# HuiHuiLan/Clustering-Hidden-Markov-Models-with-Variational-Bayesian-Hierarchical-EM

Measured on AMD Instinct MI355X. Metric: VBHEM E-steps/sec (whole node), N baseHMMs × K clusters × S states; ELBO match, higher is better.
Workload: dtype f64; 1 GPU; C4: N=100000 base HMMs, K=16 clusters, S=8 states, Sb=8, d=8, full cov, tau=10, Nv=100; N=100000, K=16, S=8, Sb=8, d=8, tau=10, parallelism=bases sharded over 1 GPU(s), 1 RCCL all-reduce/E-step

## Files before the change

clustering-hidden-markov-models-with-variational-bayesian-hierarchical-em_amd/csrc/vbhem_capi.hip:

```cpp
#include <hip/hip_runtime.h>

#include <algorithm>
#include <atomic>
#include <chrono>
#include <cmath>
#include <cstdio>
#include <cstring>
#include <cstdlib>
#include <random>
#include <string>
#include <utility>
#include <vector>

#include "vbhem_estep.h"
#include "vbhem_internal.h"
#include "vbhem_exact.h"
#include "vbhem_math.h"

static std::atomic<size_t> g_debug_extra_lds{0};

namespace {

thread_local std::string g_err;

struct TimingState {
  int level = 0;
  std::vector<std::pair<hipEvent_t, hipEvent_t>> fb, stats, em, gf, emd;
  std::vector<long long> fb_pairs;
  std::vector<hipEvent_t> pool;
  ~TimingState() {
    for (hipEvent_t e : pool) (void)hipEventDestroy(e);
  }
};
thread_local TimingState g_timing;

thread_local std::string g_last_kernel[3];
std::string split_name(const vbhem::SplitArgs &a) {
  return "vbhem::fb_split_kernel<" + std::to_string(a.S) + ", " + std::to_string(a.lpc) + ", " +
         std::to_string(a.mode) + ">";
}

struct SwitchRow {
  const char *name;
  long long unset;
  long long vbhem::Switches::*field;
};
constexpr SwitchRow kSwitchRows[] = {
#define X(name, unset, doc) {"VBHEM_" #name, unset, &vbhem::Switches::name},
    VBHEM_SWITCHES(X)
#undef X
};
constexpr int kSwitchCount = (int)(sizeof(kSwitchRows) / sizeof(kSwitchRows[0]));

long long switch_value(const SwitchRow &r, long long v) { return r.unset == 0 ? (v != 0) : v; }

const vbhem::Switches &default_switches() {
  static const vbhem::Switches def = [] {
    vbhem::Switches s;
    for (const SwitchRow &r : kSwitchRows)
      if (const char *ev = std::getenv(r.name)) {
        if (r.unset == 0) s.*r.field = ev[0] != '\0' && std::strcmp(ev, "0") != 0;
        else s.*r.field = std::strtoll(ev, nullptr, 10);
      }
    return s;
  }();
  return def;
}
thread_local vbhem::Switches g_switches = default_switches();

const SwitchRow *find_switch(const char *name) {
  if (!name) return nullptr;
  if (std::strncmp(name, "VBHEM_", 6) == 0) name += 6;
  for (const SwitchRow &r : kSwitchRows)
    if (std::strcmp(name, r.name + 6) == 0) return &r;
  return nullptr;
}

bool timing_on(hipStream_t st, bool fb_launch = false) {
  if (g_timing.level == 0 || (g_timing.level == 2 && !fb_launch)) return false;
  hipStreamCaptureStatus cs = hipStreamCaptureStatusNone;
  if (hipStreamIsCapturing(st, &cs) != hipSuccess) return false;
  return cs == hipStreamCaptureStatusNone;
}

hipEvent_t timing_event(hipStream_t st, bool record = true) {
  hipEvent_t ev = nullptr;
  if (!g_timing.pool.empty()) {
    ev = g_timing.pool.back();
    g_timing.pool.pop_back();
  } else if (hipEventCreateWithFlags(&ev, hipEventDisableSystemFence) != hipSuccess) {
    return nullptr;
  }
  if (record) (void)hipEventRecord(ev, st);
  return ev;
}
void timing_recycle(hipEvent_t ev) {
  if (ev) g_timing.pool.push_back(ev);
}

}

namespace vbhem {
const Switches &switches() { return g_switches; }
void *timing_begin(hipStream_t st) { return timing_on(st) ? timing_event(st) : nullptr; }
void timing_end_em_math(void *ev0, hipStream_t st) {
  if (ev0) g_timing.emd.emplace_back(static_cast<hipEvent_t>(ev0), timing_event(st));
}
unsigned long long flag_tag() {
  static const unsigned long long t = [] {
    std::random_device rd;
    unsigned long long v = ((unsigned long long)rd() << 32) ^ rd();
    v ^= (unsigned long long)std::chrono::steady_clock::now().time_since_epoch().count();
    return v | 1ull;
  }();
  return t;
}
}

namespace {

int fail(int code, const std::string &msg) {
  g_err = msg;
  if (code == VBHEM_ERR_HIP) (void)hipGetLastError();
  return code;
}

}

int vbhem::set_error(int code, const std::string &msg) { return fail(code, msg); }

namespace {

using vbhem::align_up;
using vbhem::hip_fail;

constexpr size_t kLdsLimit = 160 * 1024;
constexpr int kFbMaxThreads = 512;
constexpr int kExactThreads = vbhem::kExactSlots;
constexpr int kChunkMinBases = 64;
constexpr size_t kGroupBudget = (size_t)8 << 30;
constexpr int kMaxSlabs = 512;

inline int odd_up(int x) { return (x % 2 == 0) ? x + 1 : x; }

struct FbPlan {
  vbhem::FbArgs a;
  dim3 block;
  size_t lds;
  int PPB;
};

bool plan_fb(int SB, int d, int covmode, int K, int S, int T, FbPlan &out) {
  const int NE = S * SB;
  if (NE > kFbMaxThreads) return false;
  const int RS = odd_up(SB), AS = odd_up(S), ABS = odd_up(SB);
  const int np = covmode == VBHEM_COV_FULL ? d * (d + 1) / 2 : d;
  const int MS = odd_up(d), PS = odd_up(np);
  double best = -1.0;
  bool found = false;
  for (int ppb = 1; ppb <= 32; ++ppb) {
    const int BJ = std::min(ppb, K);
    const int BI = ppb / BJ;
    const int P = BI * BJ;
    if (P != ppb) continue;
    const int threads = (P * NE + 63) / 64 * 64;
    if (threads > kFbMaxThreads) break;
    size_t off = 0;
    vbhem::FbArgs a{};
    a.off_At = (int)off; off += (size_t)BJ * S * AS;
    a.off_amax = (int)off; off += (size_t)BJ * S;
    a.off_lpi = (int)off; off += (size_t)BJ * S;
    a.off_Ab = (int)off; off += (size_t)BI * SB * ABS;
    a.off_pib = (int)off; off += (size_t)BI * SB;
    a.off_flag = (int)off; off += (size_t)(P + 1) / 2;
    a.off_reg = (int)off;
    size_t k1 = 0;
    a.off_k1m = (int)k1; k1 += (size_t)BJ * S * MS;
    a.off_k1P = (int)k1; k1 += (size_t)BJ * S * PS;
    a.off_k1c = (int)k1; k1 += (size_t)BJ * S;
    a.off_k1mu = (int)k1; k1 += (size_t)BI * SB * MS;
    a.off_k1C = (int)k1; k1 += (size_t)BI * SB * PS;
    const size_t pstride = (size_t)(T - 1) * S * RS + (size_t)(T - 1) * NE + 3 * (size_t)S * RS +
                           (size_t)S * S + SB;
    const size_t reg = std::max(k1, (size_t)P * pstride);
    const size_t lds = (off + reg) * sizeof(double);
    if (lds > kLdsLimit) continue;
    const double util = double(P * NE) / threads;
    const int blocks_per_cu = std::max<int>(1, (int)(kLdsLimit / lds));
    const int waves = std::min(32, blocks_per_cu * threads / 64);
    const double score = util * std::min(waves, 16) + 1e-3 * std::min(threads, 256);
    if (score > best) {
      best = score;
      found = true;
      a.SB = SB; a.d = d; a.covmode = covmode; a.K = K; a.S = S; a.T = T;
      a.BI = BI; a.BJ = BJ; a.NE = NE; a.RS = RS; a.AS = AS; a.ABS = ABS;
      a.njb = (K + BJ - 1) / BJ;
      a.np = np; a.MS = MS; a.PS = PS;
      a.pair_stride = (int)pstride;
      out.a = a;
      out.block = dim3(threads);
      out.lds = lds;
      out.PPB = P;
    }
  }
  return found;
}

struct SplitPlan {
  bool ok = false;
  vbhem::SplitArgs a{};
  size_t lds = 0;
  size_t lds_bwd = 0;
  size_t lds_list = 0;
  int ppb = 0;
  vbhem::SplitArgs al{};
  size_t lds_l = 0;
};

SplitPlan plan_split(int SB, int d, int covmode, int K, int S, int T, int LPC) {
  SplitPlan sp;
  if (!vbhem::split_supported(S, SB, d)) return sp;
  const int SH = (S + LPC - 1) / LPC;
  const int LPP = S * LPC;
  const int XCS = (LPC * SH + 1) / 2 * 2 + 2;
  const int XP = S * XCS + 2;
  const int OFF_X = (2 * S * S + 2 * S + 1) / 2 * 2;
  double best = -1.0;
  for (int nwb = 1; nwb <= 4; ++nwb) {
    const int NT = nwb * 64;
    const int ppb = NT / LPP;
    if (ppb < 1) continue;
    const int off_Y = OFF_X + ppb * XP;
    const int off_F = (off_Y + ppb * S + 1) / 2 * 2;
    const int off_R = (off_F + (ppb + 1) / 2 + 1) / 2 * 2;
    const size_t lattice = (size_t)std::max(0, T - 2) * SH * NT;
    const size_t xi_park = S > 8 ? (size_t)ppb * S * S * LPC * SH : 0;
    const size_t region = std::max<size_t>(std::max(lattice, xi_park), 2);
    const size_t lds = ((size_t)off_R + region) * sizeof(double);
    const int off_L = (int)(off_R + region);
    const size_t lds_list = ((size_t)off_L + ((size_t)K + 2) / 2) * sizeof(double);
    if (lds_list > kLdsLimit) continue;
    const double util = double(ppb * LPP) / NT;
    if (util > best + 0.02 || (LPC != vbhem::split_lpc(S) && util >= best)) {
      best = util;
      vbhem::SplitArgs &x = sp.a;
      x.SB = SB; x.d = d; x.covmode = covmode; x.K = K; x.S = S; x.T = T; x.nwb = nwb;
      x.lpc = LPC;
      x.off_Y = off_Y; x.off_F = off_F; x.off_R = off_R; x.off_L = off_L;
      x.mode = vbhem::kFbDense;
      sp.lds = lds;
      x.off_T = off_R + 2;
      sp.lds_bwd = ((size_t)x.off_T + vbhem::kLogTabDoubles + vbhem::kExpTabDoubles) * sizeof(double);
      sp.lds_list = lds_list;
      sp.ppb = ppb;
      sp.ok = true;
    }
  }
  int best_w = 0;
  for (int nwb : {8, 4, 2, 1}) {
    if (!sp.ok) break;
    const int NT = nwb * 64;
    const int ppb = NT / LPP;
    if (ppb < 1) continue;
    const int off_Y = OFF_X + ppb * XP;
    const int off_F = (off_Y + ppb * S + 1) / 2 * 2;
    const int off_R = (off_F + (ppb + 1) / 2 + 1) / 2 * 2;
    const size_t lattice = (size_t)std::max(0, T - 2) * SH * NT;
    const size_t xi_park = S > 8 ? (size_t)ppb * S * S * LPC * SH : 0;
    const size_t region = std::max<size_t>(std::max(lattice, xi_park), 2);
    const int off_L = (int)(off_R + region);
    const int off_T = (off_L + (K + 2) / 2 + 1) / 2 * 2;
    const size_t lds = ((size_t)off_T + vbhem::kExpTabEntries + 2 * vbhem::kLogTabEntries) * sizeof(double);
    if (lds > kLdsLimit) continue;
    const int waves = std::min(8, nwb * (int)(kLdsLimit / lds));
    if (waves > best_w) {
      best_w = waves;
      vbhem::SplitArgs x = sp.a;
      x.nwb = nwb;
      x.off_Y = off_Y; x.off_F = off_F; x.off_R = off_R; x.off_L = off_L; x.off_T = off_T;
      x.mode = vbhem::kFbList;
      sp.al = x;
      sp.lds_l = lds;
    }
  }
  return sp;
}

size_t exact_stride(int S, int SB, int T) {
  return (size_t)S * S * SB * T + (size_t)vbhem::exact_wave_lds(S, SB);
}

int check_inputs(const vbhem_base_t *b, const vbhem_cluster_t *c, int T, bool need_ptrs = true) {
  if (!b || !c) return fail(VBHEM_ERR_ARG, "null base or cluster descriptor");
  if (b->N < 0 || b->SB < 1 || b->d < 1 || c->K < 1 || c->S < 1 || T < 1)
    return fail(VBHEM_ERR_ARG, "invalid sizes (need N>=0, SB>=1, d>=1, K>=1, S>=1, T>=1)");
  if (b->covmode != VBHEM_COV_DIAG && b->covmode != VBHEM_COV_FULL)
    return fail(VBHEM_ERR_ARG, "covmode must be VBHEM_COV_DIAG or VBHEM_COV_FULL");
  if (need_ptrs && b->N > 0 &&
      (!b->prior || !b->A || !b->centres || !b->covars || !c->logA || !c->logPi || !c->m ||
       !c->P || !c->c))
    return fail(VBHEM_ERR_ARG, "null input array");
  if ((long long)b->N * c->K > 0x7fffffffLL)
    return fail(VBHEM_ERR_UNSUPPORTED, "N*K exceeds 2^31-1 pairs per call; shard the bases");
  return VBHEM_OK;
}

void fill_inputs(vbhem::FbArgs &a, const vbhem_base_t *b, const vbhem_cluster_t *c) {
  a.prior = b->prior; a.A = b->A; a.centres = b->centres; a.covars = b->covars;
  a.logA = c->logA; a.logPi = c->logPi; a.m = c->m; a.P = c->P; a.c = c->c;
}

struct Carver {
  char *base;
  size_t off = 0;
  explicit Carver(void *p) : base(static_cast<char *>(p)) {}
  template <class T>
  T *take(size_t n) {
    off = align_up(off, 256);
    T *p = base ? reinterpret_cast<T *>(base + off) : nullptr;
    off += n * sizeof(T);
    return p;
  }
};

bool u_gemm_ok(const vbhem_base_t *b) {
  return vbhem::emission_kdp(b->d, b->covmode) / 4 <= vbhem::kUMaxKq && !vbhem::switches().NO_UGEMM;
}
bool need_u_ws(const vbhem_base_t *b) { return !b->U && u_gemm_ok(b); }

struct PairsWs {
  int *fpre;
  int *flags;
  double *scratch;
  double *tnu;
  double *E, *W, *bias, *shift;
  double *U;
};

inline size_t emission_w_doubles(int d, int covmode, int K, int S) {
  return (size_t)vbhem::emission_kdp(d, covmode) * vbhem::emission_ksp(K * S);
}

size_t carve_pairs(void *ws, const vbhem_base_t *b, const vbhem_cluster_t *c, int T, bool need_tnu,
                   PairsWs &w) {
  Carver cv(ws);
  const size_t np = (size_t)b->N * c->K;
  w.fpre = cv.take<int>(vbhem::kFlagPre + vbhem::kFlagHead + np);
  w.flags = w.fpre + vbhem::kFlagPre;
  w.tnu = need_tnu ? cv.take<double>(np * c->S * b->SB) : nullptr;
  w.E = cv.take<double>(np * c->S * b->SB);
  w.W = cv.take<double>(emission_w_doubles(b->d, b->covmode, c->K, c->S));
  w.bias = cv.take<double>((size_t)vbhem::emission_ksp(c->K * c->S));
  w.shift = cv.take<double>((size_t)b->d);
  w.U = need_u_ws(b) ? cv.take<double>(vbhem::u_doubles((long long)b->N * b->SB + 16, b->d,
                                                         b->covmode))
                     : nullptr;
  w.scratch = cv.take<double>(exact_stride(c->S, b->SB, T) * kExactThreads);
  return cv.off + 256;
}

struct FusedWs {
  int group;
  int nslab;
  int slab_len;
  int *fpre, *flags;
  int *gate_cnt, *list, *list_tot;
  double *Atg;
  double *scratch, *nu1, *xi, *tnu, *Z, *slabs;
  double *E, *W, *bias, *shift;
  double *U;
  double *l4parts;
};

size_t carve_fused(void *ws, const vbhem_base_t *b, const vbhem_cluster_t *c, int T, FusedWs &w,
                   int R = 1) {
  Carver cv(ws);
  const int K = c->K, S = c->S, SB = b->SB;
  const size_t per_base = (size_t)K * (S + (size_t)S * S + 2 * (size_t)S * SB) * sizeof(double);
  size_t g = std::max<size_t>(1, kGroupBudget / std::max<size_t>(1, per_base));
  g = std::min<size_t>(g, (size_t)std::max(1, b->N));
  const vbhem::Switches &sw = vbhem::switches();
  if (sw.GROUP_BASES >= 0)
    g = std::max<size_t>(1, std::min<size_t>(g, (size_t)sw.GROUP_BASES));
  w.group = (int)g;
  int maxslab = kMaxSlabs;
  if (sw.NSLAB >= 0) maxslab = (int)std::max(1ll, std::min(8192ll, sw.NSLAB));
  w.nslab = std::min<int>(w.group, maxslab);
  w.slab_len = R * (int)vbhem_stats_len(K / R, S, b->d, b->covmode);
  w.fpre = cv.take<int>(vbhem::kFlagPre + vbhem::kFlagHead + 2 * g * K);
  w.flags = w.fpre + vbhem::kFlagPre;
  w.nu1 = cv.take<double>(g * K * S);
  w.xi = cv.take<double>(g * K * S * S);
  w.tnu = cv.take<double>(g * K * S * SB);
  w.Z = cv.take<double>(g * K);
  w.slabs = cv.take<double>((size_t)w.nslab * w.slab_len);
  w.E = cv.take<double>(g * K * S * SB);
  w.W = cv.take<double>(emission_w_doubles(b->d, b->covmode, K, S));
  w.bias = cv.take<double>((size_t)vbhem::emission_ksp(K * S));
  w.shift = cv.take<double>((size_t)b->d);
  w.U = need_u_ws(b) ? cv.take<double>(vbhem::u_doubles((long long)g * SB + 16, b->d, b->covmode))
                     : nullptr;
  w.gate_cnt = cv.take<int>((size_t)w.nslab * K);
  w.list = cv.take<int>(g * K);
  w.list_tot = cv.take<int>((size_t)K);
  w.Atg = cv.take<double>((size_t)K * S * S);
  const int NU = (int)vbhem_stats_nu(b->d, b->covmode);
  w.l4parts = vbhem::list4_acc_supported(S, SB, T, K, NU)
                  ? cv.take<double>((size_t)vbhem::l4s_max_slots(kExactThreads, K) *
                                    vbhem::l4s_part_len(S, vbhem::us_nup(NU)))
                  : nullptr;
  w.scratch = cv.take<double>(exact_stride(S, SB, T) * kExactThreads);
  return cv.off + 256;
}

struct FbCtx {
  FbPlan plan;
  SplitPlan split;
  SplitPlan bwd;
  size_t bwd2_lds = 0;
  int bwd2_ppb = 0, bwd2_nwb = 0;
  bool bwd12 = false;
  bool bwd4 = false;
  bool list4 = false;
  bool list12 = false;
  bool k1_in_kernel = false;
  bool bwd2_prep = false;
  int *fpre = nullptr;
  vbhem::EmissionArgs em{};
  size_t em_lds = 0;
  bool use_u = false;
  size_t em_lds_u = 0;
  const vbhem_base_t *base = nullptr;
  double *u_ws = nullptr;
};

int prepare_fb(FbCtx &c, const vbhem_base_t *b, const vbhem_cluster_t *cl, int T,
               double smooth = 1.0, bool split_first_pass = false) {
  c.split = plan_split(b->SB, b->d, b->covmode, cl->K, cl->S, T, vbhem::split_lpc(cl->S));
  c.bwd = plan_split(b->SB, b->d, b->covmode, cl->K, cl->S, T, vbhem::split_lpc_bwd(cl->S));
  if (c.split.ok) {
    vbhem::EmissionArgs &e = c.em;
    e.SB = b->SB; e.d = b->d; e.covmode = b->covmode; e.K = cl->K; e.S = cl->S;
    e.smooth = smooth;
    e.centres = b->centres; e.covars = b->covars; e.m = cl->m; e.P = cl->P; e.c = cl->c;
    if (!vbhem::plan_emission(e, c.em_lds)) c.split.ok = false;
    if (c.split.ok && u_gemm_ok(b) && vbhem::plan_emission_u(e, c.em_lds_u)) {
      c.use_u = true;
      e.zfix = b->U;
    }
  }
  c.base = b;
  const bool have_elems = plan_fb(b->SB, b->d, b->covmode, cl->K, cl->S, T, c.plan);
  if (!c.split.ok && !have_elems)
    return fail(VBHEM_ERR_UNSUPPORTED,
                "no launch geometry fits (S*SB must be <= 512 and the per-pair lattice "
                "(2*(T-1)+3)*S*SB doubles must fit in 160 KiB of LDS)");
  if (!have_elems) c.plan = FbPlan{};
  fill_inputs(c.plan.a, b, cl);
  c.plan.a.SB = b->SB; c.plan.a.d = b->d; c.plan.a.covmode = b->covmode;
  c.plan.a.K = cl->K; c.plan.a.S = cl->S; c.plan.a.T = T;
  c.plan.a.smooth = smooth;
  if (c.split.ok) {
    vbhem::SplitArgs &a = c.split.a;
    a.prior = b->prior; a.A = b->A; a.logA = cl->logA; a.logPi = cl->logPi;
    vbhem::SplitArgs &al = c.split.al;
    al.prior = b->prior; al.A = b->A; al.logA = cl->logA; al.logPi = cl->logPi;
    vbhem::SplitArgs &ab = c.bwd.a;
    ab.prior = b->prior; ab.A = b->A; ab.logA = cl->logA; ab.logPi = cl->logPi;
    if (c.bwd.ok && cl->S <= vbhem::kBwd2MaxS && !vbhem::switches().NO_BWD2) {
      if (!split_first_pass) {
        c.bwd2_nwb = vbhem::bwd2_waves(cl->S);
        c.bwd2_lds = vbhem::bwd2_lds(cl->S, c.bwd2_nwb);
        c.bwd2_ppb = vbhem::bwd2_ppb(cl->S, c.bwd2_nwb);
        c.bwd4 = vbhem::bwd4_supported(cl->S, b->SB) && !vbhem::switches().NO_BWD4;
        c.bwd12 = vbhem::bwd12_supported(cl->S, b->SB) && !vbhem::switches().NO_BWD12;
      }
      c.list4 = vbhem::list4_supported(cl->S, b->SB, T, cl->K) && !vbhem::switches().NO_LIST4;
      c.list12 = vbhem::list12_supported(cl->S, b->SB, T, cl->K) && !vbhem::switches().NO_LIST12;
    }
    c.k1_in_kernel = c.use_u && c.bwd2_lds && !c.bwd4 && !c.bwd12 && !c.list4 && !c.list12 &&
                     c.em.kdp <= vbhem::kK1InKernelMaxKdp && !vbhem::switches().NO_K1_IN_KERNEL;
  }
  return VBHEM_OK;
}

void set_k1_operands(const FbCtx &c, int i_begin, vbhem::SplitArgs &ca) {
  if (c.base->U) {
    ca.eU = c.base->U;
    ca.e_col0 = 0;
  } else {
    ca.eU = c.u_ws;
    ca.e_col0 = (long long)i_begin * c.base->SB / 16 * 16;
  }
  ca.eW = c.em.W;
  ca.ebias = c.em.bias;
  ca.ekdp = c.em.kdp;
  ca.eksp = c.em.ksp;
  ca.esmooth = c.em.smooth;
}

int run_emission_prep(FbCtx &c, double *W, double *bias, double *shift, hipStream_t st,
                      int *zero_ints = nullptr, int n_zero = 0, double *Atg = nullptr,
                      const double *logA = nullptr) {
  if (!c.split.ok) return VBHEM_OK;
  c.em.W = W; c.em.bias = bias; c.em.shift = shift;
  c.em.zero_ints = zero_ints; c.em.n_zero = zero_ints ? n_zero : 0;
  c.em.Atg = Atg; c.em.logA = logA;
  hipError_t e = vbhem::launch_emission_prep(c.em, st);
  if (e != hipSuccess) return hip_fail(e, "emission_prep_kernel");
  return VBHEM_OK;
}

unsigned list_grid(const vbhem::SplitArgs &a, size_t lds) {
  const int cus = vbhem::device_cus();
  const int per_cu = std::max(1, vbhem::split_resident_blocks(a, lds));
  return (unsigned)(cus * per_cu);
}

int run_fb_list(const FbCtx &c, int i_begin, int i_end, int i_buf0, double *nu1, double *xi,
                double *tnu, const double *Ebuf, long long e_ld, const int *list,
                const int *list_tot, int list_cap, int *flags, double *scratch, double *LL,
                hipStream_t st, bool fold = false, bool *inlined = nullptr,
                const vbhem::StatsArgs *acc_sa = nullptr, double *acc_parts = nullptr,
                int *acc_waves = nullptr) {
  if (i_end <= i_begin) return VBHEM_OK;
  if (!c.split.lds_l) return fail(VBHEM_ERR_UNSUPPORTED, "gate-list pass does not fit LDS");
  vbhem::SplitArgs ca = c.split.al;
  ca.mode = vbhem::kFbList;
  ca.E = Ebuf; ca.e_ld = e_ld;
  ca.i_begin = i_begin; ca.i_end = i_end; ca.i_buf0 = i_buf0;
  ca.LL = nullptr; ca.nu1 = nu1; ca.xi = xi; ca.tnu = tnu;
  ca.flag_count = flags; ca.flag_list = flags + vbhem::kFlagHead;
  ca.list = list; ca.list_tot = list_tot; ca.list_cap = list_cap;
  ca.xinline = 0;
  const vbhem::Switches &sw = vbhem::switches();
  const bool acc = c.list4 && acc_sa && acc_parts && acc_sa->Us && acc_sa->Z && !acc_sa->vhem &&
                   vbhem::list4_acc_supported(ca.S, ca.SB, ca.T, ca.K, acc_sa->NU) &&
                   !sw.NO_LIST4_STATS && !sw.NO_STATS_M && !sw.NO_STATS_U;
  if (acc_waves) *acc_waves = 0;
  auto set_inline = [&](long long waves) {
    if (!(fold || (acc && !sw.NO_FOLD_EXACT)) || waves > kExactThreads || sw.NO_LIST_INLINE) return;
    ca.xinline = 1;
    ca.xscr = scratch;
    ca.xstride = (long long)exact_stride(c.plan.a.S, c.plan.a.SB, c.plan.a.T);
    vbhem::FbArgs &x = ca.xf;
    x = c.plan.a;
    x.i_begin = i_begin; x.i_end = i_end; x.i_buf0 = i_buf0;
    x.LL = LL; x.nu1 = nu1; x.xi = xi; x.tnu = tnu;
    x.flag_count = flags; x.flag_list = flags + vbhem::kFlagHead;
  };
  hipEvent_t ev0 = timing_on(st) ? timing_event(st) : nullptr;
  hipError_t e;
  if (c.list4) {
    ca.Atg = c.bwd.a.Atg;
    unsigned grid = (unsigned)(vbhem::device_cus() * std::max(1, vbhem::list4_resident_blocks(acc)));
    set_inline(vbhem::list4_inline_waves(ca, grid));
    if (acc && ca.xinline) {
      ca.acc = 1;
      ca.acc_nup = vbhem::us_nup(acc_sa->NU);
      ca.accZ = acc_sa->Z; ca.accUs = acc_sa->Us; ca.acc_parts = acc_parts;
      if (acc_waves) *acc_waves = (int)vbhem::list4_inline_waves(ca, grid);
    } else if (acc) {
      grid = (unsigned)(vbhem::device_cus() * std::max(1, vbhem::list4_resident_blocks()));
      if (fold) set_inline(vbhem::list4_inline_waves(ca, grid));
    }
    e = vbhem::launch_list4(ca, grid, st);
    if (e != hipSuccess) return hip_fail(e, "fb_list4_kernel");
    g_last_kernel[1] = "vbhem::fb_list4_kernel<" + std::to_string(ca.T) +
                       (vbhem::list4_fast(ca) ? ", true>" : ", false>");
  } else if (c.list12) {
    ca.Atg = c.bwd.a.Atg;
    const unsigned grid = (unsigned)(vbhem::device_cus() * std::max(1, vbhem::list12_resident_blocks()));
    e = vbhem::launch_list12(ca, grid, st);
    if (e != hipSuccess) return hip_fail(e, "fb_list12_kernel");
    g_last_kernel[1] = "vbhem::fb_list12_kernel<" + std::to_string(ca.T) +
                       (vbhem::list12_fast(ca) ? ", true>" : ", false>");
  } else {
    if (c.k1_in_kernel) set_k1_operands(c, i_begin, ca);
    const unsigned grid = list_grid(ca, c.split.lds_l);
    if (ca.S >= vbhem::kSplitInlineMinS && ca.S <= vbhem::kSplitInlineMaxS)
      set_inline((long long)grid * ca.nwb);
    e = vbhem::launch_split(ca, grid, c.split.lds_l, st);
    if (e != hipSuccess) return hip_fail(e, "fb_split_kernel(list)");
    g_last_kernel[1] = split_name(ca);
  }
  if (ev0) g_timing.gf.emplace_back(ev0, timing_event(st));
  if (inlined) *inlined = ca.xinline != 0;
  if (fold) return VBHEM_OK;
  vbhem::FbArgs a = c.plan.a;
  a.i_begin = i_begin; a.i_end = i_end; a.i_buf0 = i_buf0;
  a.LL = LL; a.nu1 = nu1; a.xi = xi; a.tnu = tnu;
  a.flag_count = flags; a.flag_list = flags + vbhem::kFlagHead;
  e = vbhem::launch_fb_exact(a, scratch, exact_stride(a.S, a.SB, a.T), kExactThreads, st);
  if (e != hipSuccess) return hip_fail(e, "fb_exact_kernel");
  return VBHEM_OK;
}

int run_fb(const FbCtx &c, int i_begin, int i_end, int i_buf0, double *LL, double *nu1,
           double *xi, double *tnu, double *Ebuf, long long e_ld, int *flags, double *scratch,
           hipStream_t st, int mode = vbhem::kFbDense, vbhem::FbArgs *fold = nullptr) {
  if (i_end <= i_begin) return VBHEM_OK;
  vbhem::FbArgs a = c.plan.a;
  a.i_begin = i_begin;
  a.i_end = i_end;
  a.i_buf0 = i_buf0;
  a.LL = LL; a.nu1 = nu1; a.xi = xi; a.tnu = tnu;
  a.flag_count = flags;
  a.flag_list = flags + vbhem::kFlagHead;
  hipError_t e = hipSuccess;
  const bool k1 = c.k1_in_kernel && mode == vbhem::kFbBackward;
  if (!c.split.ok) {
    e = hipMemsetAsync(flags, 0, sizeof(int), st);
    if (e != hipSuccess) return hip_fail(e, "hipMemsetAsync(flags)");
  }
  if (c.split.ok) {
    vbhem::EmissionArgs ea = c.em;
    ea.i_begin = i_begin; ea.i_end = i_end; ea.i_buf0 = i_buf0; ea.E = Ebuf; ea.e_ld = e_ld;
    size_t em_lds = c.em_lds;
    hipEvent_t em0 = !k1 && timing_on(st) ? timing_event(st) : nullptr;
    if (c.use_u) {
      em_lds = c.em_lds_u;
      if (c.base->U) {
        ea.U = c.base->U;
        ea.u_col0 = 0;
      } else {
        if (!c.u_ws) return fail(VBHEM_ERR_WORKSPACE, "no operand buffer for the emission GEMM");
        const vbhem_base_t *b = c.base;
        vbhem::UPrepArgs ua{};
        ua.N = b->N; ua.SB = b->SB; ua.d = b->d; ua.covmode = b->covmode;
        ua.kdp = c.em.kdp; ua.i_begin = i_begin; ua.i_end = i_end;
        ua.u_col0 = (long long)i_begin * b->SB / 16 * 16;
        ua.nstates = b->nstates; ua.centres = b->centres; ua.covars = b->covars;
        ua.U = c.u_ws; ua.z = c.em.shift;
        e = vbhem::launch_u_prep(ua, st);
        if (e != hipSuccess) return hip_fail(e, "u_prep_kernel");
        ea.U = c.u_ws;
        ea.u_col0 = ua.u_col0;
      }
    }
    if (!k1) {
      e = vbhem::launch_emission(ea, em_lds, st);
      if (e != hipSuccess) return hip_fail(e, "emission_kernel");
      if (em0) g_timing.em.emplace_back(em0, timing_event(st));
    }
  }
  const bool ext_timed = c.split.ok && mode == vbhem::kFbBackward && (c.bwd4 || c.bwd12 || c.bwd2_lds);
  const bool timed = timing_on(st, true);
  hipEvent_t ev0 = timed ? timing_event(st, !ext_timed) : nullptr;
  hipEvent_t ev1 = timed && ext_timed ? timing_event(st, false) : nullptr;
  if (c.split.ok) {
    const SplitPlan &sp = mode == vbhem::kFbBackward ? c.bwd : c.split;
    vbhem::SplitArgs ca = sp.a;
    ca.mode = mode;
    ca.E = Ebuf; ca.e_ld = e_ld;
    ca.i_begin = i_begin; ca.i_end = i_end; ca.i_buf0 = i_buf0;
    ca.LL = LL; ca.nu1 = nu1; ca.xi = xi; ca.tnu = tnu;
    ca.flag_count = flags; ca.flag_list = flags + vbhem::kFlagHead;
    const unsigned ntile = (unsigned)((i_end - i_begin + sp.ppb - 1) / sp.ppb);
    unsigned grid = ntile * (unsigned)ca.K;
    if (mode == vbhem::kFbBackward && c.bwd4) {
      const int ppb = vbhem::bwd4_ppb();
      const unsigned nt4 = (unsigned)((i_end - i_begin + ppb - 1) / ppb);
      const unsigned all = (unsigned)(vbhem::device_cus() * std::max(1, vbhem::bwd4_resident_blocks()));
      unsigned nb = std::max(1u, std::min(nt4, all / (unsigned)ca.K));
      if (nb >= 8) nb = nb / 8 * 8;
      e = vbhem::launch_bwd4(ca, (unsigned)ca.K * nb, st, ev1 ? ev0 : nullptr, ev1);
      if (e != hipSuccess) return hip_fail(e, "fb_bwd4_kernel");
      g_last_kernel[0] = vbhem::bwd4_o32(ca) ? "vbhem::fb_bwd4_kernel<true>" : "vbhem::fb_bwd4_kernel<false>";
    } else if (mode == vbhem::kFbBackward && c.bwd12) {
      const int ppb = vbhem::bwd12_ppb();
      const unsigned nt12 = (unsigned)((i_end - i_begin + ppb - 1) / ppb);
      const unsigned all = (unsigned)(vbhem::device_cus() * std::max(1, vbhem::bwd12_resident_blocks()));
      unsigned nb = std::max(1u, std::min(nt12, all / (unsigned)ca.K));
      if (nb >= 8) nb = nb / 8 * 8;
      e = vbhem::launch_bwd12(ca, (unsigned)ca.K * nb, st, ev1 ? ev0 : nullptr, ev1);
      if (e != hipSuccess) return hip_fail(e, "fb_bwd12_kernel");
      g_last_kernel[0] = vbhem::bwd12_o32(ca) ? "vbhem::fb_bwd12_kernel<true>" : "vbhem::fb_bwd12_kernel<false>";
    } else if (mode == vbhem::kFbBackward && c.bwd2_lds) {
      ca.nwb = c.bwd2_nwb;
      if (k1) set_k1_operands(c, i_begin, ca);
      if (k1 && c.bwd2_prep) {
        ca.prep = 1;
        ca.pm = c.em.m; ca.pP = c.em.P; ca.pc = c.em.c; ca.pz = c.em.zfix; ca.pshift = c.em.shift;
        ca.ftag = reinterpret_cast<unsigned long long *>(c.fpre);
        ca.ftag_val = vbhem::flag_tag();
      }
      const unsigned nt2 = (unsigned)((i_end - i_begin + c.bwd2_ppb - 1) / c.bwd2_ppb);
      const unsigned all = (unsigned)(vbhem::device_cus() *
                                      std::max(1, vbhem::bwd2_resident_blocks(ca.S, ca.nwb, c.bwd2_lds)));
      unsigned nb = std::max(1u, std::min(nt2, all / (unsigned)ca.K));
      if (nb >= 8) nb = nb / 8 * 8;
      const size_t lds2 = c.bwd2_lds + g_debug_extra_lds.load(std::memory_order_relaxed);
      e = vbhem::launch_bwd2(ca, (unsigned)ca.K * nb, lds2, st, ev1 ? ev0 : nullptr, ev1);
      if (e != hipSuccess) return hip_fail(e, "fb_bwd2_kernel");
      g_last_kernel[0] = "vbhem::fb_bwd2_kernel<" + std::to_string(ca.S) + ">";
    } else {
      if (mode == vbhem::kFbBackward) {
        unsigned nb = std::max(1u, std::min(ntile, list_grid(ca, sp.lds_bwd) / (unsigned)ca.K));
        if (nb >= 8) nb = nb / 8 * 8;
        grid = (unsigned)ca.K * nb;
      }
      e = vbhem::launch_split(ca, grid, mode == vbhem::kFbBackward ? sp.lds_bwd : sp.lds, st);
      if (e != hipSuccess) return hip_fail(e, "fb_split_kernel");
      g_last_kernel[0] = split_name(ca);
    }
  } else {
    const int nib = (i_end - i_begin + a.BI - 1) / a.BI;
    const dim3 grid((unsigned)nib * (unsigned)a.njb);
    e = vbhem::launch_fb(a, grid, c.plan.block, c.plan.lds, st);
    if (e != hipSuccess) return hip_fail(e, "fb_pairs_kernel");
    g_last_kernel[0] = "vbhem::fb_pairs_kernel";
  }
  if (ev0) {
    g_timing.fb.emplace_back(ev0, ev1 ? ev1 : timing_event(st));
    g_timing.fb_pairs.push_back((long long)(i_end - i_begin) * a.K);
  }
  if (fold) {
    *fold = a;
    return VBHEM_OK;
  }
  e = vbhem::launch_fb_exact(a, scratch, exact_stride(a.S, a.SB, a.T), kExactThreads, st);
  if (e != hipSuccess) return hip_fail(e, "fb_exact_kernel");
  return VBHEM_OK;
}

}

extern "C" {

const char *vbhem_last_error(void) { return g_err.c_str(); }

size_t vbhem_debug_extra_lds(size_t bytes) { return g_debug_extra_lds.exchange(bytes); }

const char *vbhem_last_kernel(int pass) {
  return (pass >= 0 && pass <= 2) ? g_last_kernel[pass].c_str() : "";
}

const char *vbhem_version(void) { return "vbhem-mi355x 0.1.0 (gfx950)"; }

size_t vbhem_stats_nu(int d, int covmode) {
  return covmode == VBHEM_COV_FULL ? (size_t)1 + d + (size_t)d * (d + 1) / 2 : (size_t)1 + 2 * d;
}

size_t vbhem_stats_len(int K, int S, int d, int covmode) {
  return (size_t)K + (size_t)K * S + (size_t)K * S * S + 2 + (size_t)K * S * vbhem_stats_nu(d, covmode);
}

size_t vbhem_prepare_base_bytes(const vbhem_base_t *base) {
  if (!base || base->N < 0 || base->SB < 1 || base->d < 1 || base->d > vbhem::kUHead ||
      (base->covmode != VBHEM_COV_DIAG && base->covmode != VBHEM_COV_FULL))
    return 0;
  if (vbhem::emission_kdp(base->d, base->covmode) / 4 > vbhem::kUMaxKq) return 0;
  return (vbhem::u_doubles((long long)base->N * base->SB, base->d, base->covmode) +
          vbhem::us_doubles(base->N, base->SB, base->d, base->covmode)) * sizeof(double);
}

int vbhem_prepare_base(const vbhem_base_t *base, double *U_dev, size_t bytes, void *stream) {
  const size_t need = vbhem_prepare_base_bytes(base);
  if (need == 0)
    return fail(VBHEM_ERR_UNSUPPORTED, "vbhem_prepare_base: invalid descriptor or d too large");
  if (!U_dev || bytes < need)
    return fail(VBHEM_ERR_WORKSPACE, "vbhem_prepare_base: need " + std::to_string(need) + " bytes");
  if (base->N > 0 && (!base->centres || !base->covars))
    return fail(VBHEM_ERR_ARG, "vbhem_prepare_base: null base array");
  vbhem::UPrepArgs ua{};
  ua.N = base->N; ua.SB = base->SB; ua.d = base->d; ua.covmode = base->covmode;
  ua.kdp = vbhem::emission_kdp(base->d, base->covmode);
  ua.i_begin = 0; ua.i_end = base->N; ua.u_col0 = 0;
  ua.nstates = base->nstates; ua.centres = base->centres; ua.covars = base->covars;
  ua.U = U_dev; ua.z = nullptr;
  hipError_t e = vbhem::launch_u_prep(ua, static_cast<hipStream_t>(stream));
  if (e != hipSuccess) return hip_fail(e, "u_prep_kernel");
  e = vbhem::launch_us_build(ua, U_dev + vbhem::u_doubles((long long)base->N * base->SB, base->d,
                                                         base->covmode),
                             static_cast<hipStream_t>(stream));
  if (e != hipSuccess) return hip_fail(e, "us_build_kernel");
  return VBHEM_OK;
}

size_t vbhem_pairs_workspace_bytes(const vbhem_base_t *base, const vbhem_cluster_t *clus, int T) {
  if (check_inputs(base, clus, T, false) != VBHEM_OK) return 0;
  PairsWs w;
  return carve_pairs(nullptr, base, clus, T, true, w);
}

}

namespace {

int estep_pairs_impl(const vbhem_base_t *base, const vbhem_cluster_t *clus, int T, double smooth,
                     double *LL_elbo_dev, double *sum_nu_1_dev, double *emit_pr_dev,
                     double *emit_mu_dev, double *emit_Mu_dev, double *sum_xi_dev,
                     double *sum_t_nu_dev, void *workspace_dev, size_t workspace_bytes,
                     void *stream) {
  if (!(smooth > 0.0) || !std::isfinite(smooth))
    return fail(VBHEM_ERR_ARG, "smooth must be a positive finite number");
  int rc = check_inputs(base, clus, T);
  if (rc != VBHEM_OK) return rc;
  if (base->N == 0) return VBHEM_OK;
  if (!LL_elbo_dev || !sum_nu_1_dev || !emit_pr_dev || !emit_mu_dev || !emit_Mu_dev || !sum_xi_dev)
    return fail(VBHEM_ERR_ARG, "null output array");
  PairsWs w;
  const size_t need = carve_pairs(nullptr, base, clus, T, sum_t_nu_dev == nullptr, w);
  if (!workspace_dev || workspace_bytes < need)
    return fail(VBHEM_ERR_WORKSPACE, "workspace too small: need " + std::to_string(need) + " bytes");
  carve_pairs(workspace_dev, base, clus, T, sum_t_nu_dev == nullptr, w);
  double *tnu = sum_t_nu_dev ? sum_t_nu_dev : w.tnu;
  hipStream_t st = static_cast<hipStream_t>(stream);
  FbCtx ctx;
  rc = prepare_fb(ctx, base, clus, T, smooth);
  if (rc != VBHEM_OK) return rc;
  ctx.u_ws = w.U;
  if (!ctx.split.ok) {
    hipError_t e0 = hipMemsetAsync(w.fpre, 0, (vbhem::kFlagPre + vbhem::kFlagHead) * sizeof(int), st);
    if (e0 != hipSuccess) return hip_fail(e0, "hipMemsetAsync(flags)");
  }
  rc = run_emission_prep(ctx, w.W, w.bias, w.shift, st, w.fpre, vbhem::kFlagPre + vbhem::kFlagHead);
  if (rc != VBHEM_OK) return rc;
  rc = run_fb(ctx, 0, base->N, 0, LL_elbo_dev, sum_nu_1_dev, sum_xi_dev, tnu, w.E,
              (long long)base->N * base->SB, w.flags,
              w.scratch, st);
  if (rc != VBHEM_OK) return rc;
  vbhem::EmitArgs ea{};
  ea.SB = base->SB; ea.d = base->d; ea.covmode = base->covmode; ea.K = clus->K; ea.S = clus->S;
  ea.i_begin = 0; ea.i_end = base->N;
  ea.centres = base->centres; ea.covars = base->covars; ea.tnu = tnu;
  ea.emit_pr = emit_pr_dev; ea.emit_mu = emit_mu_dev; ea.emit_Mu = emit_Mu_dev;
  hipError_t e = vbhem::launch_emit(ea, st);
  if (e != hipSuccess) return hip_fail(e, "pair_emit_kernel");
  return VBHEM_OK;
}

}

extern "C" {

int vbhem_estep_pairs(const vbhem_base_t *base, const vbhem_cluster_t *clus, int T,
                      double *LL_elbo_dev, double *sum_nu_1_dev, double *emit_pr_dev,
                      double *emit_mu_dev, double *emit_Mu_dev, double *sum_xi_dev,
                      double *sum_t_nu_dev, void *workspace_dev, size_t workspace_bytes,
                      void *stream) {
  return estep_pairs_impl(base, clus, T, 1.0, LL_elbo_dev, sum_nu_1_dev, emit_pr_dev, emit_mu_dev,
                          emit_Mu_dev, sum_xi_dev, sum_t_nu_dev, workspace_dev, workspace_bytes,
                          stream);
}

int vhem_estep_pairs(const vbhem_base_t *base, const vbhem_cluster_t *clus, int T, double smooth,
                     double *LL_elbo_dev, double *sum_nu_1_dev, double *emit_pr_dev,
                     double *emit_mu_dev, double *emit_Mu_dev, double *sum_xi_dev,
                     double *sum_t_nu_dev, void *workspace_dev, size_t workspace_bytes,
                     void *stream) {
  return estep_pairs_impl(base, clus, T, smooth, LL_elbo_dev, sum_nu_1_dev, emit_pr_dev,
                          emit_mu_dev, emit_Mu_dev, sum_xi_dev, sum_t_nu_dev, workspace_dev,
                          workspace_bytes, stream);
}

size_t vbhem_fused_workspace_bytes(const vbhem_base_t *base, const vbhem_cluster_t *clus, int T) {
  return vbhem_fused_trials_workspace_bytes(base, clus, 1, T);
}

size_t vbhem_fused_trials_workspace_bytes(const vbhem_base_t *base, const vbhem_cluster_t *clus,
                                          int R, int T) {
  if (check_inputs(base, clus, T, false) != VBHEM_OK || R < 1 || clus->K % R != 0) return 0;
  FusedWs w;
  return carve_fused(nullptr, base, clus, T, w, R);
}

int vbhem_estep_fused(const vbhem_base_t *base, const vbhem_cluster_t *clus, int T,
                      const double *tildeN_dev, const double *logOmega_dev, double *stats_dev,
                      double *hatZ_dev, double *LL_elbo_dev, void *workspace_dev,
                      size_t workspace_bytes, void *stream) {
  return vbhem_estep_fused_trials(base, clus, 1, T, tildeN_dev, logOmega_dev, stats_dev, hatZ_dev,
                                  LL_elbo_dev, workspace_dev, workspace_bytes, stream);
}

static std::atomic<unsigned long long *> g_done_word{nullptr};
static std::atomic<unsigned long long> g_done_val{0};

int vbhem_arm_done_word(void *word, unsigned long long value) {
  if (word && reinterpret_cast<uintptr_t>(word) % 8 != 0) return fail(VBHEM_ERR_ARG, "done word not 8-byte aligned");
  g_done_val.store(value);
  g_done_word.store(static_cast<unsigned long long *>(word));
  return VBHEM_OK;
}

int vbhem_done_word_alloc(void **host_ptr, void **dev_ptr) {
  if (!host_ptr || !dev_ptr) return fail(VBHEM_ERR_ARG, "null pointer");
  void *h = nullptr;
  hipError_t e = hipHostMalloc(&h, 64, hipHostMallocMapped | hipHostMallocCoherent);
  if (e != hipSuccess) return hip_fail(e, "hipHostMalloc(done word)");
  std::memset(h, 0, 64);
  void *d = nullptr;
  e = hipHostGetDevicePointer(&d, h, 0);
  if (e != hipSuccess) {
    (void)hipHostFree(h);
    return hip_fail(e, "hipHostGetDevicePointer(done word)");
  }
  *host_ptr = h;
  *dev_ptr = d;
  return VBHEM_OK;
}

int vbhem_done_word_free(void *host_ptr) {
  if (!host_ptr) return VBHEM_OK;
  const hipError_t e = hipHostFree(host_ptr);
  return e == hipSuccess ? VBHEM_OK : hip_fail(e, "hipHostFree(done word)");
}

struct VhemIn {
  double smooth, inf_norm;
  const double *omegaB;
};

static int fused_impl(const vbhem_base_t *base, const vbhem_cluster_t *clus, int R, int T,
                      const double *tildeN_dev, const double *logOmega_dev, double *stats_dev,
                      double *hatZ_dev, double *LL_elbo_dev, void *workspace_dev,
                      size_t workspace_bytes, void *stream, const VhemIn *vh) {
  unsigned long long *const done_word = g_done_word.exchange(nullptr);
  const unsigned long long done_val = g_done_val.load();
  int rc = check_inputs(base, clus, T);
  if (rc != VBHEM_OK) return rc;
  if (vh) {
    if (!(vh->smooth > 0.0) || !std::isfinite(vh->smooth))
      return fail(VBHEM_ERR_ARG, "smooth must be a positive finite number");
    if (!(vh->inf_norm > 0.0) || !std::isfinite(vh->inf_norm))
      return fail(VBHEM_ERR_ARG, "inf_norm must be a positive finite number");
    if (base->N > 0 && !vh->omegaB) return fail(VBHEM_ERR_ARG, "null fused argument");
  }
  if (R < 1 || clus->K % R != 0)
    return fail(VBHEM_ERR_ARG, "trials: K must be a positive multiple of R");
  if (!vh && R > 1 && clus->K > 256)
    return fail(VBHEM_ERR_UNSUPPORTED, "trials: at most 256 clusters in total (R * K_trial)");
  if (!logOmega_dev || !stats_dev ||
      (base->N > 0 && (!tildeN_dev || !hatZ_dev || !LL_elbo_dev)))
    return fail(VBHEM_ERR_ARG, "null fused argument");
  if ((vh ? vbhem::vhem_resp_lds(clus->K, clus->K / R) : vbhem::resp_lds(clus->K, clus->K / R)) >
      kLdsLimit)
    return fail(VBHEM_ERR_UNSUPPORTED, "fused: too many clusters for the responsibilities "
                                       "kernel (K <= ~2,400)");
  FusedWs w;
  const size_t need = carve_fused(nullptr, base, clus, T, w, R);
  if (!workspace_dev || workspace_bytes < need)
    return fail(VBHEM_ERR_WORKSPACE, "workspace too small: need " + std::to_string(need) + " bytes");
  carve_fused(workspace_dev, base, clus, T, w, R);
  hipStream_t st = static_cast<hipStream_t>(stream);

  const int K = clus->K, S = clus->S, SB = base->SB, d = base->d;
  vbhem::StatsArgs sa{};
  sa.K = K; sa.S = S; sa.SB = SB; sa.d = d; sa.covmode = base->covmode;
  sa.NU = (int)vbhem_stats_nu(d, base->covmode);
  sa.slab_len = w.slab_len;
  sa.KT = K / R;
  sa.SL = w.slab_len / R;
  sa.centres = base->centres; sa.covars = base->covars; sa.LL = LL_elbo_dev;
  sa.nu1 = w.nu1; sa.xi = w.xi; sa.tnu = w.tnu; sa.tildeN = tildeN_dev; sa.logOmega = logOmega_dev;
  sa.Z = w.Z; sa.hatZ = hatZ_dev; sa.slabs = w.slabs;
  if (vh) {
    sa.vhem = 1;
    sa.omegaB = vh->omegaB;
    sa.inf_norm = vh->inf_norm;
  }
  size_t slds = 0;
  int ngroups = 1;
  const bool dense_ok = vbhem::plan_stats(sa, slds, ngroups);

  FbCtx ctx;
  rc = prepare_fb(ctx, base, clus, T, vh ? vh->smooth : 1.0, vh != nullptr);
  if (rc != VBHEM_OK) return rc;
  ctx.u_ws = w.U;
  size_t sl_lds = 0;
  const vbhem::Switches &sw = vbhem::switches();
  const bool gated = !sw.FUSED_DENSE && ctx.split.ok && ctx.split.lds_l &&
                     vbhem::plan_stats_list(sa, sl_lds) &&
                     vbhem::gate_list_lds(K) <= kLdsLimit;
  if (R > 1 && !gated)
    return fail(VBHEM_ERR_UNSUPPORTED,
                "trials need the gated schedule (split-kernel shapes: S <= 16, Sb <= S)");
  if (!gated && !dense_ok)
    return fail(VBHEM_ERR_UNSUPPORTED, "statistics tile does not fit (S or d too large)");
  sa.gate_cnt = gated ? w.gate_cnt : nullptr;
  sa.list = w.list; sa.list_tot = w.list_tot; sa.list_cap = w.group;
  auto chunks = [&w](int nb) { return std::min(w.nslab, (nb + kChunkMinBases - 1) / kChunkMinBases); };
  const int nslab_used = std::max(1, chunks(std::min(base->N, w.group)));
  sa.nzero_m = std::min(nslab_used, 128);
  int stats_slabs = nslab_used;
  hipError_t e = hipSuccess;
  if (!gated || base->N == 0) {
    e = hipMemsetAsync(w.slabs, 0, sizeof(double) * (size_t)nslab_used * w.slab_len, st);
    if (e != hipSuccess) return hip_fail(e, "hipMemsetAsync(slabs)");
  }
  struct HeadGuard {
    int *fpre;
    hipStream_t st;
    ~HeadGuard() {
      if (fpre) (void)hipMemsetAsync(fpre, 0, (vbhem::kFlagPre + vbhem::kFlagHead) * sizeof(int), st);
    }
  } guard{w.fpre, st};
  if (!ctx.split.ok) {
    e = hipMemsetAsync(w.fpre, 0, (vbhem::kFlagPre + vbhem::kFlagHead) * sizeof(int), st);
    if (e != hipSuccess) return hip_fail(e, "hipMemsetAsync(flags)");
  }
  if (gated) ctx.bwd.a.Atg = w.Atg;
  if (gated && ctx.k1_in_kernel && ctx.em.zfix && ctx.bwd2_nwb * 64 >= 512 &&
      !sw.NO_BWD2_PREP) {
    ctx.em.W = w.W; ctx.em.bias = w.bias; ctx.em.shift = w.shift;
    ctx.bwd2_prep = true;
    ctx.fpre = w.fpre;
  } else {
    rc = run_emission_prep(ctx, w.W, w.bias, w.shift, st, w.fpre, vbhem::kFlagPre + vbhem::kFlagHead,
                           gated ? w.Atg : nullptr, clus->logA);
    if (rc != VBHEM_OK) return rc;
  }
  const bool fold = gated && R == 1 && base->N <= w.group && ctx.split.ok && K < kExactThreads &&
                    w.nslab <= kExactThreads && !sw.NO_FOLD_EXACT;
  sa.fold = 0;
  for (int g0 = 0; g0 < base->N; g0 += w.group) {
    const int g1 = std::min(base->N, g0 + w.group);
    const long long e_ld = (long long)w.group * SB;
    rc = run_fb(ctx, g0, g1, g0, LL_elbo_dev, w.nu1, w.xi, w.tnu, w.E, e_ld, w.flags, w.scratch,
                st, gated ? vbhem::kFbBackward : vbhem::kFbDense, fold ? &sa.fx : nullptr);
    if (rc != VBHEM_OK) return rc;
    if (fold) {
      sa.fold = 1;
      sa.xscratch = w.scratch;
      sa.xstride = (long long)exact_stride(S, SB, T);
      sa.xslots = kExactThreads;
    }
    sa.i_begin = g0; sa.i_end = g1; sa.i_buf0 = g0;
    sa.assign = gated && g0 == 0;
    sa.U = nullptr;
    sa.Us = nullptr;
    if (ctx.split.ok && ctx.use_u) {
      sa.ukdp = ctx.em.kdp;
      if (base->U) {
        sa.U = base->U; sa.uz = base->U; sa.u_col0 = 0;
        sa.Us = base->U + vbhem::u_doubles((long long)base->N * SB, base->d, base->covmode);
      } else if (ctx.u_ws) {
        sa.U = ctx.u_ws; sa.uz = ctx.em.shift; sa.u_col0 = (long long)g0 * SB / 16 * 16;
      }
    }
    const int nchunk = std::max(1, chunks(g1 - g0));
    hipEvent_t ev0 = timing_on(st) ? timing_event(st) : nullptr;
    e = vbhem::launch_resp(sa, nchunk, st);
    if (e != hipSuccess) return hip_fail(e, "resp_kernel");
    if (gated) {
      e = vbhem::launch_gate_list(sa, nchunk, st);
      if (e != hipSuccess) return hip_fail(e, "gate_list_kernel");
      if (ev0) g_timing.stats.emplace_back(ev0, timing_event(st));
      bool inl = false;
      int l4w = 0;
      rc = run_fb_list(ctx, g0, g1, g0, w.nu1, w.xi, w.tnu, w.E, e_ld, w.list, w.list_tot,
                       w.group, w.flags, w.scratch, LL_elbo_dev, st, fold, &inl, &sa, w.l4parts, &l4w);
      if (rc != VBHEM_OK) return rc;
      if (fold) sa.fold = inl ? 2 : 1;
      ev0 = timing_on(st) ? timing_event(st) : nullptr;
      int ss = nchunk;
      if (l4w > 0) {
        ss = 1;
        g_last_kernel[2] = "vbhem::list4_stats_reduce_kernel";
        e = vbhem::launch_list4_stats_reduce(sa, w.l4parts, l4w, st);
        if (e != hipSuccess) return hip_fail(e, "list4_stats_reduce_kernel");
      } else {
        g_last_kernel[2] = "vbhem::stats_list_kernels";
        e = vbhem::launch_stats_list(sa, nchunk, sl_lds, st, &ss);
      }
      if (e != hipSuccess) return hip_fail(e, "stats_list_kernel");
      if (g0 == 0) stats_slabs = ss;
    } else {
      e = vbhem::launch_stats(sa, nchunk, ngroups, slds, st);
      if (e != hipSuccess) return hip_fail(e, "stats_kernel");
    }
    if (ev0) g_timing.stats.emplace_back(ev0, timing_event(st));
  }
  e = vbhem::launch_stats_final(w.slabs, nslab_used, stats_slabs, w.slab_len, sa.KT, S, sa.SL,
                                stats_dev, st, w.fpre, done_word, done_val);
  if (e != hipSuccess) return hip_fail(e, "stats_final_kernel");
  guard.fpre = nullptr;
  return VBHEM_OK;
}

int vbhem_estep_fused_trials(const vbhem_base_t *base, const vbhem_cluster_t *clus, int R, int T,
                             const double *tildeN_dev, const double *logOmega_dev,
                             double *stats_dev, double *hatZ_dev, double *LL_elbo_dev,
                             void *workspace_dev, size_t workspace_bytes, void *stream) {
  return fused_impl(base, clus, R, T, tildeN_dev, logOmega_dev, stats_dev, hatZ_dev, LL_elbo_dev,
                    workspace_dev, workspace_bytes, stream, nullptr);
}

size_t vhem_fused_workspace_bytes(const vbhem_base_t *base, const vbhem_cluster_t *clus, int T) {
  return vbhem_fused_trials_workspace_bytes(base, clus, 1, T);
}

size_t vhem_fused_trials_workspace_bytes(const vbhem_base_t *base, const vbhem_cluster_t *clus,
                                         int R, int T) {
  return vbhem_fused_trials_workspace_bytes(base, clus, R, T);
}

int vhem_estep_fused(const vbhem_base_t *base, const vbhem_cluster_t *clus, int T, double smooth,
                     const double *Ni_dev, const double *omegaB_dev, double inf_norm,
                     const double *logOmega_dev, double *stats_dev, double *Z_dev,
                     double *LL_elbo_dev, void *workspace_dev, size_t workspace_bytes,
                     void *stream) {
  return vhem_estep_fused_trials(base, clus, 1, T, smooth, Ni_dev, omegaB_dev, inf_norm,
                                 logOmega_dev, stats_dev, Z_dev, LL_elbo_dev, workspace_dev,
                                 workspace_bytes, stream);
}

int vhem_estep_fused_trials(const vbhem_base_t *base, const vbhem_cluster_t *clus, int R, int T,
                            double smooth, const double *Ni_dev, const double *omegaB_dev,
                            double inf_norm, const double *logOmega_dev, double *stats_dev,
                            double *Z_dev, double *LL_elbo_dev, void *workspace_dev,
                            size_t workspace_bytes, void *stream) {
  const VhemIn vh{smooth, inf_norm, omegaB_dev};
  return fused_impl(base, clus, R, T, Ni_dev, logOmega_dev, stats_dev, Z_dev, LL_elbo_dev,
                    workspace_dev, workspace_bytes, stream, &vh);
}

int vbhem_set_fused_mode(int mode) {
  const int prev = g_switches.FUSED_DENSE ? VBHEM_FUSED_DENSE : VBHEM_FUSED_GATED;
  if (mode == VBHEM_FUSED_GATED || mode == VBHEM_FUSED_DENSE)
    g_switches.FUSED_DENSE = mode == VBHEM_FUSED_DENSE;
  return prev;
}

int vbhem_switch_count(void) { return kSwitchCount; }

const char *vbhem_switch_name(int index) {
  return index >= 0 && index < kSwitchCount ? kSwitchRows[index].name : nullptr;
}

int vbhem_switch_get(const char *name, long long *value) {
  const SwitchRow *r = find_switch(name);
  if (!r) return fail(VBHEM_ERR_ARG, std::string("unknown switch: ") + (name ? name : "(null)"));
  if (value) *value = g_switches.*r->field;
  return VBHEM_OK;
}

int vbhem_switch_set(const char *name, long long value, long long *previous) {
  const SwitchRow *r = find_switch(name);
  if (!r) return fail(VBHEM_ERR_ARG, std::string("unknown switch: ") + (name ? name : "(null)"));
  if (previous) *previous = g_switches.*r->field;
  g_switches.*r->field = switch_value(*r, value);
  return VBHEM_OK;
}

void vbhem_switch_reset(void) { g_switches = default_switches(); }

int vbhem_timing_enable(int on) {
  g_timing.level = (on == 1 || on == 2) ? on : 0;
  return VBHEM_OK;
}

int vbhem_timing_read(double *fb_ms, long long *fb_launches, long long *fb_pairs, double *stats_ms,
                      long long *stats_launches) {
  double f = 0.0, s = 0.0;
  long long np = 0;
  int rc = VBHEM_OK;
  auto drain = [&rc](std::vector<std::pair<hipEvent_t, hipEvent_t>> &v, double &acc) {
    for (auto &pr : v) {
      float ms = 0.f;
      if (pr.first && pr.second) {
        hipError_t e = hipEventSynchronize(pr.second);
        if (e == hipSuccess) e = hipEventElapsedTime(&ms, pr.first, pr.second);
        if (e != hipSuccess) rc = hip_fail(e, "vbhem_timing_read");
        acc += ms;
      }
      timing_recycle(pr.first);
      timing_recycle(pr.second);
    }
  };
  const long long nf = (long long)g_timing.fb.size(), ns = (long long)g_timing.stats.size();
  drain(g_timing.fb, f);
  drain(g_timing.stats, s);
  for (long long x : g_timing.fb_pairs) np += x;
  g_timing.fb.clear();
  g_timing.stats.clear();
  g_timing.fb_pairs.clear();
  if (fb_ms) *fb_ms = f;
  if (fb_launches) *fb_launches = nf;
  if (fb_pairs) *fb_pairs = np;
  if (stats_ms) *stats_ms = s;
  if (stats_launches) *stats_launches = ns;
  return rc;
}

static int drain_events(std::vector<std::pair<hipEvent_t, hipEvent_t>> &v, double *ms_out,
                        long long *n_out, const char *where) {
  double t = 0.0;
  int rc = VBHEM_OK;
  const long long n = (long long)v.size();
  for (auto &pr : v) {
    float ms = 0.f;
    if (pr.first && pr.second) {
      hipError_t e = hipEventSynchronize(pr.second);
      if (e == hipSuccess) e = hipEventElapsedTime(&ms, pr.first, pr.second);
      if (e != hipSuccess) rc = hip_fail(e, where);
      t += ms;
    }
    timing_recycle(pr.first);
    timing_recycle(pr.second);
  }
  v.clear();
  if (ms_out) *ms_out = t;
  if (n_out) *n_out = n;
  return rc;
}

int vbhem_timing_read_em_math(double *ms, long long *launches) {
  return drain_events(g_timing.emd, ms, launches, "vbhem_timing_read_em_math");
}

int vbhem_timing_read_gated(double *fwd_ms, long long *fwd_launches) {
  return drain_events(g_timing.gf, fwd_ms, fwd_launches, "vbhem_timing_read_gated");
}

int vbhem_timing_read_emission(double *em_ms, long long *em_launches) {
  double t = 0.0;
  int rc = VBHEM_OK;
  const long long n = (long long)g_timing.em.size();
  for (auto &pr : g_timing.em) {
    float ms = 0.f;
    if (pr.first && pr.second) {
      hipError_t e = hipEventSynchronize(pr.second);
      if (e == hipSuccess) e = hipEventElapsedTime(&ms, pr.first, pr.second);
      if (e != hipSuccess) rc = hip_fail(e, "vbhem_timing_read_emission");
      t += ms;
    }
    timing_recycle(pr.first);
    timing_recycle(pr.second);
  }
  g_timing.em.clear();
  if (em_ms) *em_ms = t;
  if (em_launches) *em_launches = n;
  return rc;
}

int vbhem_last_fallback_count(void *stream, const void *workspace_dev) {
  int v[vbhem::kFlagPre + 2] = {0};
  if (!workspace_dev) return fail(VBHEM_ERR_ARG, "null workspace");
  hipStream_t st = static_cast<hipStream_t>(stream);
  hipError_t e = hipMemcpyAsync(v, workspace_dev, sizeof(v), hipMemcpyDeviceToHost, st);
  if (e == hipSuccess) e = hipStreamSynchronize(st);
  if (e != hipSuccess) return hip_fail(e, "vbhem_last_fallback_count");
  if (v[vbhem::kFlagLost] == vbhem::kFlagLostMark)
    return fail(VBHEM_ERR_WORKSPACE, "fb_bwd2_kernel lost the flag-head handshake: the fused "
                                     "call's statistics are NaN (results untrusted)");
  return std::max(v[2], std::max(v[vbhem::kFlagPre], v[vbhem::kFlagPre + 1]));
}

int vbhem_host_device_pointer(void *host_ptr, void **dev_ptr) {
  if (!host_ptr || !dev_ptr) return fail(VBHEM_ERR_ARG, "null pointer");
  *dev_ptr = nullptr;
  hipPointerAttribute_t at{};
  if (hipPointerGetAttributes(&at, host_ptr) != hipSuccess || at.type != hipMemoryTypeHost) {
    (void)hipGetLastError();
    return fail(VBHEM_ERR_ARG, "not pinned host memory");
  }
  void *d = nullptr;
  hipError_t e = hipHostGetDevicePointer(&d, host_ptr, 0);
  if (e != hipSuccess || !d) {
    (void)hipGetLastError();
    return fail(VBHEM_ERR_ARG, "pinned host memory is not mapped for the device");
  }
  *dev_ptr = d;
  return VBHEM_OK;
}

}

namespace {

int estep_pairs_host_impl(int device, const vbhem_base_t *bh, const vbhem_cluster_t *ch, int T,
                          double smooth, double *LL_elbo, double *sum_nu_1, double *emit_pr,
                          double *emit_mu, double *emit_Mu, double *sum_xi) {
  int rc = check_inputs(bh, ch, T);
  if (rc != VBHEM_OK) return rc;
  if (bh->N == 0) return VBHEM_OK;
  hipError_t e = hipSetDevice(device);
  if (e != hipSuccess) return hip_fail(e, "hipSetDevice");
  const size_t N = bh->N, SB = bh->SB, d = bh->d, K = ch->K, S = ch->S;
  const size_t dC = bh->covmode == VBHEM_COV_FULL ? d * d : d;
  const size_t n_in[] = {N * SB, N * SB * SB, N * SB * d, N * SB * dC,
                         K * S * S, K * S, K * S * d, K * S * dC, K * S};
  const double *h_in[] = {bh->prior, bh->A, bh->centres, bh->covars,
                          ch->logA, ch->logPi, ch->m, ch->P, ch->c};
  const size_t n_out[] = {N * K, N * K * S, N * K * S, N * K * S * d, N * K * S * dC, N * K * S * S};
  double *h_out[] = {LL_elbo, sum_nu_1, emit_pr, emit_mu, emit_Mu, sum_xi};
  double *d_in[9] = {nullptr};
  double *d_out[6] = {nullptr};
  void *ws = nullptr;
  rc = VBHEM_OK;
  for (int k = 0; k < 9 && rc == VBHEM_OK; ++k) {
    e = hipMalloc(&d_in[k], std::max<size_t>(1, n_in[k]) * sizeof(double));
    if (e == hipSuccess) e = hipMemcpy(d_in[k], h_in[k], n_in[k] * sizeof(double), hipMemcpyHostToDevice);
    if (e != hipSuccess) rc = hip_fail(e, "upload");
  }
  for (int k = 0; k < 6 && rc == VBHEM_OK; ++k) {
    e = hipMalloc(&d_out[k], std::max<size_t>(1, n_out[k]) * sizeof(double));
    if (e != hipSuccess) rc = hip_fail(e, "hipMalloc(out)");
  }
  vbhem_base_t bd = *bh;
  vbhem_cluster_t cd = *ch;
  bd.nstates = nullptr;
  bd.U = nullptr;
  bd.prior = d_in[0]; bd.A = d_in[1]; bd.centres = d_in[2]; bd.covars = d_in[3];
  cd.logA = d_in[4]; cd.logPi = d_in[5]; cd.m = d_in[6]; cd.P = d_in[7]; cd.c = d_in[8];
  size_t wsb = 0;
  if (rc == VBHEM_OK) {
    wsb = vbhem_pairs_workspace_bytes(&bd, &cd, T);
    e = hipMalloc(&ws, wsb);
    if (e != hipSuccess) rc = hip_fail(e, "hipMalloc(workspace)");
  }
  if (rc == VBHEM_OK)
    rc = estep_pairs_impl(&bd, &cd, T, smooth, d_out[0], d_out[1], d_out[2], d_out[3], d_out[4],
                          d_out[5], nullptr, ws, wsb, nullptr);
  if (rc == VBHEM_OK) {
    e = hipDeviceSynchronize();
    if (e != hipSuccess) rc = hip_fail(e, "kernel execution");
  }
  for (int k = 0; k < 6 && rc == VBHEM_OK; ++k) {
    e = hipMemcpy(h_out[k], d_out[k], n_out[k] * sizeof(double), hipMemcpyDeviceToHost);
    if (e != hipSuccess) rc = hip_fail(e, "download");
  }
  for (int k = 0; k < 9; ++k) if (d_in[k]) (void)hipFree(d_in[k]);
  for (int k = 0; k < 6; ++k) if (d_out[k]) (void)hipFree(d_out[k]);
  if (ws) (void)hipFree(ws);
  return rc;
}

}

extern "C" {

int vbhem_estep_pairs_host(int device, const vbhem_base_t *bh, const vbhem_cluster_t *ch, int T,
                           double *LL_elbo, double *sum_nu_1, double *emit_pr, double *emit_mu,
                           double *emit_Mu, double *sum_xi) {
  return estep_pairs_host_impl(device, bh, ch, T, 1.0, LL_elbo, sum_nu_1, emit_pr, emit_mu,
                               emit_Mu, sum_xi);
}

int vhem_estep_pairs_host(int device, const vbhem_base_t *bh, const vbhem_cluster_t *ch, int T,
                          double smooth, double *LL_elbo, double *sum_nu_1, double *emit_pr,
                          double *emit_mu, double *emit_Mu, double *sum_xi) {
  return estep_pairs_host_impl(device, bh, ch, T, smooth, LL_elbo, sum_nu_1, emit_pr, emit_mu,
                               emit_Mu, sum_xi);
}

}

struct vbhem_ctx {
  int device = 0, N = 0, SB = 0, d = 0, covmode = 0, K = 0, S = 0, R = 1, T = 1;
  size_t stats_len = 0, ws_bytes = 0;
  hipStream_t stream = nullptr;
  int *nstates = nullptr;
  double *prior = nullptr, *A = nullptr, *centres = nullptr, *covars = nullptr;
  double *logA = nullptr, *logPi = nullptr, *m = nullptr, *P = nullptr, *c = nullptr;
  double *tildeN = nullptr, *logOmega = nullptr, *stats = nullptr, *hatZ = nullptr, *LL = nullptr;
  double *U = nullptr;
  void *ws = nullptr;
};

namespace {

void ctx_free(vbhem_ctx *x) {
  if (!x) return;
  int prev = 0;
  const bool dev_ok = hipGetDevice(&prev) == hipSuccess && hipSetDevice(x->device) == hipSuccess;
  void *ptrs[] = {x->nstates, x->prior, x->A, x->centres, x->covars, x->logA, x->logPi, x->m,
                  x->P, x->c, x->tildeN, x->logOmega, x->stats, x->hatZ, x->LL, x->U, x->ws};
  for (void *q : ptrs)
    if (q) (void)hipFree(q);
  if (x->stream) (void)hipStreamDestroy(x->stream);
  if (dev_ok) (void)hipSetDevice(prev);
  delete x;
}

template <class T>
hipError_t dev_alloc(T **p, size_t n) {
  return hipMalloc(reinterpret_cast<void **>(p), std::max<size_t>(1, n) * sizeof(T));
}

}

extern "C" {

int vbhem_ctx_create(int device, const vbhem_base_t *bh, int K, int S, int R, int T,
                     vbhem_ctx_t **ctx_out) {
  if (!ctx_out) return fail(VBHEM_ERR_ARG, "null context pointer");
  *ctx_out = nullptr;
  vbhem_cluster_t probe{K, S, nullptr, nullptr, nullptr, nullptr, nullptr};
  int rc = check_inputs(bh, &probe, T, false);
  if (rc != VBHEM_OK) return rc;
  if (bh->N > 0 && (!bh->prior || !bh->A || !bh->centres || !bh->covars))
    return fail(VBHEM_ERR_ARG, "null base array");
  if (R < 1 || K % R != 0) return fail(VBHEM_ERR_ARG, "trials: K must be a positive multiple of R");
  vbhem_ctx *x = new vbhem_ctx;
  x->device = device; x->N = bh->N; x->SB = bh->SB; x->d = bh->d; x->covmode = bh->covmode;
  x->K = K; x->S = S; x->R = R; x->T = T;
  x->stats_len = (size_t)R * vbhem_stats_len(K / R, S, bh->d, bh->covmode);
  hipError_t e = hipSetDevice(device);
  if (e != hipSuccess) { ctx_free(x); return hip_fail(e, "hipSetDevice"); }
  e = hipStreamCreateWithFlags(&x->stream, hipStreamNonBlocking);
  const size_t N = bh->N, SB = bh->SB, d = bh->d;
  const size_t dC = bh->covmode == VBHEM_COV_FULL ? d * d : d;
  if (e == hipSuccess) e = dev_alloc(&x->nstates, N);
  if (e == hipSuccess) e = dev_alloc(&x->prior, N * SB);
  if (e == hipSuccess) e = dev_alloc(&x->A, N * SB * SB);
  if (e == hipSuccess) e = dev_alloc(&x->centres, N * SB * d);
  if (e == hipSuccess) e = dev_alloc(&x->covars, N * SB * dC);
  if (e == hipSuccess) e = dev_alloc(&x->logA, (size_t)K * S * S);
  if (e == hipSuccess) e = dev_alloc(&x->logPi, (size_t)K * S);
  if (e == hipSuccess) e = dev_alloc(&x->m, (size_t)K * S * d);
  if (e == hipSuccess) e = dev_alloc(&x->P, (size_t)K * S * dC);
  if (e == hipSuccess) e = dev_alloc(&x->c, (size_t)K * S);
  if (e == hipSuccess) e = dev_alloc(&x->tildeN, N);
  if (e == hipSuccess) e = dev_alloc(&x->logOmega, (size_t)K);
  if (e == hipSuccess) e = dev_alloc(&x->stats, x->stats_len);
  if (e == hipSuccess) e = dev_alloc(&x->hatZ, N * K);
  if (e == hipSuccess) e = dev_alloc(&x->LL, N * K);
  if (e != hipSuccess) { ctx_free(x); return hip_fail(e, "vbhem_ctx_create(alloc)"); }
  if (N > 0) {
    if (bh->nstates) {
      e = hipMemcpy(x->nstates, bh->nstates, N * sizeof(int), hipMemcpyHostToDevice);
    } else {
      std::vector<int> ns(N, (int)SB);
      e = hipMemcpy(x->nstates, ns.data(), N * sizeof(int), hipMemcpyHostToDevice);
    }
    if (e == hipSuccess) e = hipMemcpy(x->prior, bh->prior, N * SB * 8, hipMemcpyHostToDevice);
    if (e == hipSuccess) e = hipMemcpy(x->A, bh->A, N * SB * SB * 8, hipMemcpyHostToDevice);
    if (e == hipSuccess) e = hipMemcpy(x->centres, bh->centres, N * SB * d * 8, hipMemcpyHostToDevice);
    if (e == hipSuccess) e = hipMemcpy(x->covars, bh->covars, N * SB * dC * 8, hipMemcpyHostToDevice);
    if (e != hipSuccess) { ctx_free(x); return hip_fail(e, "vbhem_ctx_create(upload)"); }
  }
  vbhem_base_t bd{bh->N, bh->SB, bh->d, bh->covmode, x->nstates, x->prior, x->A, x->centres,
                  x->covars, nullptr};
  if (const size_t ub = vbhem_prepare_base_bytes(&bd)) {
    e = hipMalloc(&x->U, ub);
    if (e != hipSuccess) { ctx_free(x); return hip_fail(e, "vbhem_ctx_create(U)"); }
    rc = vbhem_prepare_base(&bd, x->U, ub, x->stream);
    if (rc != VBHEM_OK) { ctx_free(x); return rc; }
    bd.U = x->U;
  }
  vbhem_cluster_t cd{K, S, x->logA, x->logPi, x->m, x->P, x->c};
  x->ws_bytes = vbhem_fused_trials_workspace_bytes(&bd, &cd, R, T);
  if (x->ws_bytes == 0) { ctx_free(x); return fail(VBHEM_ERR_ARG, "vbhem_ctx_create: bad sizes"); }
  e = hipMalloc(&x->ws, x->ws_bytes);
  if (e != hipSuccess) { ctx_free(x); return hip_fail(e, "vbhem_ctx_create(workspace)"); }
  *ctx_out = x;
  return VBHEM_OK;
}

int vbhem_ctx_fused(vbhem_ctx_t *x, const vbhem_cluster_t *ch, const double *tildeN_host,
                    const double *logOmega_host, double *stats_host, double *hatZ_host,
                    double *LL_host) {
  if (!x || !ch) return fail(VBHEM_ERR_ARG, "null context or cluster descriptor");
  if (ch->K != x->K || ch->S != x->S)
    return fail(VBHEM_ERR_ARG, "cluster descriptor K/S differ from the context's");
  if (!ch->logA || !ch->logPi || !ch->m || !ch->P || !ch->c || !logOmega_host || !stats_host ||
      (x->N > 0 && !tildeN_host))
    return fail(VBHEM_ERR_ARG, "null host array");
  hipError_t e = hipSetDevice(x->device);
  if (e != hipSuccess) return hip_fail(e, "hipSetDevice");
  const size_t K = x->K, S = x->S, d = x->d, N = x->N;
  const size_t dC = x->covmode == VBHEM_COV_FULL ? d * d : d;
  hipStream_t st = x->stream;
  e = hipMemcpyAsync(x->logA, ch->logA, K * S * S * 8, hipMemcpyHostToDevice, st);
  if (e == hipSuccess) e = hipMemcpyAsync(x->logPi, ch->logPi, K * S * 8, hipMemcpyHostToDevice, st);
  if (e == hipSuccess) e = hipMemcpyAsync(x->m, ch->m, K * S * d * 8, hipMemcpyHostToDevice, st);
  if (e == hipSuccess) e = hipMemcpyAsync(x->P, ch->P, K * S * dC * 8, hipMemcpyHostToDevice, st);
  if (e == hipSuccess) e = hipMemcpyAsync(x->c, ch->c, K * S * 8, hipMemcpyHostToDevice, st);
  if (e == hipSuccess) e = hipMemcpyAsync(x->logOmega, logOmega_host, K * 8, hipMemcpyHostToDevice, st);
  if (e == hipSuccess && N > 0)
    e = hipMemcpyAsync(x->tildeN, tildeN_host, N * 8, hipMemcpyHostToDevice, st);
  if (e != hipSuccess) return hip_fail(e, "vbhem_ctx_fused(upload)");
  vbhem_base_t bd{x->N, x->SB, x->d, x->covmode, x->nstates, x->prior, x->A, x->centres,
                  x->covars, x->U};
  vbhem_cluster_t cd{x->K, x->S, x->logA, x->logPi, x->m, x->P, x->c};
  int rc = vbhem_estep_fused_trials(&bd, &cd, x->R, x->T, x->tildeN, x->logOmega, x->stats,
                                    x->hatZ, x->LL, x->ws, x->ws_bytes, st);
  if (rc != VBHEM_OK) return rc;
  e = hipMemcpyAsync(stats_host, x->stats, x->stats_len * 8, hipMemcpyDeviceToHost, st);
  if (e == hipSuccess && hatZ_host && N > 0)
    e = hipMemcpyAsync(hatZ_host, x->hatZ, N * K * 8, hipMemcpyDeviceToHost, st);
  if (e == hipSuccess && LL_host && N > 0)
    e = hipMemcpyAsync(LL_host, x->LL, N * K * 8, hipMemcpyDeviceToHost, st);
  if (e == hipSuccess) e = hipStreamSynchronize(st);
  if (e != hipSuccess) return hip_fail(e, "vbhem_ctx_fused(download)");
  return VBHEM_OK;
}

void vbhem_ctx_destroy(vbhem_ctx_t *x) { ctx_free(x); }

int vbhem_estep_fused_host(int device, const vbhem_base_t *bh, const vbhem_cluster_t *ch, int T,
                           const double *tildeN_host, const double *logOmega_host,
                           double *stats_host, double *hatZ_host, double *LL_host) {
  if (!ch) return fail(VBHEM_ERR_ARG, "null cluster descriptor");
  vbhem_ctx_t *x = nullptr;
  int rc = vbhem_ctx_create(device, bh, ch->K, ch->S, 1, T, &x);
  if (rc != VBHEM_OK) return rc;
  rc = vbhem_ctx_fused(x, ch, tildeN_host, logOmega_host, stats_host, hatZ_host, LL_host);
  vbhem_ctx_destroy(x);
  return rc;
}

}
```

clustering-hidden-markov-models-with-variational-bayesian-hierarchical-em_amd/csrc/vbhem_internal.h:

```cpp
#pragma once
#include <hip/hip_runtime.h>

#include <cstddef>
#include <map>
#include <mutex>
#include <string>
#include <tuple>

#include "vbhem_estep.h"
#include "vbhem_switches.h"
#include "vbhem_list4_slots.h"

namespace vbhem {

int set_error(int code, const std::string &msg);
static inline int hip_fail(hipError_t e, const char *where) {
  return set_error(VBHEM_ERR_HIP, std::string(where) + ": " + hipGetErrorString(e));
}

static inline size_t align_up(size_t x, size_t a) { return (x + a - 1) / a * a; }

inline int current_device() {
  int dev = 0;
  if (hipGetDevice(&dev) != hipSuccess) dev = 0;
  return dev;
}
inline hipError_t set_dyn_lds(const void *fn, size_t lds) {
  static std::mutex mu;
  static std::map<std::pair<int, const void *>, size_t> done;
  const auto key = std::make_pair(current_device(), fn);
  std::lock_guard<std::mutex> g(mu);
  auto it = done.find(key);
  if (it != done.end() && it->second >= lds) return hipSuccess;
  hipError_t e = hipFuncSetAttribute(fn, hipFuncAttributeMaxDynamicSharedMemorySize, (int)lds);
  if (e == hipSuccess) done[key] = lds;
  return e;
}
inline int resident_per_cu(const void *fn, int threads, size_t lds) {
  static std::mutex mu;
  static std::map<std::tuple<int, const void *, int, size_t>, int> memo;
  const auto key = std::make_tuple(current_device(), fn, threads, lds);
  {
    std::lock_guard<std::mutex> g(mu);
    auto it = memo.find(key);
    if (it != memo.end()) return it->second;
  }
  int n = 0;
  if (set_dyn_lds(fn, lds) != hipSuccess ||
      hipOccupancyMaxActiveBlocksPerMultiprocessor(&n, fn, threads, lds) != hipSuccess || n < 1)
    return 1;
  std::lock_guard<std::mutex> g(mu);
  memo[key] = n;
  return n;
}
inline int device_cus() {
  static std::mutex mu;
  static std::map<int, int> cus;
  const int dev = current_device();
  {
    std::lock_guard<std::mutex> g(mu);
    auto it = cus.find(dev);
    if (it != cus.end()) return it->second;
  }
  int n = 0;
  if (hipDeviceGetAttribute(&n, hipDeviceAttributeMultiprocessorCount, dev) != hipSuccess || n < 1)
    return 256;
  std::lock_guard<std::mutex> g(mu);
  cus[dev] = n;
  return n;
}

constexpr int kCovDiag = 0;
constexpr int kCovFull = 1;

struct FbArgs {
  int SB, d, covmode, K, S, T;
  int BI, BJ, NE, RS, AS, ABS, njb;
  int i_begin, i_end, i_buf0;
  int np, MS, PS;
  const double *prior, *A, *centres, *covars;
  const double *logA, *logPi, *m, *P, *c;
  double *LL, *nu1, *xi, *tnu;
  int *flag_count, *flag_list;
  int off_At, off_amax, off_lpi, off_Ab, off_pib, off_flag, off_reg;
  int off_k1m, off_k1P, off_k1c, off_k1mu, off_k1C;
  int pair_stride;
  double smooth;
};

struct EmitArgs {
  int SB, d, covmode, K, S;
  int i_begin, i_end;
  const double *centres, *covars, *tnu;
  double *emit_pr, *emit_mu, *emit_Mu;
};

struct StatsArgs {
  int K, S, SB, SBp, d, covmode, NU;
  int JG;
  int NBB;
  int AST;
  int UST;
  int i_begin, i_end, i_buf0, slab_len;
  const double *centres, *covars, *LL, *nu1, *xi, *tnu, *tildeN, *logOmega;
  double *Z;
  double *hatZ, *slabs;
  int *gate_cnt;
  int *list;
  int *list_tot;
  int list_cap;
  int PB;
  int assign;
  int KT, SL;
  const double *U, *uz;
  long long u_col0;
  int ukdp;
  int nzero;
  const double *Us;
  int nzero_m;
  int fold;
  FbArgs fx;
  double *xscratch;
  long long xstride;
  int xslots;
  int vhem;
  const double *omegaB;
  double inf_norm;
};

constexpr int kSplitMaxS = 16;
template <int S>
struct SplitLPC {
#ifdef VBHEM_SPLIT_LPC5
  static constexpr int value = S <= 4 ? 1 : S == 5 ? VBHEM_SPLIT_LPC5 : S <= 8 ? 2 : 4;
#else
  static constexpr int value = S <= 4 ? 1 : S <= 8 ? 2 : 4;
#endif
};
template <int S>
struct BwdLPC {
  static constexpr int value = S <= 8 ? 1 : 2;
};
template <int S, int LPC>
struct SplitLayout {
  static constexpr int SH = (S + LPC - 1) / LPC;
  static constexpr int XCS = (LPC * SH + 1) / 2 * 2 + 2;
  static constexpr int XP = S * XCS + 2;
  static constexpr int HEAD = 2 * S * S + 2 * S;
  static constexpr int OFF_X = (HEAD + 1) / 2 * 2;
};
inline int emission_kdp(int d, int covmode) {
  const int kd = covmode == kCovFull ? d * (d + 1) / 2 + d : 2 * d;
  return (kd + 3) / 4 * 4;
}
inline int emission_ksp(int ks) { return (ks + 127) / 128 * 128; }

struct EmissionArgs {
  int SB, d, covmode, K, S, KD, CB;
  int kdp, ksp;
  bool wfull;
  bool wlds;
  int nwave;
  int i_begin, i_end, i_buf0;
  long long e_ld;
  const double *centres, *covars, *m, *P, *c;
  double *W, *bias, *shift;
  double *E;
  double smooth;
  const double *U, *zfix;
  long long u_col0;
  int urc;
  int ukqb;
  const double *logA;
  double *Atg;
  int *zero_ints;
  int n_zero;
};
bool plan_emission(EmissionArgs &a, size_t &lds);
bool plan_emission_u(EmissionArgs &a, size_t &lds);

constexpr int kUHead = 64;
constexpr int kUMaxKq = 40;
inline long long u_tiles(long long ncols) { return (ncols + 15) / 16; }
inline size_t u_doubles(long long ncols, int d, int covmode) {
  return (size_t)kUHead + (size_t)u_tiles(ncols) * (emission_kdp(d, covmode) / 4) * 64;
}
struct UPrepArgs {
  int N, SB, d, covmode, kdp;
  int i_begin, i_end;
  long long u_col0;
  const int *nstates;
  const double *centres, *covars;
  double *U;
  const double *z;
};
hipError_t launch_u_prep(const UPrepArgs &a, hipStream_t st);
__host__ __device__ inline int us_sbp(int SB) { return (SB + 3) / 4 * 4; }
__host__ __device__ inline int us_nup(int NU) { return (NU + 15) / 16 * 16; }
__host__ __device__ inline int us_nu(int d, int covmode) { return 1 + d + (covmode == kCovFull ? d * (d + 1) / 2 : d); }
inline size_t us_doubles(long long N, int SB, int d, int covmode) {
  return (size_t)N * us_sbp(SB) * us_nup(us_nu(d, covmode));
}
hipError_t launch_us_build(const UPrepArgs &a, double *Us, hipStream_t st);
hipError_t launch_emission_prep(const EmissionArgs &a, hipStream_t st);
hipError_t launch_emission(const EmissionArgs &a, size_t lds, hipStream_t st);

enum FbMode : int { kFbDense = 0, kFbBackward = 1, kFbList = 2 };

struct SplitArgs {
  int SB, d, covmode, K, S, T, nwb, lpc;
  int mode;
  int i_begin, i_end, i_buf0;
  int off_Y, off_F, off_R;
  int off_L;
  int off_T;
  const double *prior, *A;
  const double *logA, *logPi;
  const double *E;
  long long e_ld;
  double *LL, *nu1, *xi, *tnu;
  int *flag_count, *flag_list;
  const int *list, *list_tot;
  int list_cap;
  const double *Atg;
  const double *eU, *eW, *ebias;
  long long e_col0;
  int ekdp, eksp;
  double esmooth;
  int xinline;
  double *xscr;
  long long xstride;
  FbArgs xf;
  int prep;
  const double *pm, *pP, *pc, *pz;
  double *pshift;
  unsigned long long *ftag;
  unsigned long long ftag_val;
  int acc;
  int acc_nup;
  const double *accZ;
  const double *accUs;
  double *acc_parts;
};

constexpr double kLog2PiE = 1.8378770664093454835606594728112353;
__device__ __forceinline__ double em_psym(const double *P, int a, int b, int d) {
  return 0.5 * (P[a * d + b] + P[b * d + a]);
}
__device__ __forceinline__ double em_pm_full(const double *P, const double *mr, const double *zs,
                                             int a, int d) {
  double v = 0.0;
  for (int b = 0; b < d; ++b) v = fma(em_psym(P, a, b, d), mr[b] - zs[b], v);
  return v;
}
__device__ __forceinline__ double em_w_full(const double *P, int a, int b, int d) {
  return -0.5 * ((a == b) ? P[a * d + a] : em_psym(P, a, b, d));
}
__device__ __forceinline__ double em_bias(int d, double c, double q) {
  return -0.5 * (d * kLog2PiE + c + q);
}

constexpr int kK1InKernelMaxKdp = 8;
constexpr int kSplitInlineMinS = 4, kSplitInlineMaxS = 6;

__device__ __forceinline__ void k1_column(const SplitArgs &p, long long col,
                                          double (&u)[kK1InKernelMaxKdp]) {
  const long long c = col - p.e_col0;
  const double *Ut = p.eU + kUHead + (size_t)(c >> 4) * (p.ekdp / 4) * 64 + (int)(c & 15);
#pragma unroll
  for (int e = 0; e < kK1InKernelMaxKdp; ++e)
    u[e] = e < p.ekdp ? Ut[(e >> 2) * 64 + (e & 3) * 16] : 0.0;
}
__device__ __forceinline__ double k1_entry(const SplitArgs &p, int jr,
                                           const double (&u)[kK1InKernelMaxKdp]) {
  double acc = p.ebias[jr];
#pragma unroll
  for (int e = 0; e < kK1InKernelMaxKdp; ++e)
    if (e < p.ekdp) acc = fma(p.eW[(size_t)e * p.eksp + jr], u[e], acc);
  return acc;
}
bool split_supported(int S, int SB, int d);
int split_lpc(int S);
int split_lpc_bwd(int S);
hipError_t launch_split(const SplitArgs &a, unsigned grid, size_t lds, hipStream_t st);
int split_resident_blocks(const SplitArgs &a, size_t lds);

constexpr int kBwd2MaxS = 16;
int bwd2_waves(int S);
size_t bwd2_lds(int S, int nwb);
int bwd2_ppb(int S, int nwb);
int bwd2_resident_blocks(int S, int nwb, size_t lds);
hipError_t launch_bwd2(const SplitArgs &a, unsigned grid, size_t lds, hipStream_t st,
                       hipEvent_t t0 = nullptr, hipEvent_t t1 = nullptr);

void *timing_begin(hipStream_t st);
void timing_end_em_math(void *ev0, hipStream_t st);

bool bwd4_supported(int S, int SB);
int bwd4_waves();
int bwd4_ppb();
int bwd4_resident_blocks();
bool bwd4_o32(const SplitArgs &a);
bool bwd12_o32(const SplitArgs &a);
bool list4_fast(const SplitArgs &a);
bool list12_fast(const SplitArgs &a);
hipError_t launch_bwd4(const SplitArgs &a, unsigned grid, hipStream_t st, hipEvent_t t0 = nullptr,
                       hipEvent_t t1 = nullptr);
bool bwd12_supported(int S, int SB);
int bwd12_ppb();
int bwd12_resident_blocks();
hipError_t launch_bwd12(const SplitArgs &a, unsigned grid, hipStream_t st, hipEvent_t t0 = nullptr,
                        hipEvent_t t1 = nullptr);

constexpr int kList4MaxK = 1024;
bool list4_supported(int S, int SB, int T, int K);
int list4_resident_blocks(bool acc = false);
long long list4_inline_waves(const SplitArgs &a, unsigned grid);
hipError_t launch_list4(const SplitArgs &a, unsigned grid, hipStream_t st);
bool list4_acc_supported(int S, int SB, int T, int K, int NU);
hipError_t launch_list4_stats_reduce(const StatsArgs &a, const double *parts, int nw, hipStream_t st);

bool list12_supported(int S, int SB, int T, int K);
int list12_resident_blocks();
hipError_t launch_list12(const SplitArgs &a, unsigned grid, hipStream_t st);

hipError_t launch_fb(const FbArgs &a, dim3 grid, dim3 block, size_t lds, hipStream_t st);
constexpr int kFlagHead = 4;
constexpr int kFlagPre = 4;
constexpr int kFlagLost = 3;
constexpr int kFlagLostMark = 0x4C4F5354;
unsigned long long flag_tag();
constexpr int kFlagBad = 1, kFlagNonFinite = 2;
#ifndef VBHEM_EXACT_BLOCK
#define VBHEM_EXACT_BLOCK 512
#endif
constexpr int kExactBlock = VBHEM_EXACT_BLOCK;
constexpr int kExactBlocks = 131072 / kExactBlock;
constexpr int kExactSlots = kExactBlocks * kExactBlock / 64;
hipError_t launch_fb_exact(const FbArgs &a, double *scratch, size_t stride, int nslots,
                           hipStream_t st, bool from_fold = false);
hipError_t launch_emit(const EmitArgs &a, hipStream_t st);
bool plan_stats(StatsArgs &a, size_t &lds, int &ngroups);
hipError_t launch_resp(const StatsArgs &a, int nchunk, hipStream_t st);
hipError_t launch_stats(const StatsArgs &a, int nchunk, int ngroups, size_t lds, hipStream_t st);
bool plan_stats_list(StatsArgs &a, size_t &lds);
hipError_t launch_gate_list(const StatsArgs &a, int nchunk, hipStream_t st);
size_t gate_list_lds(int K);
size_t resp_lds(int K, int KT);
size_t vhem_resp_lds(int K, int KT);
hipError_t launch_stats_list(const StatsArgs &a, int nchunk, size_t lds, hipStream_t st,
                             int *stats_slabs = nullptr);
hipError_t launch_stats_final(const double *slabs, int nslab, int nslab_stats, int slab_len, int KT,
                              int S, int SL, double *out, hipStream_t st, int *fpre = nullptr,
                              unsigned long long *done = nullptr, unsigned long long done_val = 0);

}
```

clustering-hidden-markov-models-with-variational-bayesian-hierarchical-em_amd/csrc/vbhem_stats.hip:

```cpp
#include <hip/hip_runtime.h>

#include <algorithm>
#include <cmath>
#include <cstdlib>

#include "vbhem_internal.h"
#include "vbhem_exact.h"

namespace vbhem {

namespace {

typedef double double4_t __attribute__((ext_vector_type(4)));

__device__ __forceinline__ double wave_max(double v) {
#pragma unroll
  for (int off = 32; off >= 1; off >>= 1) v = fmax(v, __shfl_xor(v, off, 64));
  return v;
}
__device__ __forceinline__ double wave_sum(double v) {
#pragma unroll
  for (int off = 32; off >= 1; off >>= 1) v += __shfl_xor(v, off, 64);
  return v;
}

__device__ __forceinline__ int qdiv(int x, float inv) { return (int)(((float)x + 0.5f) * inv); }

__device__ __forceinline__ void chunk_range(int nb, int i_begin, int chunk, int nchunk, int &b0,
                                            int &b1) {
  const int per = (nb + nchunk - 1) / nchunk;
  b0 = i_begin + chunk * per;
  b1 = min(i_begin + nb, b0 + per);
}

}

constexpr double kGateZ = 1e-8;
constexpr int kGateVbhem = 0, kGateVhem = 1;
template <int GM>
struct Gate {
  static constexpr double value = GM == kGateVhem ? 0.0 : kGateZ;
};

#ifndef VBHEM_RESP_THREADS
#define VBHEM_RESP_THREADS 512
#endif
constexpr int kRespThreads = VBHEM_RESP_THREADS;
constexpr int kRespFoldWaves = 4;

__device__ __forceinline__ double group_max(double v, int G) {
  for (int off = G >> 1; off >= 1; off >>= 1) v = fmax(v, __shfl_xor(v, off, 64));
  return v;
}
__device__ __forceinline__ double group_sum(double v, int G) {
  for (int off = G >> 1; off >= 1; off >>= 1) v += __shfl_xor(v, off, 64);
  return v;
}

#ifndef VBHEM_RESP_UNROLL
#define VBHEM_RESP_UNROLL 1
#endif

#ifndef VBHEM_RESP_WPE
#define VBHEM_RESP_WPE 4
#endif
typedef unsigned int resp_u2 __attribute__((ext_vector_type(2)));

template <int KP>
__global__ __launch_bounds__(kRespThreads) __attribute__((amdgpu_waves_per_eu(VBHEM_RESP_WPE))) void resp_kernel(
    const StatsArgs p) {
  extern __shared__ double lds[];
  const int tid = threadIdx.x, lane = tid & 63, wave = tid >> 6;
  constexpr int NW = kRespThreads / 64;
  const int K = KP ? KP : p.K;
  int G = KP ? KP : 1;
  if (!KP)
    while (G < K && G < 64) G <<= 1;
  const int BPW = 64 / G;
  const int sub = lane / G, gl = lane - sub * G;
  double *accNj = lds;
  double *accLt = accNj + NW * BPW * K;
  int *gcnt = reinterpret_cast<int *>(accLt + 2 * NW);
  int b0, b1;
  chunk_range(p.i_end - p.i_begin, p.i_begin, blockIdx.x, gridDim.x, b0, b1);
  if (p.fold) {
    int *fc = p.fx.flag_count;
    const int cnt = __atomic_load_n(fc, __ATOMIC_RELAXED);
    if (blockIdx.x == 0 && tid == 0) fc[3] = cnt;
    if (cnt > 0) {
      const int nw = min(kRespFoldWaves, max(1, p.xslots / (int)gridDim.x));
      int *q = reinterpret_cast<int *>(lds), *qn = q + kRespThreads;
      auto mine = [&](int pair) { const int i = pair / K; return i >= b0 && i < b1; };
      if (exact_wave_in_lds(p.fx.S, p.fx.SB))
        fold_exact<false>(p.fx, 0, cnt, mine, p.xscratch, p.xstride, (int)blockIdx.x * nw, nw, q, qn,
                          lds + fold_lds_bytes(kRespThreads, 0, 1, 1) / sizeof(double));
      else
        fold_exact<true>(p.fx, 0, cnt, mine, p.xscratch, p.xstride, (int)blockIdx.x * nw, nw, q, qn,
                         nullptr);
    }
  }
  for (int x = tid; x < NW * BPW * K + 2 * NW; x += kRespThreads) accNj[x] = 0.0;
  for (int x = tid; x < K; x += kRespThreads) gcnt[x] = 0;
  __syncthreads();
  double l1 = 0.0, l7 = 0.0;
  if constexpr (KP > 0) {
    constexpr int BP = 64 / KP;
    const int stride = NW * BP;
    const double lo = p.logOmega[gl];
    const int nb = b1 - b0;
    const __amdgpu_buffer_rsrc_t rh = __builtin_amdgcn_make_buffer_rsrc(
        p.hatZ + (size_t)b0 * KP, (short)0, nb * KP * 8, 0x00020000);
    const __amdgpu_buffer_rsrc_t rz = __builtin_amdgcn_make_buffer_rsrc(
        p.Z + (size_t)(b0 - p.i_buf0) * KP, (short)0, nb * KP * 8, 0x00020000);
    auto step = [&](int ib, double tnb, double llb) {
#pragma clang fp contract(off)
      const bool iv = ib < b1;
      const double lz = tnb * (lo + llb);
      double mx = lz;
#pragma unroll
      for (int off = KP >> 1; off >= 1; off >>= 1) mx = fmax(mx, __shfl_xor(mx, off, 64));
      double sm = exp(lz - mx);
#pragma unroll
      for (int off = KP >> 1; off >= 1; off >>= 1) sm += __shfl_xor(sm, off, 64);
      const double lse = mx + log(sm);
      const double hz = exp(lz - lse) + 1e-50;
      const double Z = hz * tnb;
      const int off = iv ? ((ib - b0) * KP + gl) * 8 : 0x7ffffff0;
      __builtin_amdgcn_raw_buffer_store_b64(__builtin_bit_cast(resp_u2, hz), rh, off, 0, 0);
      __builtin_amdgcn_raw_buffer_store_b64(__builtin_bit_cast(resp_u2, Z), rz, off, 0, 0);
      accNj[(wave * BP + sub) * KP + gl] += iv ? Z : 0.0;
      atomicAdd(&gcnt[gl], (iv && Z > kGateZ) ? 1 : 0);
      l1 += iv ? Z * llb : 0.0;
      l7 += iv ? hz * log(hz) : 0.0;
    };
    auto ld = [&](int ib, double &tnb, double &llb) {
      const int ii = ib < b1 ? ib : b0;
      tnb = p.tildeN[ii];
      llb = p.LL[(size_t)ii * KP + gl];
    };
    int i = b0 + wave * BP + sub;
    double tA, lA, tB, lB;
    ld(i, tA, lA);
    for (; i - sub < b1; i += 2 * stride) {
      ld(i + stride, tB, lB);
      step(i, tA, lA);
      ld(i + 2 * stride, tA, lA);
      step(i + stride, tB, lB);
    }
  } else if (K <= G) {
    const int stride = NW * BPW;
    const double lo = gl < K ? p.logOmega[gl] : 0.0;
    int i = b0 + wave * BPW + sub;
    int ii = i < b1 ? i : b0;
    double tn = p.tildeN[ii];
    double ll = gl < K ? p.LL[(size_t)ii * K + gl] : 0.0;
    auto step = [&](int ib, double tnb, double llb) {
#pragma clang fp contract(off)
      const bool iv = ib < b1;
      const double lz = tnb * (lo + llb);
      double mx = gl < K ? lz : -INFINITY;
      mx = group_max(mx, G);
      double sm = gl < K ? exp(lz - mx) : 0.0;
      sm = group_sum(sm, G);
      const double lse = mx + log(sm);
      if (iv && gl < K) {
        const double hz = exp(lz - lse) + 1e-50;
        const double Z = hz * tnb;
        p.hatZ[(size_t)ib * K + gl] = hz;
        p.Z[(size_t)(ib - p.i_buf0) * K + gl] = Z;
        accNj[(wave * BPW + sub) * K + gl] += Z;
        if (Z > kGateZ) atomicAdd(&gcnt[gl], 1);
        l1 += Z * llb;
        l7 += hz * log(hz);
      }
    };
#if VBHEM_RESP_UNROLL == 2
    for (; i - sub < b1; i += 2 * stride) {
      const int i2 = i + stride, i2c = i2 < b1 ? i2 : b0;
      const int in = i + 2 * stride < b1 ? i + 2 * stride : b0;
      const double tn2 = p.tildeN[i2c];
      const double ll2 = gl < K ? p.LL[(size_t)i2c * K + gl] : 0.0;
      const double tn_n = p.tildeN[in];
      const double ll_n = gl < K ? p.LL[(size_t)in * K + gl] : 0.0;
      step(i, tn, ll);
      step(i2, tn2, ll2);
      tn = tn_n;
      ll = ll_n;
    }
#else
    for (; i - sub < b1; i += stride) {
      const int in = i + stride < b1 ? i + stride : b0;
      const double tn_n = p.tildeN[in];
      const double ll_n = gl < K ? p.LL[(size_t)in * K + gl] : 0.0;
      step(i, tn, ll);
      tn = tn_n;
      ll = ll_n;
    }
#endif
  } else
  for (int i = b0 + wave * BPW + sub; i - sub < b1; i += NW * BPW) {
#pragma clang fp contract(off)
    const bool iv = i < b1;
    const int ii = iv ? i : b0;
    const double tn = p.tildeN[ii];
    const double *LL = p.LL + (size_t)ii * K;
    double mx = -INFINITY;
    for (int j = gl; j < K; j += G) mx = fmax(mx, tn * (p.logOmega[j] + LL[j]));
    mx = group_max(mx, G);
    double sm = 0.0;
    for (int j = gl; j < K; j += G) sm += exp(tn * (p.logOmega[j] + LL[j]) - mx);
    sm = group_sum(sm, G);
    const double lse = mx + log(sm);
    if (iv) {
      for (int j = gl; j < K; j += G) {
        const double ll = LL[j];
        const double hz = exp(tn * (p.logOmega[j] + ll) - lse) + 1e-50;
        const double Z = hz * tn;
        p.hatZ[(size_t)i * K + j] = hz;
        p.Z[(size_t)(i - p.i_buf0) * K + j] = Z;
        accNj[(wave * BPW + sub) * K + j] += Z;
        if (Z > kGateZ) atomicAdd(&gcnt[j], 1);
        l1 += Z * ll;
        l7 += hz * log(hz);
      }
    }
  }
  l1 = wave_sum(l1);
  l7 = wave_sum(l7);
  if (lane == 0) {
    accLt[2 * wave] = l1;
    accLt[2 * wave + 1] = l7;
  }
  __syncthreads();
  double *slab = p.slabs + (size_t)blockIdx.x * p.slab_len;
  for (int j = tid; j < K; j += kRespThreads) {
    double s = 0.0;
    for (int w = 0; w < NW * BPW; ++w) s += accNj[w * K + j];
    slab[j] = p.assign ? s : slab[j] + s;
  }
  if (tid < 2) {
    double s = 0.0;
    for (int w = 0; w < NW; ++w) s += accLt[2 * w + tid];
    double &dst = slab[(size_t)K + (size_t)K * p.S + (size_t)K * p.S * p.S + tid];
    dst = p.assign ? s : dst + s;
  }
  if (p.gate_cnt)
    for (int j = tid; j < K; j += kRespThreads) p.gate_cnt[(size_t)blockIdx.x * K + j] = gcnt[j];
}

constexpr int kRespSlots = 4;

__global__ __launch_bounds__(kRespThreads) void resp_trials_kernel(const StatsArgs p) {
  extern __shared__ double lds[];
  const int tid = threadIdx.x, lane = tid & 63, wave = tid >> 6;
  constexpr int NW = kRespThreads / 64;
  const int K = p.K, KT = p.KT, R = K / KT, SL = p.SL, S = p.S;
  int G = 1;
  while (G < K && G < 64) G <<= 1;
  const int BPW = 64 / G;
  const int sub = lane / G, gl = lane - sub * G;
  double *accNj = lds;
  double *accLt = accNj + NW * BPW * K;
  int *gcnt = reinterpret_cast<int *>(accLt + 2 * NW * R);
  for (int x = tid; x < NW * BPW * K + 2 * NW * R; x += kRespThreads) accNj[x] = 0.0;
  for (int x = tid; x < K; x += kRespThreads) gcnt[x] = 0;
  __syncthreads();
  int tr[kRespSlots];
#pragma unroll
  for (int s = 0; s < kRespSlots; ++s) {
    const int j = gl + s * G;
    tr[s] = j < K ? j / KT : -1;
  }
  int b0, b1;
  chunk_range(p.i_end - p.i_begin, p.i_begin, blockIdx.x, gridDim.x, b0, b1);
  double l1[kRespSlots], l7[kRespSlots];
#pragma unroll
  for (int s = 0; s < kRespSlots; ++s) l1[s] = l7[s] = 0.0;
  for (int i = b0 + wave * BPW + sub; i - sub < b1; i += NW * BPW) {
#pragma clang fp contract(off)
    const bool iv = i < b1;
    const int ii = iv ? i : b0;
    const double tn = p.tildeN[ii];
    const double *LL = p.LL + (size_t)ii * K;
    double lz[kRespSlots], lse[kRespSlots];
#pragma unroll
    for (int s = 0; s < kRespSlots; ++s) {
      const int j = tr[s] >= 0 ? gl + s * G : 0;
      lz[s] = tr[s] >= 0 ? tn * (p.logOmega[j] + LL[j]) : -INFINITY;
      lse[s] = 0.0;
    }
    for (int r = 0; r < R; ++r) {
      double mx = -INFINITY;
#pragma unroll
      for (int s = 0; s < kRespSlots; ++s) mx = tr[s] == r ? fmax(mx, lz[s]) : mx;
      mx = group_max(mx, G);
      double sm = 0.0;
#pragma unroll
      for (int s = 0; s < kRespSlots; ++s) sm += tr[s] == r ? exp(lz[s] - mx) : 0.0;
      sm = group_sum(sm, G);
      const double l = mx + log(sm);
#pragma unroll
      for (int s = 0; s < kRespSlots; ++s) lse[s] = tr[s] == r ? l : lse[s];
    }
    if (iv) {
#pragma unroll
      for (int s = 0; s < kRespSlots; ++s) {
        if (tr[s] < 0) continue;
        const int j = gl + s * G;
        const double hz = exp(lz[s] - lse[s]) + 1e-50;
        const double Z = hz * tn;
        p.hatZ[(size_t)i * K + j] = hz;
        p.Z[(size_t)(i - p.i_buf0) * K + j] = Z;
        accNj[(wave * BPW + sub) * K + j] += Z;
        if (Z > kGateZ) atomicAdd(&gcnt[j], 1);
        l1[s] += Z * LL[j];
        l7[s] += hz * log(hz);
      }
    }
  }
  for (int r = 0; r < R; ++r) {
    double a = 0.0, b = 0.0;
#pragma unroll
    for (int s = 0; s < kRespSlots; ++s) {
      a += tr[s] == r ? l1[s] : 0.0;
      b += tr[s] == r ? l7[s] : 0.0;
    }
    a = wave_sum(a);
    b = wave_sum(b);
    if (lane == 0) {
      accLt[(wave * R + r) * 2] = a;
      accLt[(wave * R + r) * 2 + 1] = b;
    }
  }
  __syncthreads();
  double *slab = p.slabs + (size_t)blockIdx.x * p.slab_len;
  for (int j = tid; j < K; j += kRespThreads) {
    double s = 0.0;
    for (int w = 0; w < NW * BPW; ++w) s += accNj[w * K + j];
    const int r = j / KT;
    double &dst = slab[(size_t)r * SL + (j - r * KT)];
    dst = p.assign ? s : dst + s;
  }
  for (int x = tid; x < 2 * R; x += kRespThreads) {
    const int r = x >> 1, q = x & 1;
    double s = 0.0;
    for (int w = 0; w < NW; ++w) s += accLt[(w * R + r) * 2 + q];
    double &dst = slab[(size_t)r * SL + KT + (size_t)KT * S + (size_t)KT * S * S + q];
    dst = p.assign ? s : dst + s;
  }
  if (p.gate_cnt)
    for (int j = tid; j < K; j += kRespThreads) p.gate_cnt[(size_t)blockIdx.x * K + j] = gcnt[j];
}

__global__ __launch_bounds__(kRespThreads) void vhem_resp_kernel(const StatsArgs p) {
  extern __shared__ double lds[];
  const int tid = threadIdx.x, lane = tid & 63, wave = tid >> 6;
  constexpr int NW = kRespThreads / 64;
  const int K = p.K, KT = p.KT, R = K / KT, SL = p.SL, S = p.S;
  int G = 1;
  while (G < KT && G < 64) G <<= 1;
  const int TPS = 64 / G;
  const int sub = lane / G, gl = lane - sub * G;
  double *accNj = lds;
  double *accL = accNj + NW * K;
  int *gcnt = reinterpret_cast<int *>(accL + NW * R);
  int b0, b1;
  chunk_range(p.i_end - p.i_begin, p.i_begin, blockIdx.x, gridDim.x, b0, b1);
  if (p.fold) {
    int *fc = p.fx.flag_count;
    const int cnt = __atomic_load_n(fc, __ATOMIC_RELAXED);
    if (blockIdx.x == 0 && tid == 0) fc[3] = cnt;
    if (cnt > 0) {
      const int nw = min(kRespFoldWaves, max(1, p.xslots / (int)gridDim.x));
      int *q = reinterpret_cast<int *>(lds), *qn = q + kRespThreads;
      auto mine = [&](int pair) { const int i = pair / K; return i >= b0 && i < b1; };
      if (exact_wave_in_lds(p.fx.S, p.fx.SB))
        fold_exact<false>(p.fx, 0, cnt, mine, p.xscratch, p.xstride, (int)blockIdx.x * nw, nw, q, qn,
                          lds + fold_lds_bytes(kRespThreads, 0, 1, 1) / sizeof(double));
      else
        fold_exact<true>(p.fx, 0, cnt, mine, p.xscratch, p.xstride, (int)blockIdx.x * nw, nw, q, qn,
                         nullptr);
    }
  }
  for (int x = tid; x < NW * K + NW * R; x += kRespThreads) accNj[x] = 0.0;
  for (int x = tid; x < K; x += kRespThreads) gcnt[x] = 0;
  __syncthreads();
  const double inf_norm = p.inf_norm;
  for (int i = b0 + wave; i < b1; i += NW) {
#pragma clang fp contract(off)
    const double ni = p.tildeN[i], ob = p.omegaB[i];
    const double *LL = p.LL + (size_t)i * K;
    for (int r0 = 0; r0 < R; r0 += TPS) {
      const int r = r0 + sub;
      const bool rv = r < R;
      const int jb = (rv ? r : 0) * KT;
      double mx = -INFINITY;
      for (int j = gl; j < KT; j += G)
        mx = fmax(mx, p.logOmega[jb + j] + ni * (LL[jb + j] / inf_norm));
      mx = group_max(mx, G);
      double sm = 0.0;
      for (int j = gl; j < KT; j += G)
        sm += exp((p.logOmega[jb + j] + ni * (LL[jb + j] / inf_norm)) - mx);
      sm = group_sum(sm, G);
      const double lse = mx + log(sm);
      if (rv) {
        for (int j = gl; j < KT; j += G) {
          const double lz = p.logOmega[jb + j] + ni * (LL[jb + j] / inf_norm);
          const double Z = exp(lz - mx) / sm;
          const double w = Z * ob;
          p.hatZ[(size_t)i * K + jb + j] = Z;
          p.Z[(size_t)(i - p.i_buf0) * K + jb + j] = w;
          accNj[wave * K + jb + j] += Z;
          if (w > Gate<kGateVhem>::value) atomicAdd(&gcnt[jb + j], 1);
        }
        if (gl == 0) accL[wave * R + r] += lse;
      }
    }
  }
  __syncthreads();
  double *slab = p.slabs + (size_t)blockIdx.x * p.slab_len;
  for (int j = tid; j < K; j += kRespThreads) {
    double s = 0.0;
    for (int w = 0; w < NW; ++w) s += accNj[w * K + j];
    const int r = j / KT;
    double &dst = slab[(size_t)r * SL + (j - r * KT)];
    dst = p.assign ? s : dst + s;
  }
  for (int x = tid; x < 2 * R; x += kRespThreads) {
    const int r = x >> 1, q = x & 1;
    double s = 0.0;
    if (q == 0)
      for (int w = 0; w < NW; ++w) s += accL[w * R + r];
    double &dst = slab[(size_t)r * SL + KT + (size_t)KT * S + (size_t)KT * S * S + q];
    dst = p.assign ? s : dst + s;
  }
  if (p.gate_cnt)
    for (int j = tid; j < K; j += kRespThreads) p.gate_cnt[(size_t)blockIdx.x * K + j] = gcnt[j];
}

constexpr int kListThreads = 256;

template <int GM>
__global__ __launch_bounds__(kListThreads) void gate_list_kernel(const StatsArgs p) {
  extern __shared__ int ish[];
  const int tid = threadIdx.x, lane = tid & 63, wave = tid >> 6;
  constexpr int NW = kListThreads / 64;
  const int K = p.K, nchunk = gridDim.x, me = blockIdx.x;
  int *before = ish;
  int *total = ish + K;
  int *wcnt = ish + 2 * K;
  int *pb = wcnt + NW;
  int *pt = pb + kListThreads;
  for (int j0 = 0; j0 < K; j0 += kListThreads) {
    const int KC = min(K - j0, kListThreads), R = kListThreads / KC;
    const int r = tid / KC, j = j0 + (tid - r * KC);
    if (r < R) {
      int sb = 0, stt = 0;
      for (int c0 = r; c0 < nchunk; c0 += 32 * R) {
        int v[32];
#pragma unroll
        for (int q = 0; q < 32; ++q) {
          const int c = min(c0 + q * R, nchunk - 1);
          v[q] = p.gate_cnt[(size_t)c * K + j];
        }
#pragma unroll
        for (int q = 0; q < 32; ++q) {
          const int c = c0 + q * R;
          stt += c < nchunk ? v[q] : 0;
          sb += c < me ? v[q] : 0;
        }
      }
      pb[tid] = sb;
      pt[tid] = stt;
    }
    __syncthreads();
    if (tid < KC) {
      int sb = 0, stt = 0;
      for (int q = 0; q < R; ++q) {
        sb += pb[q * KC + tid];
        stt += pt[q * KC + tid];
      }
      before[j0 + tid] = sb;
      total[j0 + tid] = stt;
    }
    __syncthreads();
  }
  if (me == 0)
    for (int j = tid; j < K; j += kListThreads) p.list_tot[j] = total[j];
  int b0, b1;
  chunk_range(p.i_end - p.i_begin, p.i_begin, me, nchunk, b0, b1);
  unsigned long long *msk = reinterpret_cast<unsigned long long *>(
      ish + ((2 * K + NW + 2 * kListThreads + 1) & ~1));
  constexpr int kJB = 16;
  for (int i0 = b0; i0 < b1; i0 += kListThreads) {
    const int i = i0 + tid;
    const bool iv = i < b1;
    const double *Zi = p.Z + (size_t)((iv ? i : b0) - p.i_buf0) * K;
    for (int j0 = 0; j0 < K; j0 += kJB) {
      double z[kJB];
#pragma unroll
      for (int q = 0; q < kJB; ++q) z[q] = j0 + q < K ? Zi[j0 + q] : 0.0;
#pragma unroll
      for (int q = 0; q < kJB; ++q) {
        const unsigned long long m = __ballot(iv && z[q] > Gate<GM>::value);
        if (lane == 0 && j0 + q < K) msk[wave * K + j0 + q] = m;
      }
    }
    __syncthreads();
    for (int j = 0; j < K; ++j) {
      const unsigned long long m = msk[wave * K + j];
      if ((m >> lane) & 1ull) {
        int off = before[j];
        for (int w = 0; w < wave; ++w) off += __popcll(msk[w * K + j]);
        p.list[(size_t)j * p.list_cap + off + __popcll(m & ((1ull << lane) - 1ull))] = i;
      }
    }
    __syncthreads();
    for (int j = tid; j < K; j += kListThreads) {
      int t = 0;
      for (int w = 0; w < NW; ++w) t += __popcll(msk[w * K + j]);
      before[j] += t;
    }
    __syncthreads();
  }
}

constexpr int kSlThreads = 256;

template <int PER>
__global__ __launch_bounds__(kSlThreads) void stats_list_kernel(const StatsArgs p) {
  extern __shared__ double lds[];
  const int tid = threadIdx.x;
  const int K = p.K, S = p.S, SB = p.SB, d = p.d, NU = p.NU, PB = p.PB;
  const int j = blockIdx.y, c = blockIdx.x, nch = gridDim.x;
  const bool full = p.covmode == kCovFull;
  const int dd = full ? d * d : d;
  const int OT = S * SB, OM = OT + S, OU = OM + S * S;
  const int RS = (OU + SB * NU + 1) / 2 * 2;
  const int NO = S + S * S + S * NU;
  double *rec = lds;
  int *tab = reinterpret_cast<int *>(rec + (size_t)PB * RS);
  double *sz = reinterpret_cast<double *>(tab + (NU + 1) / 2 * 2);
  int *sidx = reinterpret_cast<int *>(sz + PB);
  for (int cc = tid; cc < NU; cc += kSlThreads) {
    int a = -1, b = -1;
    if (cc >= 1 && cc <= d) {
      a = cc - 1;
    } else if (cc > d) {
      if (full) {
        int k = cc - 1 - d;
        a = 0;
        while (k >= d - a) { k -= d - a; ++a; }
        b = a + k;
      } else {
        a = b = cc - 1 - d;
      }
    }
    tab[cc] = (a + 1) | ((b + 1) << 16);
  }
  const int tot = p.list_tot[j];
  const int n0 = (int)((long long)tot * c / nch), n1 = (int)((long long)tot * (c + 1) / nch);
  const int *lst = p.list + (size_t)j * p.list_cap;
  const float invNU = 1.0f / (float)NU, invOU = 1.0f / (float)OU, invUN = 1.0f / (float)(SB * NU);
  double *slab = p.slabs + (size_t)c * p.slab_len;
  const int KT = p.KT, tr = j / KT, jt = j - tr * KT;
  double *tsl = slab + (size_t)tr * p.SL;
  for (int o0 = 0; o0 < NO; o0 += PER * kSlThreads) {
    double acc[PER];
#pragma unroll
    for (int e = 0; e < PER; ++e) acc[e] = 0.0;
    for (int n = n0; n < n1; n += PB) {
      const int np = min(PB, n1 - n);
      __syncthreads();
      if (tid < np) {
        const int i = lst[n + tid];
        const size_t lp = (size_t)(i - p.i_buf0) * K + j;
        sidx[tid] = i;
        sz[tid] = p.Z[lp];
      }
      __syncthreads();
      for (int x = tid; x < np * OU; x += kSlThreads) {
        const int pq = qdiv(x, invOU), e = x - pq * OU;
        const size_t lp = (size_t)(sidx[pq] - p.i_buf0) * K + j;
        double v;
        if (e < OT) v = p.tnu[lp * OT + e];
        else if (e < OM) v = p.nu1[lp * S + (e - OT)];
        else v = p.xi[lp * S * S + (e - OM)];
        rec[(size_t)pq * RS + e] = sz[pq] * v;
      }
      for (int x = tid; x < np * SB * NU; x += kSlThreads) {
        const int pq = qdiv(x, invUN), e = x - pq * SB * NU;
        const int bb = qdiv(e, invNU), cc = e - bb * NU;
        const int i = sidx[pq];
        const int t = tab[cc], a = (t & 0xffff) - 1, b2 = (t >> 16) - 1;
        const double *mu = p.centres + ((size_t)i * SB + bb) * d;
        const double *C = p.covars + ((size_t)i * SB + bb) * dd;
        double u;
        if (a < 0) u = 1.0;
        else if (b2 < 0) u = mu[a];
        else u = (full ? C[a * d + b2] : C[a]) + mu[a] * mu[b2];
        rec[(size_t)pq * RS + OU + e] = u;
      }
      __syncthreads();
#pragma unroll
      for (int e = 0; e < PER; ++e) {
        const int o = o0 + tid + e * kSlThreads;
        if (o < S) {
          for (int pq = 0; pq < np; ++pq) acc[e] += rec[(size_t)pq * RS + OT + o];
        } else if (o < S + S * S) {
          for (int pq = 0; pq < np; ++pq) acc[e] += rec[(size_t)pq * RS + OM + (o - S)];
        } else if (o < NO) {
          const int oo = o - S - S * S;
          const int sg = qdiv(oo, invNU), cc = oo - sg * NU;
          for (int pq = 0; pq < np; ++pq) {
            const double *r = rec + (size_t)pq * RS;
            for (int bb = 0; bb < SB; ++bb) acc[e] = fma(r[sg * SB + bb], r[OU + bb * NU + cc], acc[e]);
          }
        }
      }
    }
#pragma unroll
    for (int e = 0; e < PER; ++e) {
      const int o = o0 + tid + e * kSlThreads;
      double *dst = nullptr;
      if (o < S) {
        dst = tsl + KT + (size_t)jt * S + o;
      } else if (o < S + S * S) {
        dst = tsl + KT + (size_t)KT * S + (size_t)jt * S * S + (o - S);
      } else if (o < NO) {
        const int oo = o - S - S * S;
        dst = tsl + KT + (size_t)KT * S + (size_t)KT * S * S + 2 + (size_t)jt * S * NU + oo;
      }
      if (dst) *dst = p.assign ? acc[e] : *dst + acc[e];
    }
  }
}

constexpr int kStatsThreads = 512;
constexpr int kStatsWaves = kStatsThreads / 64;
constexpr int kStatsMaxNBB = 4;
constexpr int kStatsMaxA = 8;
constexpr int kStatsMaxR = 8;

template <int TPW, int GM>
__global__ __launch_bounds__(kStatsThreads) void stats_kernel(const StatsArgs p) {
  extern __shared__ double lds[];
  const int tid = threadIdx.x, lane = tid & 63, wave = tid >> 6;
  const int K = p.K, S = p.S, SB = p.SB, SBp = p.SBp, d = p.d, NU = p.NU, NBB = p.NBB;
  const int AST = p.AST, UST = p.UST;
  const int j0 = blockIdx.y * p.JG, j1 = min(K, j0 + p.JG), JGc = j1 - j0;
  const int RG = JGc * S, SS = S * S;
  const int MT = (RG + 15) / 16, NTL = (NU + 15) / 16, ntiles = MT * NTL;
  const bool full = p.covmode == kCovFull;
  const int dd = full ? d * d : d;
  const int NA = NBB * RG * SB;
  const int NRC = NBB * SB * dd;
  const int NR = NRC + NBB * SB * d;

  double *As = lds;
  double *Us = As + (size_t)RG * AST;
  double *raw = Us + (size_t)NBB * SBp * UST;
  double *gzs = raw + (size_t)NR;
  int *tab = reinterpret_cast<int *>(gzs + (size_t)NBB * JGc);

  for (int x = tid; x < RG * AST + NBB * SBp * UST; x += kStatsThreads) As[x] = 0.0;
  for (int c = tid; c < NU; c += kStatsThreads) {
    int a = -1, b = -1;
    if (c >= 1 && c <= d) {
      a = c - 1;
    } else if (c > d) {
      if (full) {
        int k = c - 1 - d;
        a = 0;
        while (k >= d - a) { k -= d - a; ++a; }
        b = a + k;
      } else {
        a = b = c - 1 - d;
      }
    }
    tab[c] = (a + 1) | ((b + 1) << 16);
  }

  const float invNU = 1.0f / (float)NU, invSB = 1.0f / (float)SB, invS = 1.0f / (float)S;
  const float invJG = 1.0f / (float)JGc;
  const float invRSB = 1.0f / (float)(RG * SB);

  double4_t acc[TPW];
#pragma unroll
  for (int t = 0; t < TPW; ++t) acc[t] = (double4_t){0.0, 0.0, 0.0, 0.0};

  int b0, b1;
  chunk_range(p.i_end - p.i_begin, p.i_begin, blockIdx.x, gridDim.x, b0, b1);
  const double *__restrict__ tnu = p.tnu;

  double pa[kStatsMaxA], pr[kStatsMaxR], pz = 0.0;
  auto prefetch = [&](int ib) {
    const int nq = min(NBB, b1 - ib);
#pragma unroll
    for (int e = 0; e < kStatsMaxA; ++e) {
      const int x = tid + e * kStatsThreads;
      const int q = qdiv(x, invRSB), rem = x - q * RG * SB;
      pa[e] = (x < NA && q < nq) ? tnu[((size_t)(ib + q - p.i_buf0) * K * S + (size_t)j0 * S) * SB + rem]
                                 : 0.0;
    }
    const size_t gs = (size_t)ib * SB;
#pragma unroll
    for (int e = 0; e < kStatsMaxR; ++e) {
      const int x = tid + e * kStatsThreads;
      double v = 0.0;
      if (x < NRC) {
        if (x < nq * SB * dd) v = p.covars[gs * dd + x];
      } else if (x < NR) {
        const int y = x - NRC;
        if (y < nq * SB * d) v = p.centres[gs * d + y];
      }
      pr[e] = v;
    }
    if (tid < NBB * JGc) {
      const int q = qdiv(tid, invJG), jj = tid - q * JGc;
      pz = q < nq ? p.Z[(size_t)(ib + q - p.i_buf0) * K + j0 + jj] : 0.0;
    }
  };
  __syncthreads();
  if (b0 < b1) prefetch(b0);

  for (int ib = b0; ib < b1; ib += NBB) {
    const int nq = min(NBB, b1 - ib);
    if (tid < NBB * JGc) gzs[tid] = (pz > Gate<GM>::value) ? pz : 0.0;
#pragma unroll
    for (int e = 0; e < kStatsMaxR; ++e) {
      const int x = tid + e * kStatsThreads;
      if (x < NR) raw[x] = pr[e];
    }
    __syncthreads();
#pragma unroll
    for (int e = 0; e < kStatsMaxA; ++e) {
      const int x = tid + e * kStatsThreads;
      if (x < NA) {
        const int q = qdiv(x, invRSB), rem = x - q * RG * SB;
        const int r = qdiv(rem, invSB), be = rem - r * SB;
        As[r * AST + q * SBp + be] = (q < nq) ? gzs[q * JGc + qdiv(r, invS)] * pa[e] : 0.0;
      }
    }
    for (int x = tid; x < NBB * SB * NU; x += kStatsThreads) {
      const int row = qdiv(x, invNU), c = x - row * NU;
      const int q = qdiv(row, invSB), be = row - q * SB;
      double u = 0.0;
      if (q < nq) {
        const int t = tab[c], a = (t & 0xffff) - 1, b = (t >> 16) - 1;
        const double *mu = raw + NRC + (size_t)row * d;
        if (a < 0) {
          u = 1.0;
        } else if (b < 0) {
          u = mu[a];
        } else {
          const double *C = raw + (size_t)row * dd;
          u = (full ? C[a * d + b] : C[a]) + mu[a] * mu[b];
        }
      }
      Us[(q * SBp + be) * UST + c] = u;
    }
    __syncthreads();
    if (ib + NBB < b1) prefetch(ib + NBB);
#pragma unroll
    for (int t = 0; t < TPW; ++t) {
      const int tile = wave + t * kStatsWaves;
      if (tile < ntiles) {
        const int mt = tile % MT, nt = tile / MT;
        const int row = mt * 16 + (lane & 15);
        const int col = nt * 16 + (lane & 15);
        const double *arow = As + (size_t)(row < RG ? row : 0) * AST;
        const double amask = row < RG ? 1.0 : 0.0;
        for (int ks = 0; ks < NBB * SBp; ks += 4) {
          const int k = ks + (lane >> 4);
          const double av = amask * arow[k];
          const double bv = Us[k * UST + col];
          acc[t] = __builtin_amdgcn_mfma_f64_16x16x4f64(av, bv, acc[t], 0, 0, 0);
        }
      }
    }
    __syncthreads();
  }

  double *slab = p.slabs + (size_t)blockIdx.x * p.slab_len;
  double *slabU = slab + K + (size_t)K * S + (size_t)K * SS + 2;
#pragma unroll
  for (int t = 0; t < TPW; ++t) {
    const int tile = wave + t * kStatsWaves;
    if (tile < ntiles) {
      const int mt = tile % MT, nt = tile / MT;
      const int col = nt * 16 + (lane & 15);
#pragma unroll
      for (int r = 0; r < 4; ++r) {
        const int row = mt * 16 + (lane >> 4) + 4 * r;
        if (row < RG && col < NU) slabU[((size_t)j0 * S + row) * NU + col] += acc[t][r];
      }
    }
  }
}

constexpr int kNmThreads = 256;

template <int PER, int UNR, int GM>
__global__ __launch_bounds__(kNmThreads) void nm_kernel(const StatsArgs p) {
  const int tid = threadIdx.x;
  const int K = p.K, S = p.S, KS = K * S, KSS = KS * S, NO = KS + KSS;
  int b0, b1;
  chunk_range(p.i_end - p.i_begin, p.i_begin, blockIdx.x, gridDim.x, b0, b1);
  double acc[PER];
  int jo[PER];
#pragma unroll
  for (int e = 0; e < PER; ++e) {
    acc[e] = 0.0;
    const int x = tid + e * kNmThreads;
    jo[e] = x < KS ? x / S : (x < NO ? (x - KS) / (S * S) : 0);
  }
  for (int i = b0; i < b1; i += UNR) {
    double v[UNR][PER], z[UNR][PER];
#pragma unroll
    for (int u = 0; u < UNR; ++u) {
      const bool iv = i + u < b1;
      const size_t ir = (size_t)((iv ? i + u : i) - p.i_buf0);
#pragma unroll
      for (int e = 0; e < PER; ++e) {
        const int x = tid + e * kNmThreads;
        const int xc = x < NO ? x : 0;
        const double *src = xc < KS ? p.nu1 + ir * KS + xc : p.xi + ir * KSS + (xc - KS);
        v[u][e] = *src;
        z[u][e] = p.Z[ir * K + jo[e]];
      }
    }
#pragma unroll
    for (int u = 0; u < UNR; ++u) {
      const bool iv = i + u < b1;
#pragma unroll
      for (int e = 0; e < PER; ++e) {
        const int x = tid + e * kNmThreads;
        const double zz = z[u][e];
        z[u][e] = (iv && x < NO && zz > Gate<GM>::value) ? zz : 0.0;
      }
    }
#pragma unroll
    for (int u = 0; u < UNR; ++u)
#pragma unroll
      for (int e = 0; e < PER; ++e) acc[e] = fma(z[u][e], v[u][e], acc[e]);
  }
  double *slab = p.slabs + (size_t)blockIdx.x * p.slab_len + K;
#pragma unroll
  for (int e = 0; e < PER; ++e) {
    const int x = tid + e * kNmThreads;
    if (x < NO) slab[x] += acc[e];
  }
}

constexpr int kFinalCols = 16, kFinalParts = 16;
__global__ __launch_bounds__(256) void stats_final_kernel(const double *slabs, int nslab_all,
                                                          int nslab_stats, int slab_len, int KT,
                                                          int S, int SL, double *out, int *fpre,
                                                          unsigned long long tag,
                                                          unsigned long long *done,
                                                          unsigned long long done_val) {
  __shared__ double part[kFinalParts][kFinalCols];
  if (fpre && blockIdx.x == 0 && threadIdx.x == 0) {
    int *fc = fpre + kFlagPre;
    fpre[2] = fc[1];
    for (int c = 0; c < kFlagHead; ++c)
      if (!(done && c == 2)) fc[c] = 0;
    *reinterpret_cast<unsigned long long *>(fpre) = tag;
  }
  const int c = threadIdx.x % kFinalCols, pp = threadIdx.x / kFinalCols;
  const int x = blockIdx.x * kFinalCols + c;
  const int xs = x % SL, lt = KT * (1 + S + S * S);
  const int nslab = (xs < KT || (xs >= lt && xs < lt + 2)) ? nslab_all : nslab_stats;
  double acc = 0.0;
  if (x < slab_len) {
    int k = pp;
    for (; k + 3 * kFinalParts < nslab; k += 4 * kFinalParts) {
      const double *q = slabs + (size_t)k * slab_len + x;
      const double v0 = q[0], v1 = q[(size_t)kFinalParts * slab_len],
                   v2 = q[(size_t)2 * kFinalParts * slab_len], v3 = q[(size_t)3 * kFinalParts * slab_len];
      acc += v0;
      acc += v1;
      acc += v2;
      acc += v3;
    }
    for (; k < nslab; k += kFinalParts) acc += slabs[(size_t)k * slab_len + x];
  }
  part[pp][c] = acc;
  __syncthreads();
  if (pp == 0 && x < slab_len) {
    double s = part[0][c];
#pragma unroll
    for (int q = 1; q < kFinalParts; ++q) s += part[q][c];
    if (fpre && __hip_atomic_load(fpre + kFlagLost, __ATOMIC_RELAXED, __HIP_MEMORY_SCOPE_AGENT) ==
                    kFlagLostMark)
      s = __builtin_nan("");
    if (done)
      __hip_atomic_store(reinterpret_cast<unsigned long long *>(out + x), __double_as_longlong(s),
                         __ATOMIC_RELAXED, __HIP_MEMORY_SCOPE_SYSTEM);
    else
      out[x] = s;
  }
  if (done && fpre) {
    __builtin_amdgcn_s_waitcnt(0x0F70);
    __syncthreads();
    if (threadIdx.x == 0) {
      int *cnt = fpre + kFlagPre + 2;
      const int prev = __hip_atomic_fetch_add(cnt, 1, __ATOMIC_RELAXED, __HIP_MEMORY_SCOPE_AGENT);
      if (prev == (int)gridDim.x - 1) {
        __hip_atomic_store(cnt, 0, __ATOMIC_RELAXED, __HIP_MEMORY_SCOPE_AGENT);
        __hip_atomic_store(done, done_val, __ATOMIC_RELAXED, __HIP_MEMORY_SCOPE_SYSTEM);
      }
    }
  }
}

namespace {
constexpr size_t kStatsLdsTarget = 78 * 1024;
constexpr int kMaxTPW = 16;

size_t stats_lds_bytes(int RG, int AST, int NBB, int SBp, int UST, int JG, int NU, int SB, int d,
                       int dd) {
  return ((size_t)RG * AST + (size_t)NBB * SBp * UST + (size_t)NBB * SB * (dd + d) +
          (size_t)NBB * JG) * sizeof(double) +
         (size_t)NU * sizeof(int);
}
}

bool plan_stats(StatsArgs &a, size_t &lds, int &ngroups) {
  const int K = a.K, S = a.S;
  a.SBp = (a.SB + 3) / 4 * 4;
  const int NTL = (a.NU + 15) / 16;
  a.UST = NTL * 16;
  int jg = std::max(1, 128 / S);
  ngroups = (K + jg - 1) / jg;
  jg = (K + ngroups - 1) / ngroups;
  a.JG = jg;
  const int RG = jg * S;
  const int ntiles = ((RG + 15) / 16) * NTL;
  if ((ntiles + kStatsWaves - 1) / kStatsWaves > kMaxTPW) return false;
  if (K * S + K * S * S > 24 * kNmThreads) return false;
  if (RG > kStatsThreads) return false;
  const int dd = a.covmode == kCovFull ? a.d * a.d : a.d;
  int nbb = kStatsMaxNBB;
  for (; nbb >= 1; --nbb) {
    const bool regs_ok = (nbb * RG * a.SB + kStatsThreads - 1) / kStatsThreads <= kStatsMaxA &&
                         (nbb * a.SB * (dd + a.d) + kStatsThreads - 1) / kStatsThreads <= kStatsMaxR;
    a.NBB = nbb;
    a.AST = nbb * a.SBp + 1;
    lds = stats_lds_bytes(RG, a.AST, nbb, a.SBp, a.UST, jg, a.NU, a.SB, a.d, dd);
    if (regs_ok && lds <= kStatsLdsTarget) break;
  }
  if (nbb < 1) return false;
  return true;
}

template <int TPW, int GM>
static hipError_t launch_stats_t(const StatsArgs &a, int nchunk, int ngroups, size_t lds,
                                 hipStream_t st) {
  hipError_t e = set_dyn_lds(reinterpret_cast<const void *>(&stats_kernel<TPW, GM>), lds);
  if (e != hipSuccess) return e;
  hipLaunchKernelGGL((stats_kernel<TPW, GM>), dim3(nchunk, ngroups), dim3(kStatsThreads), lds, st, a);
  if ((e = hipGetLastError()) != hipSuccess) return e;
  const int no = a.K * a.S + a.K * a.S * a.S;
  if (no <= 6 * kNmThreads)
    hipLaunchKernelGGL((nm_kernel<6, 4, GM>), dim3(nchunk), dim3(kNmThreads), 0, st, a);
  else
    hipLaunchKernelGGL((nm_kernel<24, 1, GM>), dim3(nchunk), dim3(kNmThreads), 0, st, a);
  return hipGetLastError();
}

size_t resp_lds(int K, int KT) {
  int G = 1;
  while (G < K && G < 64) G <<= 1;
  const size_t R = KT >= 1 && K % KT == 0 ? (size_t)(K / KT) : 1;
  return std::max(((size_t)(kRespThreads / 64) * ((64 / G) * (size_t)K + 2 * R)) * sizeof(double) +
                      (size_t)K * sizeof(int),
                  (size_t)(kRespThreads + 1) * sizeof(int));
}

template <int KP>
static hipError_t launch_resp_k(const StatsArgs &a, int nchunk, size_t lds, hipStream_t st) {
  hipError_t e = set_dyn_lds(reinterpret_cast<const void *>(&resp_kernel<KP>), lds);
  if (e != hipSuccess) return e;
  hipLaunchKernelGGL(resp_kernel<KP>, dim3(nchunk), dim3(kRespThreads), lds, st, a);
  return hipGetLastError();
}

size_t vhem_resp_lds(int K, int KT) {
  const size_t R = KT >= 1 && K % KT == 0 ? (size_t)(K / KT) : 1;
  return std::max((size_t)(kRespThreads / 64) * ((size_t)K + R) * sizeof(double) +
                      (size_t)K * sizeof(int),
                  (size_t)(kRespThreads + 1) * sizeof(int));
}

hipError_t launch_resp(const StatsArgs &a, int nchunk, hipStream_t st) {
  size_t lds = a.vhem ? vhem_resp_lds(a.K, a.KT) : resp_lds(a.K, a.KT);
  if (a.fold) lds = std::max(lds, fold_lds_bytes(kRespThreads, kRespFoldWaves, a.fx.S, a.fx.SB));
  if (a.vhem) {
    if (a.KT < 1 || a.K % a.KT != 0 || !a.omegaB) return hipErrorInvalidValue;
    hipError_t e = set_dyn_lds(reinterpret_cast<const void *>(&vhem_resp_kernel), lds);
    if (e != hipSuccess) return e;
    hipLaunchKernelGGL(vhem_resp_kernel, dim3(nchunk), dim3(kRespThreads), lds, st, a);
    return hipGetLastError();
  }
  if (a.KT != a.K) {
    if (a.K > kRespSlots * 64 || a.KT < 1 || a.K % a.KT != 0) return hipErrorInvalidValue;
    hipError_t e = set_dyn_lds(reinterpret_cast<const void *>(&resp_trials_kernel), lds);
    if (e != hipSuccess) return e;
    hipLaunchKernelGGL(resp_trials_kernel, dim3(nchunk), dim3(kRespThreads), lds, st, a);
    return hipGetLastError();
  }
  switch (switches().RESP_GENERIC ? 0 : a.K) {
    case 4: return launch_resp_k<4>(a, nchunk, lds, st);
    case 8: return launch_resp_k<8>(a, nchunk, lds, st);
    case 16: return launch_resp_k<16>(a, nchunk, lds, st);
    case 32: return launch_resp_k<32>(a, nchunk, lds, st);
    case 64: return launch_resp_k<64>(a, nchunk, lds, st);
    default: return launch_resp_k<0>(a, nchunk, lds, st);
  }
}

hipError_t launch_stats(const StatsArgs &a, int nchunk, int ngroups, size_t lds, hipStream_t st) {
  const int RG = a.JG * a.S;
  const int ntiles = ((RG + 15) / 16) * ((a.NU + 15) / 16);
  const int tpw = (ntiles + kStatsWaves - 1) / kStatsWaves;
  if (a.vhem) {
    if (tpw <= 4) return launch_stats_t<4, kGateVhem>(a, nchunk, ngroups, lds, st);
    if (tpw <= 8) return launch_stats_t<8, kGateVhem>(a, nchunk, ngroups, lds, st);
    return launch_stats_t<16, kGateVhem>(a, nchunk, ngroups, lds, st);
  }
  if (tpw <= 4) return launch_stats_t<4, kGateVbhem>(a, nchunk, ngroups, lds, st);
  if (tpw <= 8) return launch_stats_t<8, kGateVbhem>(a, nchunk, ngroups, lds, st);
  return launch_stats_t<16, kGateVbhem>(a, nchunk, ngroups, lds, st);
}

constexpr int kSuWaves = 4;

__device__ __forceinline__ void su_output(const StatsArgs &p, const double *red, const double *zs,
                                          int c, int nch, int j, int tid, int row = -1) {
  const int S = p.S, NU = p.NU, d = p.d;
  const bool full = p.covmode == kCovFull;
  const int KT = p.KT, tr = j / KT, jt = j - tr * KT;
  double *tsl = p.slabs + (size_t)c * p.slab_len + (size_t)tr * p.SL;
  const int NO = S * NU + S + S * S;
  for (int o = tid; o < NO; o += 64 * kSuWaves) {
    double v;
    double *dst;
    if (row >= 0 && (o < S * NU ? o / NU : o < S * NU + S ? o - S * NU : (o - S * NU - S) / S) != row) continue;
    if (o < S * NU) {
      const int s2 = o / NU, f = o - s2 * NU;
      const double *rs = red + (size_t)s2 * NU;
      const double N = rs[0];
      if (f == 0) {
        v = N;
      } else if (f <= d) {
        v = fma(zs[f - 1], N, rs[f]);
      } else {
        int a = f - 1 - d, b = a;
        if (full) {
          int k = a;
          a = 0;
          while (k >= d - a) { k -= d - a; ++a; }
          b = a + k;
        }
        const double q2 = (full && a != b) ? 0.5 * rs[f] : rs[f];
        v = q2 + (zs[a] * rs[1 + b] + zs[b] * rs[1 + a]) + zs[a] * zs[b] * N;
      }
      dst = tsl + KT + (size_t)KT * S + (size_t)KT * S * S + 2 + (size_t)jt * S * NU + o;
    } else if (o < S * NU + S) {
      v = red[o];
      dst = tsl + KT + (size_t)jt * S + (o - S * NU);
    } else {
      v = red[o];
      dst = tsl + KT + (size_t)KT * S + (size_t)jt * S * S + (o - S * NU - S);
    }
    *dst = p.assign ? v : *dst + v;
    if (p.assign)
      for (int cz = c + nch; cz < p.nzero; cz += nch) dst[(size_t)(cz - c) * p.slab_len] = 0.0;
  }
}


template <int FPL, int SM>
__global__ __launch_bounds__(64 * kSuWaves) void stats_list_u_kernel(const StatsArgs p) {
  extern __shared__ double lds[];
  const int tid = threadIdx.x, lane = tid & 63, wave = tid >> 6;
  const int K = p.K, S = p.S, SB = p.SB, d = p.d, NU = p.NU, kq = p.ukdp / 4;
  const bool full = p.covmode == kCovFull;
  const int NPF = full ? d * (d + 1) / 2 : d;
  const int j = blockIdx.y, c = blockIdx.x, nch = gridDim.x;
  const int OT = S * SB, TS = (OT + 1) / 2 * 2, KP = p.ukdp + 1;
  const int WS = TS + (SB * KP + 1) / 2 * 2;
  double *tw = lds + (size_t)wave * WS;
  double *uw = tw + TS;
  double *red = lds + (size_t)kSuWaves * WS;
  double *zs = red + (size_t)S * NU + S + S * S;
  for (int a = tid; a < d; a += 64 * kSuWaves) zs[a] = p.uz[a];
  int ue[FPL];
  bool fv[FPL];
#pragma unroll
  for (int q = 0; q < FPL; ++q) {
    const int f = lane + 64 * q;
    fv[q] = f < NU;
    ue[q] = f == 0 ? -1 : f <= d ? NPF + f - 1 : f - 1 - d;
  }
  double acc[FPL][SM], accx[4], accn = 0.0;
#pragma unroll
  for (int q = 0; q < FPL; ++q)
#pragma unroll
    for (int s2 = 0; s2 < SM; ++s2) acc[q][s2] = 0.0;
#pragma unroll
  for (int e = 0; e < 4; ++e) accx[e] = 0.0;
  const int tot = p.list_tot[j];
  const int n0 = (int)((long long)tot * c / nch), n1 = (int)((long long)tot * (c + 1) / nch);
  const int *lst = p.list + (size_t)j * p.list_cap;
  const double *Ub0 = p.U + kUHead;
  for (int nb = n0 + wave; nb < n1; nb += 64 * kSuWaves) {
    const int nl = nb + lane * kSuWaves;
    const int il = nl < n1 ? lst[nl] : 0;
    const int np = min(64, (n1 - nb + kSuWaves - 1) / kSuWaves);
    for (int k = 0; k < np; ++k) {
      const int i = __builtin_amdgcn_readlane(il, k);
      const size_t lp = (size_t)(i - p.i_buf0) * K + j;
      const double z = p.Z[lp];
      {
        double v[4];
#pragma unroll
        for (int e = 0; e < 4; ++e) {
          const int x = lane + 64 * e;
          v[e] = x < OT ? p.tnu[lp * OT + x] : 0.0;
        }
#pragma unroll
        for (int e = 0; e < 4; ++e) {
          const int x = lane + 64 * e;
          if (x < OT) {
            const int s2 = x / SB, b = x - s2 * SB;
            tw[b * S + s2] = z * v[e];
          }
        }
      }
#pragma unroll
      for (int e = 0; e < 4; ++e) {
        const int x = lane + 64 * e;
        if (x < S * S) accx[e] = fma(z, p.xi[lp * S * S + x], accx[e]);
      }
      if (lane < S) accn = fma(z, p.nu1[lp * S + lane], accn);
      const long long c0 = (long long)i * SB - p.u_col0;
      for (int x0 = lane; x0 < 4 * kq * SB; x0 += 64 * 8) {
        double v[8];
#pragma unroll
        for (int e = 0; e < 8; ++e) {
          const int x = x0 + 64 * e;
          const int t4 = x / SB, b = x - t4 * SB;
          const long long col = c0 + b;
          v[e] = x < 4 * kq * SB
                     ? Ub0[(size_t)(col >> 4) * kq * 64 + (t4 >> 2) * 64 + (t4 & 3) * 16 + (col & 15)]
                     : 0.0;
        }
#pragma unroll
        for (int e = 0; e < 8; ++e) {
          const int x = x0 + 64 * e;
          const int t4 = x / SB, b = x - t4 * SB;
          if (x < 4 * kq * SB) uw[b * KP + t4] = v[e];
        }
      }
      __builtin_amdgcn_fence(__ATOMIC_RELEASE, "wavefront");
      __builtin_amdgcn_wave_barrier();
      __builtin_amdgcn_fence(__ATOMIC_ACQUIRE, "wavefront");
#pragma unroll 1
      for (int b = 0; b < SM; ++b) {
        if (b < SB) {
          double uv[FPL];
#pragma unroll
          for (int q = 0; q < FPL; ++q)
            uv[q] = !fv[q] ? 0.0 : ue[q] < 0 ? 1.0 : uw[b * KP + ue[q]];
#pragma unroll
          for (int s2 = 0; s2 < SM; ++s2) {
            if (s2 < S) {
              const double tv = tw[b * S + s2];
#pragma unroll
              for (int q = 0; q < FPL; ++q) acc[q][s2] = fma(tv, uv[q], acc[q][s2]);
            }
          }
        }
      }
      __builtin_amdgcn_fence(__ATOMIC_RELEASE, "wavefront");
      __builtin_amdgcn_wave_barrier();
      __builtin_amdgcn_fence(__ATOMIC_ACQUIRE, "wavefront");
    }
  }
  for (int w = 0; w < kSuWaves; ++w) {
    if (wave == w) {
#pragma unroll
      for (int q = 0; q < FPL; ++q)
#pragma unroll
        for (int s2 = 0; s2 < SM; ++s2) {
          const int f = lane + 64 * q;
          if (fv[q] && s2 < S) {
            double *r = red + (size_t)s2 * NU + f;
            *r = w == 0 ? acc[q][s2] : *r + acc[q][s2];
          }
        }
      if (lane < S) {
        double *r = red + (size_t)S * NU + lane;
        *r = w == 0 ? accn : *r + accn;
      }
#pragma unroll
      for (int e = 0; e < 4; ++e) {
        const int x = lane + 64 * e;
        if (x < S * S) {
          double *r = red + (size_t)S * NU + S + x;
          *r = w == 0 ? accx[e] : *r + accx[e];
        }
      }
    }
    __syncthreads();
  }
  su_output(p, red, zs, c, nch, j, tid);
}

constexpr int kSmWaves = 4;
static_assert(kSmWaves == kSuWaves, "su_output's thread stride");
typedef double dbl4 __attribute__((ext_vector_type(4)));

template <int NTW, int G, int KSM, int NXR, int PD>
__global__ __launch_bounds__(64 * kSmWaves) void stats_list_m_kernel(const StatsArgs p) {
  extern __shared__ double lds[];
  constexpr int TG = kSmWaves / G;
  const int tid = threadIdx.x, lane = tid & 63, wave = __builtin_amdgcn_readfirstlane(tid >> 6);
  const int pg = wave % G, tg = wave / G;
  const int K = p.K, S = p.S, SB = p.SB, d = p.d, NU = p.NU;
  const int SBP = us_sbp(SB), NUP = us_nup(NU), ntile = NUP / 16;
  const int OT = S * SB, NX = S + S * S;
  __shared__ int sm_map[3];
  if (wave == 0) {
    int total = 0;
    for (int x = lane; x < K; x += 64) total += p.list_tot[x];
    for (int o = 32; o > 0; o >>= 1) total += __shfl_xor(total, o, 64);
    const int nb = (int)gridDim.x, P = max(1, (total + max(1, nb - K) - 1) / max(1, nb - K));
    int pre = 0, jj = -1, cc = 0, np = 1;
    for (int x0 = 0; x0 < K && jj < 0; x0 += 64) {
      const int x = x0 + lane;
      int parts = 0;
      if (x < K) {
        const int t = p.list_tot[x], Pj = max(P, (t + p.nzero - 1) / p.nzero);
        parts = max(1, (t + Pj - 1) / Pj);
      }
      int inc = parts;
      for (int o = 1; o < 64; o <<= 1) {
        const int v = __shfl_up(inc, o, 64);
        if (lane >= o) inc += v;
      }
      const int b0 = pre + inc - parts;
      const bool hit = x < K && (int)blockIdx.x >= b0 && (int)blockIdx.x < b0 + parts;
      const unsigned long long m = __ballot(hit);
      if (m) {
        const int src = __builtin_ctzll(m);
        jj = __shfl(x, src, 64);
        cc = (int)blockIdx.x - __shfl(b0, src, 64);
        np = __shfl(parts, src, 64);
      }
      pre += __shfl(inc, 63, 64);
    }
    if (lane == 0) {
      sm_map[0] = jj;
      sm_map[1] = cc;
      sm_map[2] = np;
    }
  }
  __syncthreads();
  const int j = sm_map[0], c = sm_map[1], nch = sm_map[2];
  if (j < 0) return;
  double *red = lds;
  double *zs = red + (size_t)S * NU + S + S * S;
  for (int a = tid; a < d; a += 64 * kSmWaves) zs[a] = p.uz[a];
  const int kl = lane >> 4, cl = lane & 15;
  dbl4 acc[NTW];
#pragma unroll
  for (int t = 0; t < NTW; ++t) acc[t] = dbl4{0.0, 0.0, 0.0, 0.0};
  double ax[NXR];
#pragma unroll
  for (int r = 0; r < NXR; ++r) ax[r] = 0.0;
  const int tot = p.list_tot[j];
  const int n0 = (int)((long long)tot * c / nch), n1 = (int)((long long)tot * (c + 1) / nch);
  const int *lst = p.list + (size_t)j * p.list_cap;
  struct Ops {
    double ta[KSM], ub[NTW][KSM], xv[NXR], z;
  };
  bool ta_ok[KSM];
#pragma unroll
  for (int kk = 0; kk < KSM; ++kk) ta_ok[kk] = cl < S && 4 * kk + kl < SB;
  Ops buf[PD];
  auto load = [&](int i, Ops &o) {
    const size_t lp = (size_t)(i - p.i_buf0) * K + j;
    unsigned zo = (unsigned)lp;
    asm("" : "+v"(zo));
    o.z = p.Z[zo];
    const double *us = p.Us + (size_t)i * SBP * NUP;
    const double *tp = p.tnu + lp * OT, *n1p = p.nu1 + lp * S, *xp = p.xi + lp * S * S;
#pragma unroll
    for (int kk = 0; kk < KSM; ++kk) {
      const int b = 4 * kk + kl;
      o.ta[kk] = tp[ta_ok[kk] ? (unsigned)(cl * SB + b) : 0u];
#pragma unroll
      for (int t = 0; t < NTW; ++t) {
        const int ft = min(tg + TG * t, ntile - 1);
        o.ub[t][kk] = us[(unsigned)((ft * SBP + b) * 16 + cl)];
      }
    }
#pragma unroll
    for (int r = 0; r < NXR; ++r) {
      const int x = lane + 64 * (tg + TG * r);
      o.xv[r] = *(x < S ? n1p + x : xp + (x < NX ? x - S : 0));
    }
  };
  auto compute = [&](const Ops &o) {
#pragma unroll
    for (int kk = 0; kk < KSM; ++kk) {
      const double av = o.z * (ta_ok[kk] ? o.ta[kk] : 0.0);
#pragma unroll
      for (int t = 0; t < NTW; ++t)
        if (tg + TG * t < ntile) acc[t] = __builtin_amdgcn_mfma_f64_16x16x4f64(av, o.ub[t][kk], acc[t], 0, 0, 0);
    }
#pragma unroll
    for (int r = 0; r < NXR; ++r) ax[r] = fma(o.z, o.xv[r], ax[r]);
  };
  const int nf = n0 + pg;
  const int cnt = nf < n1 ? (n1 - nf + G - 1) / G : 0;
  if (cnt > 0) {
    const int kmax = cnt - 1;
    const int *lw = lst + nf;
#pragma unroll
    for (int u = 0; u < PD - 1; ++u) load(lw[G * min(u, kmax)], buf[u]);
    int inext = lw[G * min(PD - 1, kmax)];
    for (int k0 = 0; k0 < cnt; k0 += PD) {
#pragma unroll
      for (int u = 0; u < PD; ++u) {
        const int k = k0 + u;
        const int il = inext;
        inext = lw[G * min(k + PD, kmax)];
        load(il, buf[(u + PD - 1) % PD]);
        if (k < cnt) compute(buf[u]);
      }
    }
  }
  for (int g = 0; g < G; ++g) {
    if (pg == g) {
#pragma unroll
      for (int t = 0; t < NTW; ++t) {
        const int f = 16 * (tg + TG * t) + cl;
        if (tg + TG * t < ntile && f < NU)
#pragma unroll
          for (int v = 0; v < 4; ++v) {
            const int s2 = kl + 4 * v;
            if (s2 < S) {
              double *r = red + (size_t)s2 * NU + f;
              *r = g == 0 ? acc[t][v] : *r + acc[t][v];
            }
          }
      }
#pragma unroll
      for (int r = 0; r < NXR; ++r) {
        const int x = lane + 64 * (tg + TG * r);
        if (x < NX) {
          double *o = red + (size_t)S * NU + x;
          *o = g == 0 ? ax[r] : *o + ax[r];
        }
      }
    }
    __syncthreads();
  }
  su_output(p, red, zs, c, nch, j, tid);
}

constexpr int kL4rParts = 16, kL4rCols = 64, kL4rThreads = kL4rParts * kL4rCols;
__global__ __launch_bounds__(kL4rThreads) void list4_stats_reduce_kernel(const StatsArgs p,
                                                                        const double *parts, int nw) {
  extern __shared__ double lds[];
  __shared__ int plan[2];
  __shared__ double part[kL4rParts][kL4rCols];
  const int tid = threadIdx.x, S = p.S, j = blockIdx.x / S, s2 = blockIdx.x - j * S;
  const int NU = p.NU, NUP = us_nup(NU), d = p.d;
  if (tid == 0) {
    int nitem = 0, pre = 0;
    for (int x = 0; x < p.K; ++x) {
      if (x == j) pre = nitem;
      nitem += l4s_items(p.list_tot[x]);
    }
    const int per = l4s_per_wave(nitem, nw), n = l4s_items(p.list_tot[j]);
    plan[0] = l4s_slot(pre, j, per);
    plan[1] = n ? l4s_slot(pre + n - 1, j, per) - plan[0] + 1 : 0;
  }
  __syncthreads();
  const int s0 = plan[0], ns = plan[1];
  const int NO = S * NU + S + S * S, PL = l4s_part_len(S, NUP);
  double *red = lds;
  double *zs = red + NO;
  for (int a = tid; a < d; a += kL4rThreads) zs[a] = p.uz[a];
  const int q = tid / kL4rCols, col = tid - q * kL4rCols;
  const bool cv = col < NU + 1 + S;
  const int src = col < NU ? s2 * NUP + col : col == NU ? S * NUP + s2 : S * NUP + S + s2 * S + (col - NU - 1);
  const int dst = col < NU ? s2 * NU + col : col == NU ? S * NU + s2 : S * NU + S + s2 * S + (col - NU - 1);
  const int k0 = (int)((long long)ns * q / kL4rParts), k1 = (int)((long long)ns * (q + 1) / kL4rParts);
  double acc = 0.0;
  if (cv) {
    const double *g = parts + (size_t)s0 * PL + src;
    int k = k0;
    for (; k + 7 < k1; k += 8) {
      double v[8];
#pragma unroll
      for (int u = 0; u < 8; ++u) v[u] = g[(size_t)(k + u) * PL];
#pragma unroll
      for (int u = 0; u < 8; ++u) acc += v[u];
    }
    for (; k < k1; ++k) acc += g[(size_t)k * PL];
  }
  part[q][col] = acc;
  __syncthreads();
  if (q == 0 && cv) {
    double t = part[0][col];
#pragma unroll
    for (int x = 1; x < kL4rParts; ++x) t += part[x][col];
    red[dst] = t;
  }
  __syncthreads();
  if (tid < 64 * kSuWaves) su_output(p, red, zs, 0, 1, j, tid, s2);
}

template <int LG, int SM>
__global__ __launch_bounds__(64 * kSuWaves) void stats_list_g_kernel(const StatsArgs p) {
  extern __shared__ double lds[];
  constexpr int NG = 64 / LG;
  const int tid = threadIdx.x, lane = tid & 63, wave = tid >> 6;
  const int grp = lane / LG, gl = lane - grp * LG;
  const int K = p.K, S = p.S, SB = p.SB, d = p.d, NU = p.NU, kq = p.ukdp / 4;
  const bool full = p.covmode == kCovFull;
  const int NPF = full ? d * (d + 1) / 2 : d;
  const int j = blockIdx.y, c = blockIdx.x, nch = gridDim.x;
  const int OT = S * SB, TS = (OT + 1) / 2 * 2, KP = p.ukdp + 1;
  const int WS = TS + (SB * KP + 1) / 2 * 2;
  double *tw = lds + (size_t)(wave * NG + grp) * WS;
  double *uw = tw + TS;
  double *red = lds + (size_t)kSuWaves * NG * WS;
  double *zs = red + (size_t)S * NU + S + S * S;
  for (int a = tid; a < d; a += 64 * kSuWaves) zs[a] = p.uz[a];
  const bool fv = gl < NU;
  const int ue = gl == 0 ? -1 : gl <= d ? NPF + gl - 1 : gl - 1 - d;
  double acc[SM], accx[4], accn = 0.0;
#pragma unroll
  for (int s2 = 0; s2 < SM; ++s2) acc[s2] = 0.0;
#pragma unroll
  for (int e = 0; e < 4; ++e) accx[e] = 0.0;
  const int tot = p.list_tot[j];
  const int n0 = (int)((long long)tot * c / nch), n1 = (int)((long long)tot * (c + 1) / nch);
  const int *lst = p.list + (size_t)j * p.list_cap;
  const double *Ub0 = p.U + kUHead;
  const int nu4 = 4 * kq * SB;
  for (int nb = n0 + wave * NG; nb < n1; nb += kSuWaves * NG) {
    const int n = nb + grp;
    const bool pv = n < n1;
    const int i = lst[pv ? n : n0];
    const size_t lp = (size_t)(i - p.i_buf0) * K + j;
    const double z = pv ? p.Z[lp] : 0.0;
    double tv[4], xv[4], uv[8];
#pragma unroll
    for (int e = 0; e < 4; ++e) {
      const int x = gl + LG * e;
      tv[e] = x < OT ? p.tnu[lp * OT + x] : 0.0;
      xv[e] = x < S * S ? p.xi[lp * S * S + x] : 0.0;
    }
    const double nv = gl < S ? p.nu1[lp * S + gl] : 0.0;
    const long long c0 = (long long)i * SB - p.u_col0;
#pragma unroll
    for (int e = 0; e < 8; ++e) {
      const int x = gl + LG * e;
      const int t4 = x / SB, b = x - t4 * SB;
      const long long col = c0 + b;
      uv[e] = x < nu4 ? Ub0[(size_t)(col >> 4) * kq * 64 + (t4 >> 2) * 64 + (t4 & 3) * 16 + (col & 15)]
                      : 0.0;
    }
#pragma unroll
    for (int e = 0; e < 4; ++e) {
      const int x = gl + LG * e;
      if (x < OT) {
        const int s2 = x / SB, b = x - s2 * SB;
        tw[b * S + s2] = z * tv[e];
      }
      accx[e] = fma(z, xv[e], accx[e]);
    }
    accn = fma(z, nv, accn);
#pragma unroll
    for (int e = 0; e < 8; ++e) {
      const int x = gl + LG * e;
      const int t4 = x / SB, b = x - t4 * SB;
      if (x < nu4) uw[b * KP + t4] = uv[e];
    }
    __builtin_amdgcn_fence(__ATOMIC_RELEASE, "wavefront");
    __builtin_amdgcn_wave_barrier();
    __builtin_amdgcn_fence(__ATOMIC_ACQUIRE, "wavefront");
    if (fv) {
#pragma unroll 1
      for (int b = 0; b < SB; ++b) {
        const double u = ue < 0 ? 1.0 : uw[b * KP + ue];
#pragma unroll
        for (int s2 = 0; s2 < SM; ++s2)
          if (s2 < S) acc[s2] = fma(tw[b * S + s2], u, acc[s2]);
      }
    }
    __builtin_amdgcn_fence(__ATOMIC_RELEASE, "wavefront");
    __builtin_amdgcn_wave_barrier();
    __builtin_amdgcn_fence(__ATOMIC_ACQUIRE, "wavefront");
  }
  for (int w = 0; w < kSuWaves; ++w) {
    if (wave == w) {
      for (int g = 0; g < NG; ++g) {
        if (grp == g) {
          const bool first = w == 0 && g == 0;
#pragma unroll
          for (int s2 = 0; s2 < SM; ++s2)
            if (fv && s2 < S) {
              double *r = red + (size_t)s2 * NU + gl;
              *r = first ? acc[s2] : *r + acc[s2];
            }
          if (gl < S) {
            double *r = red + (size_t)S * NU + gl;
            *r = first ? accn : *r + accn;
          }
#pragma unroll
          for (int e = 0; e < 4; ++e) {
            const int x = gl + LG * e;
            if (x < S * S) {
              double *r = red + (size_t)S * NU + S + x;
              *r = first ? accx[e] : *r + accx[e];
            }
          }
        }
        __builtin_amdgcn_fence(__ATOMIC_RELEASE, "wavefront");
        __builtin_amdgcn_wave_barrier();
        __builtin_amdgcn_fence(__ATOMIC_ACQUIRE, "wavefront");
      }
    }
    __syncthreads();
  }
  su_output(p, red, zs, c, nch, j, tid);
}

size_t gate_list_lds(int K) {
  const size_t ints = (size_t)2 * K + kListThreads / 64 + 2 * kListThreads;
  return (ints + 1) / 2 * 2 * sizeof(int) +
         (size_t)(kListThreads / 64) * K * sizeof(unsigned long long);
}

hipError_t launch_gate_list(const StatsArgs &a, int nchunk, hipStream_t st) {
  const size_t lds = gate_list_lds(a.K);
  auto *fn = a.vhem ? &gate_list_kernel<kGateVhem> : &gate_list_kernel<kGateVbhem>;
  hipError_t e = set_dyn_lds(reinterpret_cast<const void *>(fn), lds);
  if (e != hipSuccess) return e;
  hipLaunchKernelGGL(fn, dim3(nchunk), dim3(kListThreads), lds, st, a);
  return hipGetLastError();
}

namespace {
constexpr size_t kSlLdsBudget = 48 * 1024;
int sl_record(const StatsArgs &a) {
  const int OU = a.S * a.SB + a.S + a.S * a.S;
  return (OU + a.SB * a.NU + 1) / 2 * 2;
}
}

bool plan_stats_list(StatsArgs &a, size_t &lds) {
  const size_t rs = (size_t)sl_record(a) * sizeof(double);
  const size_t tab = (size_t)(a.NU + 1) / 2 * 2 * sizeof(int);
  if (rs + tab + 12 > kSlLdsBudget) return false;
  a.PB = (int)std::min<size_t>(6, (kSlLdsBudget - tab) / (rs + 12));
  lds = (size_t)a.PB * (rs + 12) + tab;
  return a.PB >= 1;
}

template <int FPL, int SM>
static hipError_t launch_su(const StatsArgs &a, const dim3 &grid, hipStream_t st) {
  const int OT = a.S * a.SB, KP = a.ukdp + 1;
  const size_t ws = (size_t)(OT + 1) / 2 * 2 + ((size_t)a.SB * KP + 1) / 2 * 2;
  const size_t lds = ((size_t)kSuWaves * ws + (size_t)a.S * a.NU + a.S + (size_t)a.S * a.S + a.d) *
                     sizeof(double);
  auto *fn = &stats_list_u_kernel<FPL, SM>;
  hipError_t e = set_dyn_lds(reinterpret_cast<const void *>(fn), lds);
  if (e != hipSuccess) return e;
  hipLaunchKernelGGL(fn, grid, dim3(64 * kSuWaves), lds, st, a);
  return hipGetLastError();
}

template <int NTW, int G, int KSM, int NXR, int PD>
static hipError_t launch_sm_pd(const StatsArgs &a, const dim3 &grid, hipStream_t st) {
  const size_t lds = ((size_t)a.S * a.NU + a.S + (size_t)a.S * a.S + a.d) * sizeof(double);
  auto *fn = &stats_list_m_kernel<NTW, G, KSM, NXR, PD>;
  hipError_t e = set_dyn_lds(reinterpret_cast<const void *>(fn), lds);
  if (e != hipSuccess) return e;
  long long nb = (long long)resident_per_cu(reinterpret_cast<const void *>(fn), 64 * kSmWaves, lds) *
                 device_cus();
  if (switches().SU_BLOCKS >= 0) nb = switches().SU_BLOCKS;
  nb = std::min<long long>(std::max<long long>(nb, a.K + 1), grid.x);
  hipLaunchKernelGGL(fn, dim3((unsigned)nb), dim3(64 * kSmWaves), lds, st, a);
  return hipGetLastError();
}

#ifndef VBHEM_SM_PDD
#define VBHEM_SM_PDD 3
#endif
template <int NTW, int G, int KSM, int NXR>
static hipError_t launch_sm(const StatsArgs &a, const dim3 &grid, hipStream_t st) {
  return launch_sm_pd<NTW, G, KSM, NXR, VBHEM_SM_PDD>(a, grid, st);
}

template <int NTW, int G, int KSM>
static hipError_t launch_sm_x(const StatsArgs &a, const dim3 &grid, hipStream_t st) {
  constexpr int TG = kSmWaves / G;
  const int nxr = ((a.S + a.S * a.S + 63) / 64 + TG - 1) / TG;
  if (nxr <= 1) return launch_sm<NTW, G, KSM, 1>(a, grid, st);
  if (nxr <= 2) return launch_sm<NTW, G, KSM, 2>(a, grid, st);
  if (nxr <= 3) return launch_sm<NTW, G, KSM, 3>(a, grid, st);
  return launch_sm<NTW, G, KSM, 5>(a, grid, st);
}

template <int KSM>
static hipError_t launch_sm_k(const StatsArgs &a, const dim3 &grid, hipStream_t st) {
  const int nt = us_nup(a.NU) / 16;
  switch (nt) {
    case 1: return launch_sm_x<1, 4, KSM>(a, grid, st);
    case 2: return launch_sm_x<2, 4, KSM>(a, grid, st);
    case 3: return launch_sm_x<3, 4, KSM>(a, grid, st);
    case 4: return launch_sm_x<4, 4, KSM>(a, grid, st);
    case 5: case 6: return launch_sm_x<3, 2, KSM>(a, grid, st);
    case 7: case 8: return launch_sm_x<4, 2, KSM>(a, grid, st);
    default: return launch_sm_x<3, 1, KSM>(a, grid, st);
  }
}

template <int LG, int SM>
static hipError_t launch_sg(const StatsArgs &a, const dim3 &grid, hipStream_t st) {
  const int OT = a.S * a.SB, KP = a.ukdp + 1;
  const size_t ws = (size_t)(OT + 1) / 2 * 2 + ((size_t)a.SB * KP + 1) / 2 * 2;
  const size_t lds = ((size_t)kSuWaves * (64 / LG) * ws + (size_t)a.S * a.NU + a.S +
                      (size_t)a.S * a.S + a.d) * sizeof(double);
  auto *fn = &stats_list_g_kernel<LG, SM>;
  hipError_t e = set_dyn_lds(reinterpret_cast<const void *>(fn), lds);
  if (e != hipSuccess) return e;
  hipLaunchKernelGGL(fn, grid, dim3(64 * kSuWaves), lds, st, a);
  return hipGetLastError();
}

static int sg_lanes(const StatsArgs &a) {
  if (switches().NO_STATS_G) return 0;
  const int OT = a.S * a.SB, nu4 = a.ukdp * a.SB;
  for (int LG : {8, 16, 32})
    if (a.NU <= LG && OT <= 4 * LG && a.S * a.S <= 4 * LG && nu4 <= 8 * LG) return LG;
  return 0;
}

template <int LG>
static hipError_t launch_sg_s(const StatsArgs &a, const dim3 &grid, hipStream_t st) {
  if (a.S <= 4) return launch_sg<LG, 4>(a, grid, st);
  if (a.S <= 8) return launch_sg<LG, 8>(a, grid, st);
  if (a.S <= 12) return launch_sg<LG, 12>(a, grid, st);
  return launch_sg<LG, 16>(a, grid, st);
}

template <int FPL>
static hipError_t launch_su_s(const StatsArgs &a, const dim3 &grid, hipStream_t st) {
  if (a.S <= 4) return launch_su<FPL, 4>(a, grid, st);
  if (a.S <= 8) return launch_su<FPL, 8>(a, grid, st);
  if (a.S <= 12) return launch_su<FPL, 12>(a, grid, st);
  return launch_su<FPL, 16>(a, grid, st);
}

hipError_t launch_stats_list(const StatsArgs &a, int nchunk, size_t lds, hipStream_t st,
                             int *stats_slabs) {
  if (stats_slabs) *stats_slabs = nchunk;
  const int NO = a.S + a.S * a.S + a.S * a.NU;
  const dim3 grid(nchunk, a.K);
  const Switches &sw = switches();
  const bool no_u = sw.NO_STATS_U;
  const long long NOb = (long long)a.S + (long long)a.S * a.S + (long long)a.S * a.NU;
  long long cap = (4ll << 20) / (NOb * std::max(1, a.K));
  cap = std::min<long long>(cap, 4096 / std::max(1, a.K));
  if (sw.SU_BLOCKS >= 0) cap = sw.SU_BLOCKS / std::max(1, a.K);
  const int nb = (int)std::max(1ll, std::min((long long)nchunk, cap));
  const dim3 g2(nb, a.K);
  StatsArgs b = a;
  b.nzero = nchunk;
  const int lg = a.U ? sg_lanes(a) : 0;
  if (a.fold == 1) {
    hipError_t e = launch_fb_exact(a.fx, a.xscratch, (size_t)a.xstride, kExactSlots, st, true);
    if (e != hipSuccess) return e;
  }
  const bool z32 = (unsigned long long)(a.i_end - a.i_buf0) * (unsigned long long)a.K < (1ull << 32);
  if (a.Us && !no_u && z32 && a.S <= 16 && a.SB <= 16 && us_nup(a.NU) <= 12 * 16 &&
      !sw.NO_STATS_M) {
    if (a.nzero_m > 0) b.nzero = std::min(a.nzero_m, nchunk);
    if (stats_slabs) *stats_slabs = b.nzero;
    const dim3 g1((unsigned)std::min<long long>((long long)nchunk * a.K, 1ll << 30));
    switch (us_sbp(a.SB) / 4) {
      case 1: return launch_sm_k<1>(b, g1, st);
      case 2: return launch_sm_k<2>(b, g1, st);
      case 3: return launch_sm_k<3>(b, g1, st);
      default: return launch_sm_k<4>(b, g1, st);
    }
  }
  const bool su = a.NU <= 64 || sw.STATS_U;
  if (a.U && su && a.S <= 16 && a.SB <= a.S && a.NU <= 3 * 64 && !no_u) {
    const dim3 gg(sw.SU_BLOCKS >= 0 ? nb : std::max(1, nb / 2), a.K);
    switch (lg) {
      case 8: return launch_sg_s<8>(b, gg, st);
      case 16: return launch_sg_s<16>(b, gg, st);
      case 32: return launch_sg_s<32>(b, gg, st);
      default: break;
    }
    if (a.NU <= 64) return launch_su_s<1>(b, g2, st);
    if (a.NU <= 128) return launch_su_s<2>(b, g2, st);
    return launch_su_s<3>(b, g2, st);
  }
  if (NO <= 4 * kSlThreads) {
    hipLaunchKernelGGL((stats_list_kernel<4>), grid, dim3(kSlThreads), lds, st, a);
  } else {
    hipError_t e = set_dyn_lds(reinterpret_cast<const void *>(&stats_list_kernel<8>), lds);
    if (e != hipSuccess) return e;
    hipLaunchKernelGGL((stats_list_kernel<8>), grid, dim3(kSlThreads), lds, st, a);
  }
  return hipGetLastError();
}

hipError_t launch_list4_stats_reduce(const StatsArgs &a, const double *parts, int nw, hipStream_t st) {
  if (!parts || nw < 1 || !a.uz || !a.list_tot) return hipErrorInvalidValue;
  StatsArgs b = a;
  b.nzero = 1;
  if (a.NU + 1 + a.S > kL4rCols) return hipErrorInvalidValue;
  const size_t lds = ((size_t)(a.S * a.NU + a.S + a.S * a.S) + a.d) * sizeof(double);
  hipLaunchKernelGGL(list4_stats_reduce_kernel, dim3(a.K * a.S), dim3(kL4rThreads), lds, st, b, parts, nw);
  return hipGetLastError();
}

hipError_t launch_stats_final(const double *slabs, int nslab, int nslab_stats, int slab_len, int KT,
                              int S, int SL, double *out, hipStream_t st, int *fpre,
                              unsigned long long *done, unsigned long long done_val) {
  if (nslab_stats < 1 || nslab_stats > nslab || SL < 1 || slab_len % SL != 0) return hipErrorInvalidValue;
  hipLaunchKernelGGL(stats_final_kernel, dim3((slab_len + kFinalCols - 1) / kFinalCols), dim3(256),
                     0, st, slabs, nslab, nslab_stats, slab_len, KT, S, SL, out, fpre,
                     fpre ? flag_tag() : 0ull, fpre ? done : nullptr, done_val);
  return hipGetLastError();
}

}
```

clustering-hidden-markov-models-with-variational-bayesian-hierarchical-em_amd/csrc/vbhem_switches.h:

```cpp
#pragma once

#define VBHEM_SWITCHES(X)                                                                      \
  X(FUSED_DENSE, 0, "dense schedule instead of the gated one (vbhem_set_fused_mode)")          \
  X(NO_UGEMM, 0, "emission on the raw / generic kernels instead of the prepared operand")      \
  X(GROUP_BASES, -1, "tests: at most n bases per group of the fused call")                     \
  X(NSLAB, -1, "tests: at most n statistics slabs (1 .. 8192)")                                \
  X(NO_BWD2, 0, "backward pass on fb_split_kernel's backward mode, not fb_bwd2_kernel")        \
  X(NO_BWD4, 0, "S = 8: fb_bwd2_kernel<8> instead of fb_bwd4_kernel")                          \
  X(NO_BWD12, 0, "S = 12: fb_bwd2_kernel<12> instead of fb_bwd12_kernel")                      \
  X(NO_LIST4, 0, "S = 8: fb_split_kernel's list mode instead of fb_list4_kernel")              \
  X(NO_LIST12, 0, "S = 12: fb_split_kernel's list mode instead of fb_list12_kernel")           \
  X(NO_K1_IN_KERNEL, 0, "short K1 through the emission GEMM, not inside the recursion")        \
  X(NO_LIST4_STATS, 0, "S = 8: per-pair outputs + stats_list_m_kernel, not sums in fb_list4_kernel") \
  X(NO_LIST_INLINE, 0, "the gate-list pass's flagged pairs through an fb_exact_kernel launch") \
  X(NO_BWD2_PREP, 0, "emission_prep_kernel launched, not its work inside fb_bwd2_kernel")      \
  X(NO_FOLD_EXACT, 0, "the backward pass's fallback as a launch, not folded into resp_kernel") \
  X(EM_NOBST, 0, "the one-chunk emission GEMM without buffer stores")                          \
  X(EM_SPLIT, -1, "the one-chunk emission GEMM in whole (0) or half (1) tiles")                \
  X(EM_NODB, 0, "the chunked emission GEMM on emission_u_kernel, not emission_db_kernel")      \
  X(RESP_GENERIC, 0, "resp_kernel's generic path for every K")                                 \
  X(SU_BLOCKS, -1, "gated statistics: the block count")                                        \
  X(NO_STATS_G, 0, "gated statistics: no lane-grouped kernel")                                 \
  X(NO_STATS_U, 0, "gated statistics: the covariance-gather kernel")                           \
  X(NO_STATS_M, 0, "gated statistics: without stats_list_m_kernel")                            \
  X(STATS_U, 0, "gated statistics: the prepared-operand kernel at any NU")                     \
  X(EM_HOST_MATH, 0, "the EM loop's per-iteration math on the host")

namespace vbhem {

struct Switches {
#define X(name, unset, doc) long long name = unset;
  VBHEM_SWITCHES(X)
#undef X
};

const Switches &switches();

}
```

Measured before the change: 582.9 E-steps/s.

## Pass resp gate masks to gate-list kernel and fold list4 reduce into final stats

resp_kernel now records per-base gate bitmasks with a wavefront ballot and stores them in a new workspace buffer. gate_list_kernel reads these masks instead of reloading Z and comparing it again. The per-lane LDS atomicAdd on gate counts is replaced by a register count plus one atomic per lane at the end. When all bases fit in one group, list4_stats_reduce_kernel's work moves into a templated stats_final_kernel, which saves a launch and a pass over the partial sums, at the cost of more code paths and extra workspace.

Result: no change. 588.1 E-steps/s (median of 6 runs) (+0.9%).

```diff
diff --git a/clustering-hidden-markov-models-with-variational-bayesian-hierarchical-em_amd/csrc/vbhem_capi.hip b/clustering-hidden-markov-models-with-variational-bayesian-hierarchical-em_amd/csrc/vbhem_capi.hip
--- a/clustering-hidden-markov-models-with-variational-bayesian-hierarchical-em_amd/csrc/vbhem_capi.hip
+++ b/clustering-hidden-markov-models-with-variational-bayesian-hierarchical-em_amd/csrc/vbhem_capi.hip
@@ -34,7 +34,7 @@
 };
 thread_local TimingState g_timing;
 
-thread_local std::string g_last_kernel[3];
+thread_local std::string g_last_kernel[4];
 std::string split_name(const vbhem::SplitArgs &a) {
   return "vbhem::fb_split_kernel<" + std::to_string(a.S) + ", " + std::to_string(a.lpc) + ", " +
          std::to_string(a.mode) + ">";
@@ -370,6 +370,7 @@
   double *E, *W, *bias, *shift;
   double *U;
   double *l4parts;
+  unsigned long long *gate_mask;
 };
 
 size_t carve_fused(void *ws, const vbhem_base_t *b, const vbhem_cluster_t *c, int T, FusedWs &w,
@@ -410,6 +411,7 @@
                                     vbhem::l4s_part_len(S, vbhem::us_nup(NU)))
                   : nullptr;
   w.scratch = cv.take<double>(exact_stride(S, SB, T) * kExactThreads);
+  w.gate_mask = cv.take<unsigned long long>(vbhem::gate_mask_words(g, w.nslab, K));
   return cv.off + 256;
 }
 
@@ -733,7 +735,7 @@
 size_t vbhem_debug_extra_lds(size_t bytes) { return g_debug_extra_lds.exchange(bytes); }
 
 const char *vbhem_last_kernel(int pass) {
-  return (pass >= 0 && pass <= 2) ? g_last_kernel[pass].c_str() : "";
+  return (pass >= 0 && pass <= 3) ? g_last_kernel[pass].c_str() : "";
 }
 
 const char *vbhem_version(void) { return "vbhem-mi355x 0.1.0 (gfx950)"; }
@@ -979,6 +981,7 @@
   if (!gated && !dense_ok)
     return fail(VBHEM_ERR_UNSUPPORTED, "statistics tile does not fit (S or d too large)");
   sa.gate_cnt = gated ? w.gate_cnt : nullptr;
+  sa.gate_mask = gated && !vh && R == 1 && !sw.NO_GATE_MASK ? w.gate_mask : nullptr;
   sa.list = w.list; sa.list_tot = w.list_tot; sa.list_cap = w.group;
   auto chunks = [&w](int nb) { return std::min(w.nslab, (nb + kChunkMinBases - 1) / kChunkMinBases); };
   const int nslab_used = std::max(1, chunks(std::min(base->N, w.group)));
@@ -1014,6 +1017,7 @@
   const bool fold = gated && R == 1 && base->N <= w.group && ctx.split.ok && K < kExactThreads &&
                     w.nslab <= kExactThreads && !sw.NO_FOLD_EXACT;
   sa.fold = 0;
+  vbhem::FinalFold ffold{};
   for (int g0 = 0; g0 < base->N; g0 += w.group) {
     const int g1 = std::min(base->N, g0 + w.group);
     const long long e_ld = (long long)w.group * SB;
@@ -1058,8 +1062,12 @@
       if (l4w > 0) {
         ss = 1;
         g_last_kernel[2] = "vbhem::list4_stats_reduce_kernel";
-        e = vbhem::launch_list4_stats_reduce(sa, w.l4parts, l4w, st);
-        if (e != hipSuccess) return hip_fail(e, "list4_stats_reduce_kernel");
+        if (base->N <= w.group && R == 1 && !sw.NO_FINAL_FOLD) {
+          ffold = vbhem::FinalFold{w.l4parts, l4w, sa.list_tot, sa.uz, K, sa.NU, d, base->covmode};
+        } else {
+          e = vbhem::launch_list4_stats_reduce(sa, w.l4parts, l4w, st);
+          if (e != hipSuccess) return hip_fail(e, "list4_stats_reduce_kernel");
+        }
       } else {
         g_last_kernel[2] = "vbhem::stats_list_kernels";
         e = vbhem::launch_stats_list(sa, nchunk, sl_lds, st, &ss);
@@ -1073,7 +1081,9 @@
     if (ev0) g_timing.stats.emplace_back(ev0, timing_event(st));
   }
   e = vbhem::launch_stats_final(w.slabs, nslab_used, stats_slabs, w.slab_len, sa.KT, S, sa.SL,
-                                stats_dev, st, w.fpre, done_word, done_val);
+                                stats_dev, st, w.fpre, done_word, done_val,
+                                ffold.parts ? &ffold : nullptr);
+  g_last_kernel[3] = ffold.parts ? "vbhem::stats_final_kernel<true>" : "vbhem::stats_final_kernel<false>";
   if (e != hipSuccess) return hip_fail(e, "stats_final_kernel");
   guard.fpre = nullptr;
   return VBHEM_OK;
@@ -1085,6 +1095,21 @@
                              void *workspace_dev, size_t workspace_bytes, void *stream) {
   return fused_impl(base, clus, R, T, tildeN_dev, logOmega_dev, stats_dev, hatZ_dev, LL_elbo_dev,
                     workspace_dev, workspace_bytes, stream, nullptr);
+}
+
+int vbhem_fused_gate_lists(const vbhem_base_t *base, const vbhem_cluster_t *clus, int T,
+                           void *workspace_dev, void *stream, int *tot, int *list, size_t list_ints,
+                           int *cap) {
+  if (!base || !clus || !workspace_dev || !tot || !cap) return fail(VBHEM_ERR_ARG, "null argument");
+  FusedWs w;
+  carve_fused(workspace_dev, base, clus, T, w, 1);
+  *cap = w.group;
+  hipStream_t st = static_cast<hipStream_t>(stream);
+  hipError_t e = hipMemcpyAsync(tot, w.list_tot, sizeof(int) * (size_t)clus->K, hipMemcpyDeviceToHost, st);
+  if (e == hipSuccess && list && list_ints >= (size_t)clus->K * w.group)
+    e = hipMemcpyAsync(list, w.list, sizeof(int) * (size_t)clus->K * w.group, hipMemcpyDeviceToHost, st);
+  if (e == hipSuccess) e = hipStreamSynchronize(st);
+  return e == hipSuccess ? VBHEM_OK : hip_fail(e, "vbhem_fused_gate_lists");
 }
 
 size_t vhem_fused_workspace_bytes(const vbhem_base_t *base, const vbhem_cluster_t *clus, int T) {
diff --git a/clustering-hidden-markov-models-with-variational-bayesian-hierarchical-em_amd/csrc/vbhem_internal.h b/clustering-hidden-markov-models-with-variational-bayesian-hierarchical-em_amd/csrc/vbhem_internal.h
--- a/clustering-hidden-markov-models-with-variational-bayesian-hierarchical-em_amd/csrc/vbhem_internal.h
+++ b/clustering-hidden-markov-models-with-variational-bayesian-hierarchical-em_amd/csrc/vbhem_internal.h
@@ -106,6 +106,7 @@
   double *Z;
   double *hatZ, *slabs;
   int *gate_cnt;
+  unsigned long long *gate_mask;
   int *list;
   int *list_tot;
   int list_cap;
@@ -346,12 +347,32 @@
 bool plan_stats_list(StatsArgs &a, size_t &lds);
 hipError_t launch_gate_list(const StatsArgs &a, int nchunk, hipStream_t st);
 size_t gate_list_lds(int K);
+__host__ __device__ inline int gate_mask_kb(int K) {
+  int G = 1;
+  while (G < K && G < 64) G <<= 1;
+  return K <= 64 ? G : (K + 63) / 64 * 64;
+}
+__host__ __device__ inline size_t gate_mask_chunk_words(int nb, int nchunk, int K) {
+  const int per = (nb + nchunk - 1) / nchunk;
+  return ((size_t)per * gate_mask_kb(K) + 63) / 64;
+}
+inline size_t gate_mask_words(size_t group, int nslab, int K) {
+  return ((group + (size_t)nslab) * gate_mask_kb(K) + 63) / 64 + (size_t)nslab;
+}
 size_t resp_lds(int K, int KT);
 size_t vhem_resp_lds(int K, int KT);
 hipError_t launch_stats_list(const StatsArgs &a, int nchunk, size_t lds, hipStream_t st,
                              int *stats_slabs = nullptr);
+struct FinalFold {
+  const double *parts;
+  int nw;
+  const int *list_tot;
+  const double *uz;
+  int K, NU, d, covmode;
+};
 hipError_t launch_stats_final(const double *slabs, int nslab, int nslab_stats, int slab_len, int KT,
                               int S, int SL, double *out, hipStream_t st, int *fpre = nullptr,
-                              unsigned long long *done = nullptr, unsigned long long done_val = 0);
-
-}
+                              unsigned long long *done = nullptr, unsigned long long done_val = 0,
+                              const FinalFold *fold = nullptr);
+
+}
diff --git a/clustering-hidden-markov-models-with-variational-bayesian-hierarchical-em_amd/csrc/vbhem_stats.hip b/clustering-hidden-markov-models-with-variational-bayesian-hierarchical-em_amd/csrc/vbhem_stats.hip
--- a/clustering-hidden-markov-models-with-variational-bayesian-hierarchical-em_amd/csrc/vbhem_stats.hip
+++ b/clustering-hidden-markov-models-with-variational-bayesian-hierarchical-em_amd/csrc/vbhem_stats.hip
@@ -3,6 +3,7 @@
 #include <algorithm>
 #include <cmath>
 #include <cstdlib>
+#include <type_traits>
 
 #include "vbhem_internal.h"
 #include "vbhem_exact.h"
@@ -102,7 +103,11 @@
   for (int x = tid; x < NW * BPW * K + 2 * NW; x += kRespThreads) accNj[x] = 0.0;
   for (int x = tid; x < K; x += kRespThreads) gcnt[x] = 0;
   __syncthreads();
+  unsigned long long *gm =
+      p.gate_mask ? p.gate_mask + (size_t)blockIdx.x * gate_mask_chunk_words(p.i_end - p.i_begin, gridDim.x, K)
+                  : nullptr;
   double l1 = 0.0, l7 = 0.0;
+  int gc = 0;
   if constexpr (KP > 0) {
     constexpr int BP = 64 / KP;
     const int stride = NW * BP;
@@ -112,7 +117,12 @@
         p.hatZ + (size_t)b0 * KP, (short)0, nb * KP * 8, 0x00020000);
     const __amdgpu_buffer_rsrc_t rz = __builtin_amdgcn_make_buffer_rsrc(
         p.Z + (size_t)(b0 - p.i_buf0) * KP, (short)0, nb * KP * 8, 0x00020000);
-    auto step = [&](int ib, double tnb, double llb) {
+    const __amdgpu_buffer_rsrc_t rm = __builtin_amdgcn_make_buffer_rsrc(
+        gm, (short)0, gm ? (nb + BP - 1) / BP * 8 : 0, 0x00020000);
+    const bool mreg = !gm || (nb + stride - 1) / stride + 1 <= 64;
+    unsigned long long mw = 0;
+    int nstep = 0;
+    auto step = [&](int ib, double tnb, double llb, auto in_regs) {
 #pragma clang fp contract(off)
       const bool iv = ib < b1;
       const double lz = tnb * (lo + llb);
@@ -129,7 +139,16 @@
       __builtin_amdgcn_raw_buffer_store_b64(__builtin_bit_cast(resp_u2, hz), rh, off, 0, 0);
       __builtin_amdgcn_raw_buffer_store_b64(__builtin_bit_cast(resp_u2, Z), rz, off, 0, 0);
       accNj[(wave * BP + sub) * KP + gl] += iv ? Z : 0.0;
-      atomicAdd(&gcnt[gl], (iv && Z > kGateZ) ? 1 : 0);
+      const bool gt = iv && Z > kGateZ;
+      gc += gt ? 1 : 0;
+      const unsigned long long m = __ballot(gt);
+      if constexpr (decltype(in_regs)::value) {
+        mw = lane == nstep ? m : mw;
+        ++nstep;
+      } else {
+        __builtin_amdgcn_raw_buffer_store_b64(__builtin_bit_cast(resp_u2, m), rm,
+                                              (lane == 0 && iv) ? (ib - b0) / BP * 8 : 0x7ffffff0, 0, 0);
+      }
       l1 += iv ? Z * llb : 0.0;
       l7 += iv ? hz * log(hz) : 0.0;
     };
@@ -138,14 +157,23 @@
       tnb = p.tildeN[ii];
       llb = p.LL[(size_t)ii * KP + gl];
     };
-    int i = b0 + wave * BP + sub;
-    double tA, lA, tB, lB;
-    ld(i, tA, lA);
-    for (; i - sub < b1; i += 2 * stride) {
-      ld(i + stride, tB, lB);
-      step(i, tA, lA);
-      ld(i + 2 * stride, tA, lA);
-      step(i + stride, tB, lB);
+    auto steps = [&](auto in_regs) {
+      int i = b0 + wave * BP + sub;
+      double tA, lA, tB, lB;
+      ld(i, tA, lA);
+      for (; i - sub < b1; i += 2 * stride) {
+        ld(i + stride, tB, lB);
+        step(i, tA, lA, in_regs);
+        ld(i + 2 * stride, tA, lA);
+        step(i + stride, tB, lB, in_regs);
+      }
+    };
+    if (mreg) {
+      steps(std::true_type{});
+      const int w = wave + lane * NW;
+      if (gm && lane < nstep && w * BP < nb) gm[w] = mw;
+    } else {
+      steps(std::false_type{});
     }
   } else if (K <= G) {
     const int stride = NW * BPW;
@@ -163,16 +191,20 @@
       double sm = gl < K ? exp(lz - mx) : 0.0;
       sm = group_sum(sm, G);
       const double lse = mx + log(sm);
+      bool gt = false;
       if (iv && gl < K) {
         const double hz = exp(lz - lse) + 1e-50;
         const double Z = hz * tnb;
         p.hatZ[(size_t)ib * K + gl] = hz;
         p.Z[(size_t)(ib - p.i_buf0) * K + gl] = Z;
         accNj[(wave * BPW + sub) * K + gl] += Z;
-        if (Z > kGateZ) atomicAdd(&gcnt[gl], 1);
+        gt = Z > kGateZ;
         l1 += Z * llb;
         l7 += hz * log(hz);
       }
+      gc += gt ? 1 : 0;
+      const unsigned long long m = __ballot(gt);
+      if (gm && lane == 0 && iv) gm[(ib - b0) / BPW] = m;
     };
 #if VBHEM_RESP_UNROLL == 2
     for (; i - sub < b1; i += 2 * stride) {
@@ -219,12 +251,16 @@
         p.hatZ[(size_t)i * K + j] = hz;
         p.Z[(size_t)(i - p.i_buf0) * K + j] = Z;
         accNj[(wave * BPW + sub) * K + j] += Z;
-        if (Z > kGateZ) atomicAdd(&gcnt[j], 1);
+        const bool gt = Z > kGateZ;
+        if (gt) atomicAdd(&gcnt[j], 1);
+        const unsigned long long m = __ballot(gt);
+        if (gm && gl == 0) gm[(size_t)(i - b0) * (gate_mask_kb(K) / 64) + (j >> 6)] = m;
         l1 += Z * ll;
         l7 += hz * log(hz);
       }
     }
   }
+  if (K <= G && gl < K) atomicAdd(&gcnt[gl], gc);
   l1 = wave_sum(l1);
   l7 = wave_sum(l7);
   if (lane == 0) {
@@ -451,6 +487,18 @@
   int *wcnt = ish + 2 * K;
   int *pb = wcnt + NW;
   int *pt = pb + kListThreads;
+  int b0, b1;
+  chunk_range(p.i_end - p.i_begin, p.i_begin, me, nchunk, b0, b1);
+  const unsigned long long *gm = nullptr;
+  int KB = 0;
+  if (GM == kGateVbhem && p.gate_mask) {
+    KB = gate_mask_kb(K);
+    gm = p.gate_mask + (size_t)me * gate_mask_chunk_words(p.i_end - p.i_begin, nchunk, K);
+  }
+  auto mword = [&](int i, int j0) {
+    return i < b1 ? gm[((size_t)(i - b0) * KB + j0) >> 6] : 0ull;
+  };
+  unsigned long long mw = gm ? mword(b0 + tid, 0) : 0ull;
   for (int j0 = 0; j0 < K; j0 += kListThreads) {
     const int KC = min(K - j0, kListThreads), R = kListThreads / KC;
     const int r = tid / KC, j = j0 + (tid - r * KC);
@@ -487,8 +535,6 @@
   }
   if (me == 0)
     for (int j = tid; j < K; j += kListThreads) p.list_tot[j] = total[j];
-  int b0, b1;
-  chunk_range(p.i_end - p.i_begin, p.i_begin, me, nchunk, b0, b1);
   unsigned long long *msk = reinterpret_cast<unsigned long long *>(
       ish + ((2 * K + NW + 2 * kListThreads + 1) & ~1));
   constexpr int kJB = 16;
@@ -496,7 +542,18 @@
     const int i = i0 + tid;
     const bool iv = i < b1;
     const double *Zi = p.Z + (size_t)((iv ? i : b0) - p.i_buf0) * K;
+    const int msh = (int)(((size_t)(i - b0) * KB) & 63);
     for (int j0 = 0; j0 < K; j0 += kJB) {
+      if (gm) {
+        if ((j0 & 63) == 0 && (i0 > b0 || j0 > 0)) mw = mword(i, j0);
+#pragma unroll
+        for (int q = 0; q < kJB; ++q) {
+          const unsigned long long m =
+              __ballot(j0 + q < K && ((mw >> ((msh + (j0 & 63) + q) & 63)) & 1ull));
+          if (lane == 0 && j0 + q < K) msk[wave * K + j0 + q] = m;
+        }
+        continue;
+      }
       double z[kJB];
 #pragma unroll
       for (int q = 0; q < kJB; ++q) z[q] = j0 + q < K ? Zi[j0 + q] : 0.0;
@@ -853,68 +910,6 @@
   }
 }
 
-constexpr int kFinalCols = 16, kFinalParts = 16;
-__global__ __launch_bounds__(256) void stats_final_kernel(const double *slabs, int nslab_all,
-                                                          int nslab_stats, int slab_len, int KT,
-                                                          int S, int SL, double *out, int *fpre,
-                                                          unsigned long long tag,
-                                                          unsigned long long *done,
-                                                          unsigned long long done_val) {
-  __shared__ double part[kFinalParts][kFinalCols];
-  if (fpre && blockIdx.x == 0 && threadIdx.x == 0) {
-    int *fc = fpre + kFlagPre;
-    fpre[2] = fc[1];
-    for (int c = 0; c < kFlagHead; ++c)
-      if (!(done && c == 2)) fc[c] = 0;
-    *reinterpret_cast<unsigned long long *>(fpre) = tag;
-  }
-  const int c = threadIdx.x % kFinalCols, pp = threadIdx.x / kFinalCols;
-  const int x = blockIdx.x * kFinalCols + c;
-  const int xs = x % SL, lt = KT * (1 + S + S * S);
-  const int nslab = (xs < KT || (xs >= lt && xs < lt + 2)) ? nslab_all : nslab_stats;
-  double acc = 0.0;
-  if (x < slab_len) {
-    int k = pp;
-    for (; k + 3 * kFinalParts < nslab; k += 4 * kFinalParts) {
-      const double *q = slabs + (size_t)k * slab_len + x;
-      const double v0 = q[0], v1 = q[(size_t)kFinalParts * slab_len],
-                   v2 = q[(size_t)2 * kFinalParts * slab_len], v3 = q[(size_t)3 * kFinalParts * slab_len];
-      acc += v0;
-      acc += v1;
-      acc += v2;
-      acc += v3;
-    }
-    for (; k < nslab; k += kFinalParts) acc += slabs[(size_t)k * slab_len + x];
-  }
-  part[pp][c] = acc;
-  __syncthreads();
-  if (pp == 0 && x < slab_len) {
-    double s = part[0][c];
-#pragma unroll
-    for (int q = 1; q < kFinalParts; ++q) s += part[q][c];
-    if (fpre && __hip_atomic_load(fpre + kFlagLost, __ATOMIC_RELAXED, __HIP_MEMORY_SCOPE_AGENT) ==
-                    kFlagLostMark)
-      s = __builtin_nan("");
-    if (done)
-      __hip_atomic_store(reinterpret_cast<unsigned long long *>(out + x), __double_as_longlong(s),
-                         __ATOMIC_RELAXED, __HIP_MEMORY_SCOPE_SYSTEM);
-    else
-      out[x] = s;
-  }
-  if (done && fpre) {
-    __builtin_amdgcn_s_waitcnt(0x0F70);
-    __syncthreads();
-    if (threadIdx.x == 0) {
-      int *cnt = fpre + kFlagPre + 2;
-      const int prev = __hip_atomic_fetch_add(cnt, 1, __ATOMIC_RELAXED, __HIP_MEMORY_SCOPE_AGENT);
-      if (prev == (int)gridDim.x - 1) {
-        __hip_atomic_store(cnt, 0, __ATOMIC_RELAXED, __HIP_MEMORY_SCOPE_AGENT);
-        __hip_atomic_store(done, done_val, __ATOMIC_RELAXED, __HIP_MEMORY_SCOPE_SYSTEM);
-      }
-    }
-  }
-}
-
 namespace {
 constexpr size_t kStatsLdsTarget = 78 * 1024;
 constexpr int kMaxTPW = 16;
@@ -1037,6 +1032,39 @@
 
 constexpr int kSuWaves = 4;
 
+__device__ __forceinline__ double su_entry(const double *red, const double *zs, int S, int NU, int d,
+                                           bool full, int KT, int jt, int o, size_t &off) {
+  double v;
+  if (o < S * NU) {
+    const int s2 = o / NU, f = o - s2 * NU;
+    const double *rs = red + (size_t)s2 * NU;
+    const double N = rs[0];
+    if (f == 0) {
+      v = N;
+    } else if (f <= d) {
+      v = fma(zs[f - 1], N, rs[f]);
+    } else {
+      int a = f - 1 - d, b = a;
+      if (full) {
+        int k = a;
+        a = 0;
+        while (k >= d - a) { k -= d - a; ++a; }
+        b = a + k;
+      }
+      const double q2 = (full && a != b) ? 0.5 * rs[f] : rs[f];
+      v = q2 + (zs[a] * rs[1 + b] + zs[b] * rs[1 + a]) + zs[a] * zs[b] * N;
+    }
+    off = KT + (size_t)KT * S + (size_t)KT * S * S + 2 + (size_t)jt * S * NU + o;
+  } else if (o < S * NU + S) {
+    v = red[o];
+    off = KT + (size_t)jt * S + (o - S * NU);
+  } else {
+    v = red[o];
+    off = KT + (size_t)KT * S + (size_t)jt * S * S + (o - S * NU - S);
+  }
+  return v;
+}
+
 __device__ __forceinline__ void su_output(const StatsArgs &p, const double *red, const double *zs,
                                           int c, int nch, int j, int tid, int row = -1) {
   const int S = p.S, NU = p.NU, d = p.d;
@@ -1045,36 +1073,10 @@
   double *tsl = p.slabs + (size_t)c * p.slab_len + (size_t)tr * p.SL;
   const int NO = S * NU + S + S * S;
   for (int o = tid; o < NO; o += 64 * kSuWaves) {
-    double v;
-    double *dst;
     if (row >= 0 && (o < S * NU ? o / NU : o < S * NU + S ? o - S * NU : (o - S * NU - S) / S) != row) continue;
-    if (o < S * NU) {
-      const int s2 = o / NU, f = o - s2 * NU;
-      const double *rs = red + (size_t)s2 * NU;
-      const double N = rs[0];
-      if (f == 0) {
-        v = N;
-      } else if (f <= d) {
-        v = fma(zs[f - 1], N, rs[f]);
-      } else {
-        int a = f - 1 - d, b = a;
-        if (full) {
-          int k = a;
-          a = 0;
-          while (k >= d - a) { k -= d - a; ++a; }
-          b = a + k;
-        }
-        const double q2 = (full && a != b) ? 0.5 * rs[f] : rs[f];
-        v = q2 + (zs[a] * rs[1 + b] + zs[b] * rs[1 + a]) + zs[a] * zs[b] * N;
-      }
-      dst = tsl + KT + (size_t)KT * S + (size_t)KT * S * S + 2 + (size_t)jt * S * NU + o;
-    } else if (o < S * NU + S) {
-      v = red[o];
-      dst = tsl + KT + (size_t)jt * S + (o - S * NU);
-    } else {
-      v = red[o];
-      dst = tsl + KT + (size_t)KT * S + (size_t)jt * S * S + (o - S * NU - S);
-    }
+    size_t off;
+    const double v = su_entry(red, zs, S, NU, d, full, KT, jt, o, off);
+    double *dst = tsl + off;
     *dst = p.assign ? v : *dst + v;
     if (p.assign)
       for (int cz = c + nch; cz < p.nzero; cz += nch) dst[(size_t)(cz - c) * p.slab_len] = 0.0;
@@ -1428,6 +1430,140 @@
   if (tid < 64 * kSuWaves) su_output(p, red, zs, 0, 1, j, tid, s2);
 }
 
+constexpr int kFinalCols = 16, kFinalParts = 16;
+static_assert(kFinalParts == kL4rParts, "the folded reduction's partitions");
+template <bool FOLD>
+__global__ __launch_bounds__(FOLD ? kL4rThreads : 256) void stats_final_kernel(
+    const double *slabs, int nslab_all, int nslab_stats, int slab_len, int KT, int S, int SL,
+    double *out, int *fpre, unsigned long long tag, unsigned long long *done,
+    unsigned long long done_val, const FinalFold f) {
+  constexpr int NC = FOLD ? kL4rCols : kFinalCols;
+  extern __shared__ double lds[];
+  __shared__ double part[kFinalParts][NC];
+  __shared__ int plan[2];
+  if (fpre && blockIdx.x == 0 && threadIdx.x == 0) {
+    int *fc = fpre + kFlagPre;
+    fpre[2] = fc[1];
+    for (int c = 0; c < kFlagHead; ++c)
+      if (!(done && c == 2)) fc[c] = 0;
+    *reinterpret_cast<unsigned long long *>(fpre) = tag;
+  }
+  const int c = threadIdx.x % NC, pp = threadIdx.x / NC;
+  const int nrow = FOLD ? f.K * S : 0;
+  long long x = -1;
+  double s = 0.0;
+  if (FOLD && (int)blockIdx.x < nrow) {
+    const int tid = threadIdx.x, j = blockIdx.x / S, s2 = blockIdx.x - j * S;
+    const int NU = f.NU, NUP = us_nup(NU), d = f.d;
+    if (tid == 0) {
+      int nitem = 0, pre = 0;
+      for (int y = 0; y < f.K; ++y) {
+        if (y == j) pre = nitem;
+        nitem += l4s_items(f.list_tot[y]);
+      }
+      const int per = l4s_per_wave(nitem, f.nw), n = l4s_items(f.list_tot[j]);
+      plan[0] = l4s_slot(pre, j, per);
+      plan[1] = n ? l4s_slot(pre + n - 1, j, per) - plan[0] + 1 : 0;
+    }
+    __syncthreads();
+    const int s0 = plan[0], ns = plan[1];
+    const int NO = S * NU + S + S * S, PL = l4s_part_len(S, NUP);
+    double *red = lds;
+    double *zs = red + NO;
+    for (int a = tid; a < d; a += kL4rThreads) zs[a] = f.uz[a];
+    const bool cv = c < NU + 1 + S;
+    const int src = c < NU ? s2 * NUP + c : c == NU ? S * NUP + s2 : S * NUP + S + s2 * S + (c - NU - 1);
+    const int dst = c < NU ? s2 * NU + c : c == NU ? S * NU + s2 : S * NU + S + s2 * S + (c - NU - 1);
+    const int k0 = (int)((long long)ns * pp / kL4rParts), k1 = (int)((long long)ns * (pp + 1) / kL4rParts);
+    double acc = 0.0;
+    if (cv) {
+      const double *g = f.parts + (size_t)s0 * PL + src;
+      int k = k0;
+      for (; k + 7 < k1; k += 8) {
+        double v[8];
+#pragma unroll
+        for (int u = 0; u < 8; ++u) v[u] = g[(size_t)(k + u) * PL];
+#pragma unroll
+        for (int u = 0; u < 8; ++u) acc += v[u];
+      }
+      for (; k < k1; ++k) acc += g[(size_t)k * PL];
+    }
+    part[pp][c] = acc;
+    __syncthreads();
+    if (pp == 0 && cv) {
+      double t = part[0][c];
+#pragma unroll
+      for (int q = 1; q < kL4rParts; ++q) t += part[q][c];
+      red[dst] = t;
+    }
+    __syncthreads();
+    if (pp == 0 && cv) {
+      size_t off;
+      s = su_entry(red, zs, S, NU, d, f.covmode == kCovFull, KT, j, dst, off);
+      x = (long long)off;
+    }
+  } else {
+    const int lt = KT * (1 + S + S * S);
+    int xc, nslab;
+    bool xv;
+    if (FOLD) {
+      const int y = ((int)blockIdx.x - nrow) * NC + c;
+      xv = y < KT + 2;
+      xc = y < KT ? y : lt + (y - KT);
+      nslab = nslab_all;
+    } else {
+      xc = blockIdx.x * NC + c;
+      xv = xc < slab_len;
+      const int xs = xc % SL;
+      nslab = (xs < KT || (xs >= lt && xs < lt + 2)) ? nslab_all : nslab_stats;
+    }
+    double acc = 0.0;
+    if (xv) {
+      int k = pp;
+      for (; k + 3 * kFinalParts < nslab; k += 4 * kFinalParts) {
+        const double *q = slabs + (size_t)k * slab_len + xc;
+        const double v0 = q[0], v1 = q[(size_t)kFinalParts * slab_len],
+                     v2 = q[(size_t)2 * kFinalParts * slab_len], v3 = q[(size_t)3 * kFinalParts * slab_len];
+        acc += v0;
+        acc += v1;
+        acc += v2;
+        acc += v3;
+      }
+      for (; k < nslab; k += kFinalParts) acc += slabs[(size_t)k * slab_len + xc];
+    }
+    part[pp][c] = acc;
+    __syncthreads();
+    if (pp == 0 && xv) {
+      s = part[0][c];
+#pragma unroll
+      for (int q = 1; q < kFinalParts; ++q) s += part[q][c];
+      x = xc;
+    }
+  }
+  if (x >= 0) {
+    if (fpre && __hip_atomic_load(fpre + kFlagLost, __ATOMIC_RELAXED, __HIP_MEMORY_SCOPE_AGENT) ==
+                    kFlagLostMark)
+      s = __builtin_nan("");
+    if (done)
+      __hip_atomic_store(reinterpret_cast<unsigned long long *>(out + x), __double_as_longlong(s),
+                         __ATOMIC_RELAXED, __HIP_MEMORY_SCOPE_SYSTEM);
+    else
+      out[x] = s;
+  }
+  if (done && fpre) {
+    __builtin_amdgcn_s_waitcnt(0x0F70);
+    __syncthreads();
+    if (threadIdx.x == 0) {
+      int *cnt = fpre + kFlagPre + 2;
+      const int prev = __hip_atomic_fetch_add(cnt, 1, __ATOMIC_RELAXED, __HIP_MEMORY_SCOPE_AGENT);
+      if (prev == (int)gridDim.x - 1) {
+        __hip_atomic_store(cnt, 0, __ATOMIC_RELAXED, __HIP_MEMORY_SCOPE_AGENT);
+        __hip_atomic_store(done, done_val, __ATOMIC_RELAXED, __HIP_MEMORY_SCOPE_SYSTEM);
+      }
+    }
+  }
+}
+
 template <int LG, int SM>
 __global__ __launch_bounds__(64 * kSuWaves) void stats_list_g_kernel(const StatsArgs p) {
   extern __shared__ double lds[];
@@ -1742,11 +1878,23 @@
 
 hipError_t launch_stats_final(const double *slabs, int nslab, int nslab_stats, int slab_len, int KT,
                               int S, int SL, double *out, hipStream_t st, int *fpre,
-                              unsigned long long *done, unsigned long long done_val) {
+                              unsigned long long *done, unsigned long long done_val,
+                              const FinalFold *fold) {
   if (nslab_stats < 1 || nslab_stats > nslab || SL < 1 || slab_len % SL != 0) return hipErrorInvalidValue;
-  hipLaunchKernelGGL(stats_final_kernel, dim3((slab_len + kFinalCols - 1) / kFinalCols), dim3(256),
+  if (fold) {
+    const FinalFold &f = *fold;
+    if (!f.parts || f.nw < 1 || !f.uz || !f.list_tot || f.K != KT || SL != slab_len ||
+        f.NU + 1 + S > kL4rCols)
+      return hipErrorInvalidValue;
+    const size_t lds = ((size_t)(S * f.NU + S + S * S) + f.d) * sizeof(double);
+    hipLaunchKernelGGL(stats_final_kernel<true>, dim3(KT * S + (KT + 2 + kL4rCols - 1) / kL4rCols),
+                       dim3(kL4rThreads), lds, st, slabs, nslab, nslab_stats, slab_len, KT, S, SL, out,
+                       fpre, fpre ? flag_tag() : 0ull, fpre ? done : nullptr, done_val, f);
+    return hipGetLastError();
+  }
+  hipLaunchKernelGGL(stats_final_kernel<false>, dim3((slab_len + kFinalCols - 1) / kFinalCols), dim3(256),
                      0, st, slabs, nslab, nslab_stats, slab_len, KT, S, SL, out, fpre,
-                     fpre ? flag_tag() : 0ull, fpre ? done : nullptr, done_val);
+                     fpre ? flag_tag() : 0ull, fpre ? done : nullptr, done_val, FinalFold{});
   return hipGetLastError();
 }
 
diff --git a/clustering-hidden-markov-models-with-variational-bayesian-hierarchical-em_amd/csrc/vbhem_switches.h b/clustering-hidden-markov-models-with-variational-bayesian-hierarchical-em_amd/csrc/vbhem_switches.h
--- a/clustering-hidden-markov-models-with-variational-bayesian-hierarchical-em_amd/csrc/vbhem_switches.h
+++ b/clustering-hidden-markov-models-with-variational-bayesian-hierarchical-em_amd/csrc/vbhem_switches.h
@@ -19,6 +19,8 @@
   X(EM_SPLIT, -1, "the one-chunk emission GEMM in whole (0) or half (1) tiles")                \
   X(EM_NODB, 0, "the chunked emission GEMM on emission_u_kernel, not emission_db_kernel")      \
   X(RESP_GENERIC, 0, "resp_kernel's generic path for every K")                                 \
+  X(NO_GATE_MASK, 0, "gate_list_kernel compares Z again, not resp_kernel's gate masks")        \
+  X(NO_FINAL_FOLD, 0, "list4_stats_reduce_kernel launched, not its sums inside stats_final_kernel") \
   X(SU_BLOCKS, -1, "gated statistics: the block count")                                        \
   X(NO_STATS_G, 0, "gated statistics: no lane-grouped kernel")                                 \
   X(NO_STATS_U, 0, "gated statistics: the covariance-gather kernel")                           \
```
